# lighttransport/nanort

Hardware: AMD Instinct MI355X
Metric: Mrays/s (primary + 1-bounce) at 1920x1080, 1M-tri mesh; BVH build ms (higher is better)
Workload: dtype f32; 1 GPU; C3: Plane(1000,500) = 1,000,000 triangles fp32; 1920x1080 objrender-camera primaries + 1 cosine bounce per hit (2073600 + 2055142 rays per GPU per step); parallelism=replicated BVH, interleaved image rows per GPU

## Files before the change

### nanort_amd/csrc/api_ctx.hip

```cpp
#include "ctx.h"

struct TunableDesc {
  const char *name;
  long long lo, hi;
  long long (*get)(const nrt_ctx *);
  void (*set)(nrt_ctx *, long long);
};
#define NRT_TUNABLE(name_, lo_, hi_, field_, type_)                                                          \
  {name_, lo_, hi_, [](const nrt_ctx *c) -> long long { return (long long)c->field_; },                      \
   [](nrt_ctx *c, long long v) { c->field_ = (type_)v; }}
static const TunableDesc kTunables[] = {
    NRT_TUNABLE("refill_min", 1, 64, refill_min, unsigned),
    NRT_TUNABLE("trav_min", 1, 64, trav_min, unsigned),
    NRT_TUNABLE("trav_min4", 1, 64, trav_min4, unsigned),
    NRT_TUNABLE("f64_row_fetch", 0, 1, f64_row_fetch, int),
    NRT_TUNABLE("leaf_min", 1, 64, leaf_min, unsigned),
    NRT_TUNABLE("chunk_tail_pct", 0, 100, chunk_tail_pct, unsigned),
    NRT_TUNABLE("parts", 1, kMaxParts, num_parts, unsigned),
    NRT_TUNABLE("static_pct", 0, 100, static_pct, unsigned),
    NRT_TUNABLE("static_bands", 1, 64, static_bands, unsigned),
    NRT_TUNABLE("static_slice_groups", 1, 64, static_slice_groups, unsigned),
    NRT_TUNABLE("blocks_per_cu", 0, 8, max_blocks_per_cu, unsigned),
    NRT_TUNABLE("debug", 0, 0x7FFFFFFF, debug_flags, unsigned),
    NRT_TUNABLE("morton", 0, 1, morton, int),
    NRT_TUNABLE("cyl_split", 1, 64, cyl_split, int),
    NRT_TUNABLE("cyl_seg_radii", 1, 1024, cyl_seg_radii, int),
#ifdef NRT_PROF
    NRT_TUNABLE("subtree_rows", 0, 1, subtree_rows, int),
#endif
    NRT_TUNABLE("wide", 0, 1, wide, int),
    NRT_TUNABLE("wide4_big", 0, 2, wide4_big_ok, int),
    NRT_TUNABLE("wide4", 0, 1, wide4, int),
    NRT_TUNABLE("leaf_compact", 0, 1, leaf_compact, int),
    NRT_TUNABLE("tail_quad", 0, 16, tail_quad, unsigned),
    NRT_TUNABLE("dyn_head", 0, 1, dyn_head, int),
    NRT_TUNABLE("order4", 0, 1, order4, int),
    NRT_TUNABLE("launch_timing", 0, 1, launch_timing, int),
    NRT_TUNABLE("host_pipeline", 0, 1, host_pipeline, int),
    NRT_TUNABLE("wide_scramble", 0, 1, wide_scramble, int),
    {"chunk", 32, 1 << 20, [](const nrt_ctx *c) -> long long { return c->chunk; },
     [](nrt_ctx *c, long long v) { c->chunk = (unsigned)(v / 32) * 32u; }},
    {"lds_stack", 16, 32, [](const nrt_ctx *c) -> long long { return c->lds_stack; },
     [](nrt_ctx *c, long long v) { if (v == 16 || v == 24 || v == 32) c->lds_stack = (int)v; }},
    {"wide_stack", 8, 16, [](const nrt_ctx *c) -> long long { return c->wide_stack; },
     [](nrt_ctx *c, long long v) { if (v == 8 || v == 10 || v == 12 || v == 16) c->wide_stack = (int)v; }},
};
#undef NRT_TUNABLE

static const TunableDesc *tunable_find(const char *name) {
  if (!name) return nullptr;
  for (const TunableDesc &d : kTunables)
    if (!strcmp(d.name, name)) return &d;
  return nullptr;
}
static bool tunable_set(nrt_ctx *c, const char *name, long long v) {
  const TunableDesc *d = tunable_find(name);
  if (!d) return false;
  d->set(c, std::min(d->hi, std::max(d->lo, v)));
  memset(c->occupancy, 0, sizeof(c->occupancy));
  return true;
}

extern "C" {

nrt_status nrtCreate(int device, nrt_ctx **out) {
  if (!out) return fail(nullptr, NRT_ERR_INVALID, "nrtCreate: out == NULL");
  *out = nullptr;
  int ndev = 0;
  hipError_t e = hipGetDeviceCount(&ndev);
  if (e != hipSuccess || ndev <= 0)
    return fail(nullptr, NRT_ERR_DEVICE, "nrtCreate: no HIP device visible (%s)",
                e == hipSuccess ? "count == 0" : hipGetErrorString(e));
  if (device < 0 || device >= ndev)
    return fail(nullptr, NRT_ERR_INVALID, "nrtCreate: device %d out of range [0,%d)", device, ndev);
  nrt_ctx *c = new nrt_ctx();
  c->device = device;
  if ((e = hipSetDevice(device)) != hipSuccess ||
      (e = hipStreamCreateWithFlags(&c->stream, hipStreamNonBlocking)) != hipSuccess ||
      (e = hipEventCreate(&c->ev_b0)) != hipSuccess || (e = hipEventCreate(&c->ev_b1)) != hipSuccess ||
      (e = hipEventCreateWithFlags(&c->ev_build_state, hipEventDisableTiming)) != hipSuccess ||
      (e = hipEventCreateWithFlags(&c->ev_refit, hipEventDisableTiming)) != hipSuccess ||
      (e = hipHostMalloc(&c->build_state, kBuildPinnedBytes, hipHostMallocDefault)) != hipSuccess ||
      (e = hipMalloc((void **)&c->d_counters, 16 * sizeof(unsigned long long))) != hipSuccess) {
    fail(nullptr, NRT_ERR_DEVICE, "nrtCreate: %s", hipGetErrorString(e));
    nrtDestroy(c);
    return NRT_ERR_DEVICE;
  }
  for (nrt_ctx::LaunchSlot &sl : c->slots) {
    if ((e = hipMalloc((void **)&sl.d_cursor, 2 * kCursorStrideWords * 4 * kMaxParts)) != hipSuccess ||
        (e = hipMemset(sl.d_cursor, 0, 2 * kCursorStrideWords * 4 * kMaxParts)) != hipSuccess ||
        (e = hipEventCreateWithFlags(&sl.done, hipEventDisableTiming)) != hipSuccess ||
        (e = hipEventCreate(&sl.t0)) != hipSuccess || (e = hipEventCreate(&sl.t1)) != hipSuccess ||
        (e = hipHostMalloc((void **)&sl.h_done, sizeof(DoneRec), hipHostMallocPortable | hipHostMallocMapped | hipHostMallocCoherent)) != hipSuccess ||
        (e = hipHostGetDevicePointer((void **)&sl.d_done, sl.h_done, 0)) != hipSuccess ||
        (e = hipMalloc((void **)&sl.d_count, sizeof(DoneCount))) != hipSuccess ||
        (e = hipMemset(sl.d_count, 0, sizeof(DoneCount))) != hipSuccess ||
        (e = hipMemset((char *)sl.d_count + offsetof(DoneCount, t_begin), 0xFF, sizeof(unsigned long long))) != hipSuccess) {
      fail(nullptr, NRT_ERR_DEVICE, "nrtCreate: %s", hipGetErrorString(e));
      nrtDestroy(c);
      return NRT_ERR_DEVICE;
    }
  }
  for (nrt_ctx::LaunchSlot &sl : c->slots) memset(sl.h_done, 0, sizeof(DoneRec));
  hipDeviceProp_t prop;
  if (hipGetDeviceProperties(&prop, device) == hipSuccess && prop.multiProcessorCount > 0)
    c->num_cus = prop.multiProcessorCount;
  const bool allow_env = env_overrides_allowed();
  for (const TunableDesc &d : kTunables) {
    if (!allow_env) break;
    char env[64] = "NRT_";
    size_t k = 4;
    for (const char *p = d.name; *p && k + 1 < sizeof(env); p++) env[k++] = (char)toupper((unsigned char)*p);
    env[k] = 0;
    if (const char *e = getenv(env)) (void)tunable_set(c, d.name, atoll(e));
  }
  *out = c;
  return NRT_OK;
}

void nrtDestroy(nrt_ctx *c) {
  if (!c) return;
  (void)hipSetDevice(c->device);
  if (c->stream) (void)hipStreamSynchronize(c->stream);
  if (c->ev_refit) (void)refit_host_wait_locked(c);
  for (nrt_ctx::LaunchSlot &sl : c->slots) {
    if (sl.h_done || sl.done) (void)slot_done(c, sl);
    if (sl.d_cursor) (void)hipFree(sl.d_cursor);
    if (sl.d_count) (void)hipFree(sl.d_count);
    if (sl.h_done) (void)hipHostFree(sl.h_done);
    if (sl.spill.p) (void)hipFree(sl.spill.p);
    if (sl.spill_tmin.p) (void)hipFree(sl.spill_tmin.p);
    if (sl.cyl_hits.p) (void)hipFree(sl.cyl_hits.p);
    if (sl.cyl_bits.p) (void)hipFree(sl.cyl_bits.p);
    if (sl.done) (void)hipEventDestroy(sl.done);
    if (sl.t0) (void)hipEventDestroy(sl.t0);
    if (sl.t1) (void)hipEventDestroy(sl.t1);
  }
  free_tree(c);
  free_mesh(c);
  DevBuf *bufs[] = {&c->b_verts, &c->b_radii, &c->b_faces, &c->st_rays, &c->st_hits, &c->st_mask, &c->st_skip, &c->b_nodes, &c->b_indices, &c->b_tris, &c->b_wide, &c->b_wide4, &c->b_wide_scratch, &c->b_build_ws, &c->b_wave_clock, &c->b_seg_verts, &c->b_seg_radii, &c->b_seg_prim, &c->b_seg_off, &c->b_refit_plan, &c->b_refit_stage, &c->b_max_index, &c->b_verts1, &c->b_tris1, &c->st_times, &c->b_prim_masks, &c->b_leaf_masks, &c->st_ray_masks};
  for (DevBuf *b : bufs)
    if (b->p) (void)hipFree(b->p);
  if (c->d_counters) (void)hipFree(c->d_counters);
  if (c->build_state) (void)hipHostFree(c->build_state);
  if (c->h_max_index) (void)hipHostFree(c->h_max_index);
  hipEvent_t evs[] = {c->ev_b0, c->ev_b1, c->ev_build_state, c->ev_refit};
  for (hipEvent_t ev : evs)
    if (ev) (void)hipEventDestroy(ev);
  for (int k = 0; k < 2; k++)
    for (hipEvent_t e : {c->ev_in[k], c->ev_tr[k], c->ev_out[k]})
      if (e) (void)hipEventDestroy(e);
  if (c->copy_in) (void)hipStreamDestroy(c->copy_in);
  if (c->copy_out) (void)hipStreamDestroy(c->copy_out);
  if (c->stream) (void)hipStreamDestroy(c->stream);
  delete c;
}

const char *nrtLastError(const nrt_ctx *c) { return c ? c->err.c_str() : g_create_error.c_str(); }

const char *nrtVersion(void) { return "libnanort_hip 0.1 (gfx950, HIP)"; }

nrt_status nrtHostAlloc(size_t bytes, void **out) {
  if (!out) return fail(nullptr, NRT_ERR_INVALID, "nrtHostAlloc: out == NULL");
  *out = nullptr;
  if (bytes == 0) return NRT_OK;
  const hipError_t e = hipHostMalloc(out, bytes, hipHostMallocPortable);
  if (e != hipSuccess) {
    *out = nullptr;
    return fail(nullptr, NRT_ERR_DEVICE, "nrtHostAlloc: hipHostMalloc(%zu) failed: %s", bytes, hipGetErrorString(e));
  }
  return NRT_OK;
}
void nrtHostFree(void *p) {
  if (p) (void)hipHostFree(p);
}

int nrtDeviceCount(void) {
  int n = 0;
  if (hipGetDeviceCount(&n) != hipSuccess) {
    (void)hipGetLastError();
    return 0;
  }
  return n;
}

float nrtLastTraverseMs(nrt_ctx *c) {
  if (!c) return -1.f;
  hipEvent_t t0, t1;
  {
    std::unique_lock<std::mutex> lock(c->launch_mutex);
    if (c->last_timed_slot < 0) return -1.f;
    nrt_ctx::LaunchSlot &sl = c->slots[c->last_timed_slot];
    if (sl.last_has_rec) {
      if (wait_record(sl) != hipSuccess) return -1.f;
      const unsigned long long b = sl.h_done->t_begin, e = sl.h_done->t_end;
      const hipStream_t s = sl.stream;
      lock.unlock();
      if (hipStreamSynchronize(s) != hipSuccess) return -1.f;
      return e >= b ? (float)((double)(e - b) * 1e-5) : -1.f;
    }
    if (!sl.last_timed) return -1.f;
    t0 = sl.t0;
    t1 = sl.t1;
  }
  if (hipEventSynchronize(t1) != hipSuccess) return -1.f;
  float ms = -1.f;
  if (hipEventElapsedTime(&ms, t0, t1) != hipSuccess) return -1.f;
  return ms;
}

float nrtLastBuildMs(nrt_ctx *c) {
  if (!c || !c->have_build_time) return -1.f;
  return c->stats.build_secs * 1e3f;
}

nrt_status nrtSetLaunchTiming(nrt_ctx *c, int on) {
  if (!c) return NRT_ERR_INVALID;
  std::lock_guard<std::mutex> lock(c->launch_mutex);
  c->launch_timing = on ? 1 : 0;
  return NRT_OK;
}

nrt_status nrtSetTunable(nrt_ctx *c, const char *name, long long value) {
  if (!c) return NRT_ERR_INVALID;
  std::lock_guard<std::mutex> lock(c->launch_mutex);
  if (!tunable_set(c, name, value)) return fail(c, NRT_ERR_INVALID, "nrtSetTunable: unknown tunable '%s'", name ? name : "(null)");
  return NRT_OK;
}
nrt_status nrtGetTunable(nrt_ctx *c, const char *name, long long *value_out) {
  if (!c || !value_out) return NRT_ERR_INVALID;
  const TunableDesc *d = tunable_find(name);
  if (!d) return fail(c, NRT_ERR_INVALID, "nrtGetTunable: unknown tunable '%s'", name ? name : "(null)");
  std::lock_guard<std::mutex> lock(c->launch_mutex);
  *value_out = d->get(c);
  return NRT_OK;
}

const char *nrtLastKernelName(const nrt_ctx *c) { return c ? c->last_kernel : ""; }

#ifdef NRT_PROF
int nrtDebugCounters(nrt_ctx *c, unsigned long long *out, int cap) {
  if (!c || !out || cap < 16) return 1;
  if (hipStreamSynchronize(c->stream) != hipSuccess) return 1;
  if (hipDeviceSynchronize() != hipSuccess) return 1;
  return hipMemcpy(out, c->d_counters, 16 * sizeof(unsigned long long), hipMemcpyDeviceToHost) == hipSuccess ? 0 : 1;
}

long nrtDebugWaveClocks(nrt_ctx *c, unsigned long long *out, long cap) {
  if (!c || !out || !c->b_wave_clock.p) return -1;
  if (hipDeviceSynchronize() != hipSuccess) return -1;
  const long n = std::min<long>(cap, (long)c->wave_clock_waves);
  if (hipMemcpy(out, c->b_wave_clock.p, (size_t)n * kWaveClockWords * sizeof(unsigned long long), hipMemcpyDeviceToHost) != hipSuccess) return -1;
  return (long)c->wave_clock_waves;
}

#endif

}

nrt_status nrt_internal_tree_view(nrt_ctx *c, nrt::TreeViewF32 *out) {
  if (!c || !out) return NRT_ERR_INVALID;
  if (c->prec != 4 || !c->d_nodes || !c->d_wide) return fail(c, NRT_ERR_INVALID, "no fp32 tree on the device");
  HIPCHK(c, hipSetDevice(c->device));
  HIPCHK(c, refit_host_wait(c));
  HIPCHK(c, hipStreamSynchronize(c->stream));
  out->nodes = (const nrt_node_f32 *)c->d_nodes;
  out->indices = c->d_indices;
  out->wide = c->d_wide;
  out->wide4 = c->d_wide4;
  out->prims = c->d_tris;
  out->num_nodes = (uint32_t)c->num_nodes;
  out->num_indices = (uint32_t)c->num_indices;
  out->packed_leaves = c->packed_leaves;
  out->root_is_branch = c->root_is_branch;
  out->tree_nested = c->tree_nested;
  out->prim_kind = (uint32_t)c->prim_kind;
  out->tree_depth = c->tree_depth;
  out->max_leaf_count = c->max_leaf_count;
  out->generation = c->generation;
  return NRT_OK;
}
uint64_t nrt_internal_generation(const nrt_ctx *c) { return c ? c->generation : 0; }
int nrt_internal_device(const nrt_ctx *c) { return c ? c->device : 0; }
int nrt_internal_prim_kind(const nrt_ctx *c) { return c ? c->prim_kind : (int)kPrimTriangles; }
```

### nanort_amd/csrc/api_tree.hip

```cpp
#include "ctx.h"

template <typename T>
static nrt_status finish_leaf_records(nrt_ctx *c, hipStream_t s) {
  if (nrt_status st = ensure(c, c->b_tris, std::max<size_t>(1, c->num_indices) * leaf_record_bytes<T>(c->prim_kind))) return st;
  c->d_tris = c->b_tris.p;
  HIPCHK(c, launch_gather_leaf<T>(c->prim_kind, c->d_indices, c->d_faces, (const T *)c->d_verts, (const T *)c->d_radii, c->d_tris, (uint32_t)c->num_indices, s));
  if (c->d_verts1 && c->prim_kind == kPrimTriangles) {
    if (nrt_status st = ensure(c, c->b_tris1, std::max<size_t>(1, c->num_indices) * leaf_record_bytes<T>(c->prim_kind))) return st;
    c->d_tris1 = c->b_tris1.p;
    HIPCHK(c, launch_gather_leaf<T>(c->prim_kind, c->d_indices, c->d_faces, (const T *)c->d_verts1, (const T *)nullptr, c->d_tris1, (uint32_t)c->num_indices, s));
  }
  return NRT_OK;
}

template <typename T>
static nrt_status finish_wide(nrt_ctx *c, hipStream_t s) {
  nrt_status st;
  if ((st = ensure(c, c->b_wide, std::max<size_t>(1, c->num_branch_records) * sizeof(WideNode<T>)))) return st;
  c->d_wide = c->b_wide.p;
  c->packed_leaves = (c->min_leaf_count >= 1 && c->max_leaf_count <= kPackedMaxCount &&
                      c->num_indices <= (uint64_t)kPackedFirstMask) ? 1u : 0u;
  const size_t tiles = (c->num_nodes + 1023) / 1024;
  if ((st = ensure(c, c->b_wide_scratch, (tiles + c->num_nodes + 1) * sizeof(uint32_t)))) return st;
  c->d_wide4 = nullptr;
  if (c->wide4 && sizeof(T) == 4 && (c->num_branch_records < (1ull << 25) || (c->prim_kind == kPrimTriangles && c->wide4_big_ok))) {
    if ((st = ensure(c, c->b_wide4, std::max<size_t>(1, c->num_branch_records) * sizeof(Wide4Node<T>)))) return st;
    c->d_wide4 = c->b_wide4.p;
  }
  HIPCHK(c, launch_make_wide<T>((const typename Wire<T>::Node *)c->d_nodes, (uint32_t)c->num_nodes, c->packed_leaves,
                                (uint32_t *)c->b_wide_scratch.p, (WideNode<T> *)c->d_wide, (Wide4Node<T> *)c->d_wide4,
                                c->wide_scramble ? c->num_branch_records : 0u, s));
  return NRT_OK;
}

template <typename T>
static nrt_status finish_tree(nrt_ctx *c, hipStream_t s) {
  nrt_status st = finish_leaf_records<T>(c, s);
  return st ? st : finish_wide<T>(c, s);
}

template <typename T>
static nrt_status set_tree(nrt_ctx *c, const typename Wire<T>::Node *nodes, uint64_t num_nodes,
                           const uint32_t *indices, uint64_t num_indices) {
  if (!c) return NRT_ERR_INVALID;
  if (c->prec != (int)sizeof(T)) return fail(c, NRT_ERR_PRECISION, "nrtSetTree: set a mesh of this precision first");
  if (!nodes || !indices || num_nodes == 0) return fail(c, NRT_ERR_INVALID, "nrtSetTree: empty tree");
  if (num_nodes >= 0xFFFFFFFFull || num_indices >= 0xFFFFFFFFull)
    return fail(c, NRT_ERR_INVALID, "nrtSetTree: tree too large");
  for (uint64_t i = 0; i < num_indices; i++)
    if (indices[i] >= c->num_faces)
      return fail(c, NRT_ERR_INVALID, "nrtSetTree: indices[%llu]=%u >= num_faces %u",
                  (unsigned long long)i, indices[i], c->num_faces);
  uint32_t depth = 0, max_leaf = 0, min_leaf = 0xFFFFFFFFu, nested = 1;
  {
    std::vector<std::pair<uint32_t, uint32_t> > st;
    std::vector<uint8_t> seen(num_nodes, 0);
    st.push_back(std::make_pair(0u, 0u));
    while (!st.empty()) {
      std::pair<uint32_t, uint32_t> e = st.back();
      st.pop_back();
      const typename Wire<T>::Node &n = nodes[e.first];
      if (seen[e.first]) return fail(c, NRT_ERR_INVALID, "nrtSetTree: node %u reachable twice", e.first);
      seen[e.first] = 1;
      depth = std::max(depth, e.second);
      if (n.flag == 0) {
        if (n.data[0] >= num_nodes || n.data[1] >= num_nodes)
          return fail(c, NRT_ERR_INVALID, "nrtSetTree: node %u child out of range", e.first);
        if (n.axis < 0 || n.axis > 2) return fail(c, NRT_ERR_INVALID, "nrtSetTree: node %u axis %d", e.first, n.axis);
        for (int ch = 0; ch < 2; ch++) {
          const typename Wire<T>::Node &k = nodes[n.data[ch]];
          for (int ax = 0; ax < 3; ax++)
            if (!(k.bmin[ax] >= n.bmin[ax] && k.bmax[ax] <= n.bmax[ax])) nested = 0;
        }
        st.push_back(std::make_pair(n.data[1], e.second + 1));
        st.push_back(std::make_pair(n.data[0], e.second + 1));
      } else {
        if ((uint64_t)n.data[1] + n.data[0] > num_indices)
          return fail(c, NRT_ERR_INVALID, "nrtSetTree: leaf %u slots out of range", e.first);
        max_leaf = std::max(max_leaf, n.data[0]);
        min_leaf = std::min(min_leaf, n.data[0]);
      }
    }
  }
  HIPCHK(c, hipSetDevice(c->device));
  HIPCHK(c, wait_for_launches(c));
  free_tree(c);
  c->num_nodes = num_nodes;
  c->num_indices = num_indices;
  c->tree_depth = depth;
  c->max_leaf_count = max_leaf;
  c->min_leaf_count = min_leaf;
  c->root_is_branch = nodes[0].flag == 0 ? 1u : 0u;
  c->tree_nested = nested;
  c->num_branch_records = 0;
  for (uint64_t i = 0; i < num_nodes; i++)
    if (nodes[i].flag == 0) c->num_branch_records++;
  nrt_status st;
  if ((st = ensure(c, c->b_nodes, num_nodes * sizeof(typename Wire<T>::Node)))) return st;
  if ((st = ensure(c, c->b_indices, std::max<uint64_t>(1, num_indices) * sizeof(uint32_t)))) return st;
  c->d_nodes = c->b_nodes.p;
  c->d_indices = (uint32_t *)c->b_indices.p;
  HIPCHK(c, hipMemcpy(c->d_nodes, nodes, num_nodes * sizeof(typename Wire<T>::Node), hipMemcpyHostToDevice));
  HIPCHK(c, hipMemcpy(c->d_indices, indices, num_indices * sizeof(uint32_t), hipMemcpyHostToDevice));
  if ((st = finish_tree<T>(c, c->stream))) return st;
  HIPCHK(c, hipStreamSynchronize(c->stream));
  return NRT_OK;
}

template <typename T>
static nrt_status get_tree(nrt_ctx *c, typename Wire<T>::Node *nodes_out, uint32_t *indices_out) {
  if (!c) return NRT_ERR_INVALID;
  if (c->prec != (int)sizeof(T)) return fail(c, NRT_ERR_PRECISION, "nrtGetTree: precision mismatch");
  if (!c->d_nodes) return fail(c, NRT_ERR_INVALID, "nrtGetTree: no tree");
  NRT_RANGE("nrtGetTree (read-back)");
  HIPCHK(c, hipSetDevice(c->device));
  HIPCHK(c, refit_host_wait(c));
  HIPCHK(c, hipStreamSynchronize(c->stream));
  if (nodes_out)
    HIPCHK(c, hipMemcpy(nodes_out, c->d_nodes, c->num_nodes * sizeof(typename Wire<T>::Node), hipMemcpyDeviceToHost));
  if (indices_out)
    HIPCHK(c, hipMemcpy(indices_out, c->d_indices, c->num_indices * sizeof(uint32_t), hipMemcpyDeviceToHost));
  return NRT_OK;
}

template <typename T>
static nrt_status get_tree_bounds(nrt_ctx *c, T *bmin, T *bmax) {
  if (!c || !bmin || !bmax) return NRT_ERR_INVALID;
  if (c->prec != (int)sizeof(T)) return fail(c, NRT_ERR_PRECISION, "nrtGetTreeBounds: precision mismatch");
  if (!c->d_nodes) return fail(c, NRT_ERR_INVALID, "nrtGetTreeBounds: no tree");
  HIPCHK(c, hipSetDevice(c->device));
  HIPCHK(c, refit_host_wait(c));
  HIPCHK(c, hipStreamSynchronize(c->stream));
  T box[6];
  HIPCHK(c, hipMemcpy(box, c->d_nodes, sizeof(box), hipMemcpyDeviceToHost));
  for (int k = 0; k < 3; k++) {
    bmin[k] = box[k];
    bmax[k] = box[3 + k];
  }
  return NRT_OK;
}

template <typename T>
static nrt_status build(nrt_ctx *c, const typename Wire<T>::BuildOptions *opt, nrt_build_stats *stats_out,
                        uint64_t *num_nodes_out) {
  if (!c) return NRT_ERR_INVALID;
  if (c->prec != (int)sizeof(T)) return fail(c, NRT_ERR_PRECISION, "nrtBuild: set a mesh of this precision first");
  if (c->num_faces == 0) return fail(c, NRT_ERR_EMPTY, "nrtBuild: no primitives (reference Build() returns false)");
  uint32_t min_leaf = 4, max_depth = 256, bin_size = 64;
  if (opt) {
    min_leaf = opt->min_leaf_primitives;
    max_depth = opt->max_tree_depth;
    bin_size = opt->bin_size;
  }
  if (bin_size < 2) return fail(c, NRT_ERR_INVALID, "nrtBuild: bin_size must be > 1 (nanort.h:1905)");
  NRT_RANGE("nrtBuild");
  HIPCHK(c, hipSetDevice(c->device));
  HIPCHK(c, wait_for_launches(c));
  free_tree(c);
  BuildResult res;
  std::string err;
  HIPCHK(c, hipEventRecord(c->ev_b0, c->stream));
  const bool segs = c->prim_kind == kPrimCylinders && c->num_segs != 0 && sizeof(T) == 4;
  const uint32_t build_n = segs ? c->num_segs : c->num_faces;
  hipError_t e = gpu_build<T>(c->stream, segs ? (const T *)c->b_seg_verts.p : (const T *)c->d_verts, c->prim_kind == kPrimTriangles ? (const T *)c->d_verts1 : nullptr, c->d_faces, segs ? (const T *)c->b_seg_radii.p : (const T *)c->d_radii,
                              c->prim_kind, segs ? (const uint32_t *)c->b_seg_prim.p : nullptr, build_n, min_leaf, max_depth,
                              bin_size, (c->morton ? kBuildMorton : 0u) | (c->subtree_rows ? 0u : kBuildSubtreeDfs), &c->b_build_ws, &c->b_nodes, &c->b_indices, c->build_state, c->ev_build_state, &err);
  if (e != hipSuccess) return fail(c, NRT_ERR_DEVICE, "nrtBuild: %s (%s)", err.c_str(), hipGetErrorString(e));
  c->d_nodes = c->b_nodes.p;
  c->d_indices = (uint32_t *)c->b_indices.p;
  c->num_indices = build_n;
  NRT_RANGE_PUSH("build: leaf-ordered primitive records");
  nrt_status fst = finish_leaf_records<T>(c, c->stream);
  NRT_RANGE_POP();
  if (fst) {
    free_tree(c);
    return fst;
  }
  if ((e = gpu_build_result(c->build_state, c->ev_build_state, &res)) != hipSuccess) {
    free_tree(c);
    return fail(c, NRT_ERR_DEVICE, "nrtBuild: %s", hipGetErrorString(e));
  }
  c->num_nodes = res.num_nodes;
  c->tree_depth = res.max_depth;
  c->max_leaf_count = res.max_leaf_count;
  c->num_branch_records = res.num_branches;
  c->root_is_branch = res.num_nodes > 1 ? 1u : 0u;
  c->min_leaf_count = 1;
  c->tree_nested = 1;
  NRT_RANGE_PUSH("build: WideNode / Wide4Node records");
  fst = finish_wide<T>(c, c->stream);
  NRT_RANGE_POP();
  if (fst) {
    free_tree(c);
    return fst;
  }
  HIPCHK(c, hipEventRecord(c->ev_b1, c->stream));
  HIPCHK(c, hipEventSynchronize(c->ev_b1));
  c->have_build_time = true;
  float ms = 0.f;
  HIPCHK(c, hipEventElapsedTime(&ms, c->ev_b0, c->ev_b1));
  c->stats.max_tree_depth = res.max_depth;
  c->stats.num_leaf_nodes = res.num_leaves;
  c->stats.num_branch_nodes = res.num_branches;
  c->stats.build_secs = (ms + (segs ? c->segment_ms : 0.f)) * 1e-3f;
  if (stats_out) *stats_out = c->stats;
  if (num_nodes_out) *num_nodes_out = c->num_nodes;
  return NRT_OK;
}

template <typename T>
static nrt_status refit_plan(nrt_ctx *c, hipStream_t s) {
  if (c->refit_planned) return NRT_OK;
  if (nrt_status st = ensure(c, c->b_refit_plan, refit_plan_bytes(c->tree_depth, c->num_nodes))) return st;
  HIPCHK(c, launch_refit_plan<T>((const typename Wire<T>::Node *)c->d_nodes, c->num_nodes, c->num_branch_records, c->tree_depth,
                                 c->root_is_branch, (uint32_t *)c->b_refit_plan.p, s));
  c->refit_planned = true;
  return NRT_OK;
}

template <typename T>
static nrt_status refit_finish(nrt_ctx *c, const char *fn, hipError_t e, bool device, hipStream_t s, const char *remedy) {
  nrt_status st = NRT_OK;
  c->tree_nested = 1;
  if (e == hipSuccess && (st = finish_tree<T>(c, s))) e = hipErrorUnknown;
  if (e == hipSuccess && !device) e = hipStreamSynchronize(s);
  if (e == hipSuccess && device) {
    std::lock_guard<std::mutex> lock(c->launch_mutex);
    if ((e = hipEventRecord(c->ev_refit, s)) == hipSuccess) c->refit_pending = true;
  }
  if (e != hipSuccess) {
    const std::string why = st ? c->err : std::string(hipGetErrorString(e));
    (void)hipStreamSynchronize(s);
    free_tree(c);
    free_mesh(c);
    return fail(c, NRT_ERR_DEVICE, "%s: %s (the context's tree and primitives were dropped: %s)", fn, why.c_str(), remedy);
  }
  c->generation++;
  return NRT_OK;
}

template <typename T>
static nrt_status refit(nrt_ctx *c, const T *vertices, size_t stride, bool device, hipStream_t s) {
  const char *fn = device ? "nrtRefitDevice" : "nrtRefit";
  if (!c) return NRT_ERR_INVALID;
  if (!vertices) return fail(c, NRT_ERR_INVALID, "%s: NULL vertices", fn);
  if (c->prec != 0 && c->prec != (int)sizeof(T))
    return fail(c, NRT_ERR_PRECISION, "%s: the context holds %s primitives", fn, c->prec == 8 ? "f64" : "f32");
  if (c->prim_kind != kPrimTriangles) return fail(c, NRT_ERR_INVALID, "%s: only triangle meshes refit (this context holds %s)", fn,
                                                  kPrimKinds[c->prim_kind].name);
  if (c->d_verts1)
    return fail(c, NRT_ERR_INVALID, "%s: the context holds a motion keyframe (nrtSetMeshMotion): its boxes cover both keyframes and a refit of "
                "one would shrink them; remove the keyframe or set the mesh and build again", fn);
  if (!c->d_nodes) return fail(c, NRT_ERR_INVALID, "%s: no tree (call nrtBuild or nrtSetTree)", fn);
  if (stride < 3 * sizeof(T)) return fail(c, NRT_ERR_INVALID, "%s: vertex stride %zu < %zu", fn, stride, 3 * sizeof(T));
  if (device && (stride % sizeof(T) != 0 || (uintptr_t)vertices % sizeof(T) != 0))
    return fail(c, NRT_ERR_INVALID, "%s: vertex stride %zu or pointer not aligned to %zu bytes", fn, stride, sizeof(T));
  NRT_RANGE("nrtRefit");
  HIPCHK(c, hipSetDevice(c->device));
  HIPCHK(c, wait_for_launches(c));
  if (!device) s = c->stream;
  nrt_status st = NRT_OK;
  const uint32_t nv = c->num_verts;
  const size_t block = nv ? (size_t)(nv - 1) * stride + 3 * sizeof(T) : 0;
  const void *src = vertices;
  if (!device && nv) {
    if ((st = ensure(c, c->b_refit_stage, block))) return st;
    HIPCHK(c, hipMemcpyAsync(c->b_refit_stage.p, vertices, block, hipMemcpyHostToDevice, s));
    src = c->b_refit_stage.p;
  }
  if ((st = refit_plan<T>(c, s))) return st;
  const hipError_t e = launch_refit<T>(src, stride, nv, (T *)c->d_verts, c->d_faces, c->d_indices,
                                       (typename Wire<T>::Node *)c->d_nodes, c->num_nodes, c->num_branch_records, c->tree_depth,
                                       (const uint32_t *)c->b_refit_plan.p, s);
  return refit_finish<T>(c, fn, e, device, s, "set the mesh again");
}

static nrt_status refit_prims(nrt_ctx *c, const float *positions, const float *radii, uint32_t n, bool device, hipStream_t s) {
  const char *fn = device ? "nrtRefitPrimsDevice" : "nrtRefitPrims";
  if (!c) return NRT_ERR_INVALID;
  if (!positions) return fail(c, NRT_ERR_INVALID, "%s: NULL positions", fn);
  if (c->prec == 8) return fail(c, NRT_ERR_PRECISION, "%s: the context holds f64 primitives", fn);
  if (c->prec != 0 && c->prim_kind == kPrimTriangles)
    return fail(c, NRT_ERR_INVALID, "%s: this context holds triangles: refit a mesh with nrtRefit / nrtRefitDevice", fn);
  if (c->prec != 0 && c->prim_kind == kPrimCylinders)
    return fail(c, NRT_ERR_INVALID, "%s: cylinders do not refit: the tree is built over segments the builder cut them into, and which "
                "cylinder end a slot of the index array stands for is not recoverable from it (nrtSetCylinders + nrtBuild again)", fn);
  if (!c->d_nodes) return fail(c, NRT_ERR_INVALID, "%s: no tree (call nrtBuild or nrtSetTree)", fn);
  const PrimKind &k = kPrimKinds[c->prim_kind];
  if (n != c->num_faces) return fail(c, NRT_ERR_INVALID, "%s: num_prims %u differs from the context's %u %s", fn, n, c->num_faces, k.name);
  if (device && ((uintptr_t)positions % sizeof(float) != 0 || (uintptr_t)radii % sizeof(float) != 0))
    return fail(c, NRT_ERR_INVALID, "%s: pointer not aligned to 4 bytes", fn);
  NRT_RANGE("nrtRefitPrims");
  HIPCHK(c, hipSetDevice(c->device));
  HIPCHK(c, wait_for_launches(c));
  if (!device) s = c->stream;
  if (nrt_status st = refit_plan<float>(c, s)) return st;
  const hipMemcpyKind dir = device ? hipMemcpyDeviceToDevice : hipMemcpyHostToDevice;
  hipError_t e = hipMemcpyAsync(c->d_verts, positions, (size_t)k.pos_floats * n * sizeof(float), dir, s);
  if (e == hipSuccess && radii) e = hipMemcpyAsync(c->d_radii, radii, (size_t)k.radius_floats * n * sizeof(float), dir, s);
  if (e == hipSuccess)
    e = launch_refit_prims(c->prim_kind, (const float *)c->d_verts, (const float *)c->d_radii, c->d_indices, (nrt_node_f32 *)c->d_nodes, c->num_nodes,
                           c->num_branch_records, c->tree_depth, (const uint32_t *)c->b_refit_plan.p, s);
  return refit_finish<float>(c, fn, e, device, s, "set the primitives again");
}

extern "C" {

nrt_status nrtBuild_f32(nrt_ctx *c, const nrt_build_options_f32 *o, nrt_build_stats *st, uint64_t *nn) {
  return build<float>(c, o, st, nn);
}
nrt_status nrtBuild_f64(nrt_ctx *c, const nrt_build_options_f64 *o, nrt_build_stats *st, uint64_t *nn) {
  return build<double>(c, o, st, nn);
}

nrt_status nrtGetTree_f32(nrt_ctx *c, nrt_node_f32 *n, uint32_t *i) { return get_tree<float>(c, n, i); }
nrt_status nrtGetTree_f64(nrt_ctx *c, nrt_node_f64 *n, uint32_t *i) { return get_tree<double>(c, n, i); }
nrt_status nrtTreeSize(nrt_ctx *c, uint64_t *nn, uint64_t *ni) {
  if (!c) return NRT_ERR_INVALID;
  if (nn) *nn = c->num_nodes;
  if (ni) *ni = c->num_indices;
  return NRT_OK;
}
nrt_status nrtGetTreeBounds_f32(nrt_ctx *c, float *lo, float *hi) { return get_tree_bounds<float>(c, lo, hi); }
nrt_status nrtGetTreeBounds_f64(nrt_ctx *c, double *lo, double *hi) { return get_tree_bounds<double>(c, lo, hi); }

nrt_status nrtSetTree_f32(nrt_ctx *c, const nrt_node_f32 *n, uint64_t nn, const uint32_t *i, uint64_t ni) {
  return set_tree<float>(c, n, nn, i, ni);
}
nrt_status nrtSetTree_f64(nrt_ctx *c, const nrt_node_f64 *n, uint64_t nn, const uint32_t *i, uint64_t ni) {
  return set_tree<double>(c, n, nn, i, ni);
}

nrt_status nrtRefit_f32(nrt_ctx *c, const float *v, size_t stride) { return refit<float>(c, v, stride, false, nullptr); }
nrt_status nrtRefit_f64(nrt_ctx *c, const double *v, size_t stride) { return refit<double>(c, v, stride, false, nullptr); }
nrt_status nrtRefitDevice_f32(nrt_ctx *c, const float *v, size_t stride, void *s) { return refit<float>(c, v, stride, true, (hipStream_t)s); }
nrt_status nrtRefitDevice_f64(nrt_ctx *c, const double *v, size_t stride, void *s) { return refit<double>(c, v, stride, true, (hipStream_t)s); }
nrt_status nrtRefitPrims_f32(nrt_ctx *c, const float *p, const float *r, uint32_t n) { return refit_prims(c, p, r, n, false, nullptr); }
nrt_status nrtRefitPrimsDevice_f32(nrt_ctx *c, const float *p, const float *r, uint32_t n, void *s) { return refit_prims(c, p, r, n, true, (hipStream_t)s); }

}
```

### nanort_amd/csrc/build.hip

```cpp
#include <stddef.h>
#include <stdlib.h>

#include <algorithm>
#include <string>
#include <vector>


#include "build_dev.h"
#include "kernels.h"
#include "minmax_dev.h"
#include "prims_dev.h"

namespace nrt {

#ifndef NRT_BIN_REPL
#define NRT_BIN_REPL 4
#endif
#ifndef NRT_BIN_PRELOAD
#define NRT_BIN_PRELOAD 1
#endif
#ifndef NRT_BUILD_TILE
#define NRT_BUILD_TILE 2048
#endif
constexpr int kTile = NRT_BUILD_TILE;
constexpr int kSceneReplicas = 16;

template <typename E>
struct __attribute__((packed, aligned(4))) Vec3Of {
  E x, y, z;
};

template <typename T, bool MOTION>
__global__ __launch_bounds__(256) void k_prim_records(const T *__restrict__ verts, const T *__restrict__ verts1,
                                                      const uint32_t *__restrict__ faces,
                                                      const T *__restrict__ radii, int kind, uint32_t n,
                                                      const uint32_t *__restrict__ prim_map,
                                                      PrimRec<T> *__restrict__ recs,
                                                      BoundsAcc<T> *__restrict__ scene) {
  typedef typename Ord<T>::U U;
  __shared__ U s_acc[12];
  if (threadIdx.x < 12) s_acc[threadIdx.x] = (threadIdx.x % 6 < 3) ? Ord<T>::highest() : Ord<T>::lowest();
  __syncthreads();
  T lo[3], hi[3], clo[3], chi[3];
#pragma unroll
  for (int k = 0; k < 3; k++) {
    lo[k] = clo[k] = Lim<T>::max();
    hi[k] = chi[k] = -Lim<T>::max();
  }
  for (uint32_t i = blockIdx.x * 256u + threadIdx.x; i < n; i += gridDim.x * 256u) {
    PrimRec<T> r;
    Vec3Of<uint32_t> f = {0, 0, 0};
    Vec3Of<T> v0 = {T(0), T(0), T(0)}, v1 = v0, v2 = v0;
    if (faces) {
      f = *reinterpret_cast<const Vec3Of<uint32_t> *>(faces + 3 * (size_t)i);
      v0 = *reinterpret_cast<const Vec3Of<T> *>(verts + 3 * (size_t)f.x);
      v1 = *reinterpret_cast<const Vec3Of<T> *>(verts + 3 * (size_t)f.y);
      v2 = *reinterpret_cast<const Vec3Of<T> *>(verts + 3 * (size_t)f.z);
    }
    Vec3Of<T> w0 = v0, w1 = v0, w2 = v0;
    if constexpr (MOTION) {
      w0 = *reinterpret_cast<const Vec3Of<T> *>(verts1 + 3 * (size_t)f.x);
      w1 = *reinterpret_cast<const Vec3Of<T> *>(verts1 + 3 * (size_t)f.y);
      w2 = *reinterpret_cast<const Vec3Of<T> *>(verts1 + 3 * (size_t)f.z);
    }
#pragma unroll
    for (int k = 0; k < 3; k++) {
      const T p0 = k == 0 ? v0.x : (k == 1 ? v0.y : v0.z), p1 = k == 0 ? v1.x : (k == 1 ? v1.y : v1.z), p2 = k == 0 ? v2.x : (k == 1 ? v2.y : v2.z);
      prim_box_axis<T>(faces != nullptr, kind, i, k, verts, radii, p0, p1, p2, r.bmin[k], r.bmax[k], r.c[k]);
      if constexpr (MOTION) {
        const T q0 = k == 0 ? w0.x : (k == 1 ? w0.y : w0.z), q1 = k == 0 ? w1.x : (k == 1 ? w1.y : w1.z), q2 = k == 0 ? w2.x : (k == 1 ? w2.y : w2.z);
        T bmin1, bmax1, c1;
        prim_box_axis<T>(true, kind, i, k, verts1, radii, q0, q1, q2, bmin1, bmax1, c1);
        r.bmin[k] = tmin(r.bmin[k], bmin1);
        r.bmax[k] = tmax(r.bmax[k], bmax1);
        r.c[k] = (r.c[k] + c1) * T(0.5);
      }
      lo[k] = tmin(lo[k], r.bmin[k]);
      hi[k] = tmax(hi[k], r.bmax[k]);
      clo[k] = tmin(clo[k], r.c[k]);
      chi[k] = tmax(chi[k], r.c[k]);
    }
    r.prim = prim_map ? prim_map[i] : i;
    recs[i] = r;
  }
#pragma unroll
  for (int k = 0; k < 3; k++) {
    for (int off = 32; off > 0; off >>= 1) {
      lo[k] = tmin(lo[k], __shfl_xor(lo[k], off));
      hi[k] = tmax(hi[k], __shfl_xor(hi[k], off));
      clo[k] = tmin(clo[k], __shfl_xor(clo[k], off));
      chi[k] = tmax(chi[k], __shfl_xor(chi[k], off));
    }
  }
  if ((threadIdx.x & 63) == 0) {
#pragma unroll
    for (int k = 0; k < 3; k++) {
      atomicMin(&s_acc[k], Ord<T>::enc(lo[k]));
      atomicMax(&s_acc[3 + k], Ord<T>::enc(hi[k]));
      atomicMin(&s_acc[6 + k], Ord<T>::enc(clo[k]));
      atomicMax(&s_acc[9 + k], Ord<T>::enc(chi[k]));
    }
  }
  __syncthreads();
  BoundsAcc<T> *rep = scene + 1 + (blockIdx.x % kSceneReplicas);
  if (threadIdx.x < 12) {
    if (threadIdx.x % 6 < 3)
      atomicMin(&rep->v[threadIdx.x], s_acc[threadIdx.x]);
    else
      atomicMax(&rep->v[threadIdx.x], s_acc[threadIdx.x]);
  }
}

template <typename T>
struct GBins {
  uint32_t count[3][kMaxBins];
  typename Ord<T>::U bmin[3][kMaxBins][3];
  typename Ord<T>::U bmax[3][kMaxBins][3];
};

template <typename T>
__device__ __forceinline__ void clean_bins(GBins<T> *g, int k, unsigned bin) {
  g->count[k][bin] = 0;
  empty_box_e<T>(g->bmin[k][bin], g->bmax[k][bin]);
}
template <typename T>
__device__ __forceinline__ void clean_acc(BoundsAcc<T> *acc) {
  typedef typename Ord<T>::U U;
#pragma unroll
  for (int j = 0; j < 12; j++) acc->v[j] = (j % 6 < 3) ? (U)Ord<T>::highest() : (U)Ord<T>::lowest();
}

#ifndef NRT_TOP_REP
#define NRT_TOP_REP 4
#endif
constexpr uint32_t kRep = NRT_TOP_REP, kRepNodes = 8, kRepMinChunks = 64;
__device__ __forceinline__ bool rep_node(uint32_t num_active, uint32_t nchunks) {
  return kRep > 1u && num_active <= kRepNodes && nchunks >= kRepMinChunks;
}

template <typename T>
__global__ void k_init_scene(BoundsAcc<T> *scene, LevelInfo *info, uint32_t top_cap, GBins<T> *gbins, BoundsAcc<T> *child_acc,
                             uint32_t max_active) {
  if (blockIdx.x > 0) {
    const uint32_t c = blockIdx.x - 1u;
    for (int k = 0; k < 3; k++) clean_bins<T>(&gbins[max_active + c], k, threadIdx.x);
    if (threadIdx.x < 2) clean_acc<T>(&child_acc[2u * max_active + 2u * c + threadIdx.x]);
    return;
  }
  if (threadIdx.x < 12)
    for (int r = 0; r <= kSceneReplicas; r++) scene[r].v[threadIdx.x] = (threadIdx.x % 6 < 3) ? Ord<T>::highest() : Ord<T>::lowest();
  for (int k = 0; k < 3; k++) clean_bins<T>(&gbins[0], k, threadIdx.x);
  if (threadIdx.x < 2) clean_acc<T>(&child_acc[threadIdx.x]);
  if (threadIdx.x == 0) {
    info->num_active = 0;
    info->num_chunks = 0;
    info->num_small = 0;
    info->max_depth = 0;
    info->num_leaves = 0;
    info->num_branches = 0;
    info->max_leaf_count = 0;
    info->error = 0;
    info->cand_begin = 0;
    info->cand_end = 1;
    info->top_count = 1;
    info->child_base = 1;
    info->top_cap = top_cap;
    info->num_levels = 1;
    info->level_begin[0] = 0;
    info->level_begin[1] = 1;
  }
}

template <typename T>
__device__ __forceinline__ uint32_t classify(uint32_t n, uint32_t depth, LeafRule rule) {
  if (n <= (uint32_t)kHandoff) return KIND_SMALL;
  if (is_leaf(n, depth, rule)) return KIND_LEAF;
  return KIND_SPLIT;
}

template <typename T>
__device__ __forceinline__ void combine_scene(BoundsAcc<T> *scene, unsigned j) {
  typename Ord<T>::U x = scene[0].v[j];
  for (int r = 1; r <= kSceneReplicas; r++) {
    const typename Ord<T>::U y = scene[r].v[j];
    x = (j % 6 < 3) ? (y < x ? y : x) : (y > x ? y : x);
  }
  scene[0].v[j] = x;
}
template <typename T>
__global__ void k_combine_scene(BoundsAcc<T> *scene) {
  if (threadIdx.x < 12) combine_scene<T>(scene, threadIdx.x);
}

template <typename T>
__global__ void k_make_root(BoundsAcc<T> *scene, uint32_t n, LeafRule rule, uint32_t buf, TopNode<T> *top,
                            uint32_t *small_list, LevelInfo *info) {
  if (threadIdx.x < 12) combine_scene<T>(scene, threadIdx.x);
  __syncthreads();
  if (threadIdx.x != 0) return;
  TopNode<T> t;
#pragma unroll
  for (int k = 0; k < 3; k++) {
    t.bmin[k] = Ord<T>::dec(scene->v[k]);
    t.bmax[k] = Ord<T>::dec(scene->v[3 + k]);
    t.cmin[k] = Ord<T>::dec(scene->v[6 + k]);
    t.cmax[k] = Ord<T>::dec(scene->v[9 + k]);
  }
  t.l = 0;
  t.r = n;
  t.depth = 0;
  t.kind = classify<T>(n, 0, rule);
  t.axis = 0;
  t.split_bin = kMedian;
  t.nleft = 0;
  t.child0 = 0;
  t.size = 1;
  t.dfs = 0;
  t.buf = buf;
  t.chunk_base = 0;
  t.nchunks = 0;
  t.parent = kNoParent;
  top[0] = t;
  if (t.kind == KIND_SMALL) small_list[atomicAdd(&info->num_small, 1u)] = 0;
}

constexpr int kSortTile = 4096;

__device__ __forceinline__ uint32_t expand_bits10(uint32_t v) {
  v = (v * 0x00010001u) & 0xFF0000FFu;
  v = (v * 0x00000101u) & 0x0F00F00Fu;
  v = (v * 0x00000011u) & 0xC30C30C3u;
  v = (v * 0x00000005u) & 0x49249249u;
  return v;
}

template <typename T>
__global__ __launch_bounds__(256) void k_morton_keys(const PrimRec<T> *__restrict__ recs, uint32_t n,
                                                     const BoundsAcc<T> *__restrict__ scene,
                                                     uint32_t *__restrict__ keys, uint32_t *__restrict__ vals) {
  const uint32_t i = blockIdx.x * 256u + threadIdx.x;
  if (i >= n) return;
  uint32_t q[3];
#pragma unroll
  for (int k = 0; k < 3; k++) {
    const T lo = Ord<T>::dec(scene->v[6 + k]), hi = Ord<T>::dec(scene->v[9 + k]);
    q[k] = (uint32_t)bin_of<T>(recs[i].c[k], lo, bin_scale<T>(lo, hi, 1024), 1024);
  }
  keys[i] = (expand_bits10(q[0]) << 2) | (expand_bits10(q[1]) << 1) | expand_bits10(q[2]);
  vals[i] = i;
}

__global__ __launch_bounds__(256) void k_radix_hist(const uint32_t *__restrict__ keys, uint32_t n, int shift,
                                                    uint32_t *__restrict__ block_hist, uint32_t num_blocks) {
  __shared__ uint32_t s_h[256];
  s_h[threadIdx.x] = 0;
  __syncthreads();
  const uint32_t base = blockIdx.x * kSortTile;
  for (uint32_t k = threadIdx.x; k < (uint32_t)kSortTile; k += 256u) {
    const uint32_t i = base + k;
    if (i < n) atomicAdd(&s_h[(keys[i] >> shift) & 255u], 1u);
  }
  __syncthreads();
  block_hist[(size_t)threadIdx.x * num_blocks + blockIdx.x] = s_h[threadIdx.x];
}

__global__ __launch_bounds__(1024) void k_radix_scan(uint32_t *hist, uint32_t count) {
  __shared__ uint32_t s_wave[16];
  __shared__ uint32_t s_carry;
  const unsigned tid = threadIdx.x, lane = tid & 63, w = tid >> 6;
  if (tid == 0) s_carry = 0;
  __syncthreads();
  for (uint32_t base = 0; base < count; base += 1024u) {
    const uint32_t i = base + tid;
    const uint32_t v = i < count ? hist[i] : 0u;
    uint32_t inc = v;
    for (int off = 1; off < 64; off <<= 1) {
      const uint32_t t = __shfl_up(inc, off);
      if (lane >= (unsigned)off) inc += t;
    }
    if (lane == 63) s_wave[w] = inc;
    __syncthreads();
    uint32_t pre = s_carry;
    for (unsigned j = 0; j < w; j++) pre += s_wave[j];
    if (i < count) hist[i] = pre + inc - v;
    __syncthreads();
    if (tid == 1023) s_carry = pre + inc;
    __syncthreads();
  }
}

__global__ __launch_bounds__(256) void k_radix_scatter(const uint32_t *__restrict__ keys_in,
                                                       const uint32_t *__restrict__ vals_in,
                                                       uint32_t *__restrict__ keys_out, uint32_t *__restrict__ vals_out,
                                                       uint32_t n, int shift, const uint32_t *__restrict__ block_hist,
                                                       uint32_t num_blocks) {
  __shared__ uint32_t s_off[4][256];
  const unsigned tid = threadIdx.x, lane = tid & 63, w = tid >> 6;
  const uint32_t base = blockIdx.x * kSortTile + w * (kSortTile / 4);
  for (int d = lane; d < 256; d += 64) s_off[w][d] = 0;
  __syncthreads();
  for (uint32_t r = 0; r < (uint32_t)kSortTile / 4; r += 64u) {
    const uint32_t i = base + r + lane;
    if (i < n) atomicAdd(&s_off[w][(keys_in[i] >> shift) & 255u], 1u);
  }
  __syncthreads();
  {
    const uint32_t g = block_hist[(size_t)tid * num_blocks + blockIdx.x];
    uint32_t run = g;
    for (int ww = 0; ww < 4; ww++) {
      const uint32_t c = s_off[ww][tid];
      s_off[ww][tid] = run;
      run += c;
    }
  }
  __syncthreads();
  const unsigned long long lt = (1ull << lane) - 1ull;
  for (uint32_t r = 0; r < (uint32_t)kSortTile / 4; r += 64u) {
    const uint32_t i = base + r + lane;
    const bool valid = i < n;
    uint32_t key = 0, val = 0, d = 0;
    if (valid) {
      key = keys_in[i];
      val = vals_in[i];
      d = (key >> shift) & 255u;
    }
    unsigned long long same = valid ? __ballot(valid) : ~__ballot(valid);
#pragma unroll
    for (int b = 0; b < 8; b++) {
      const unsigned long long bal = __ballot((d >> b) & 1u);
      same &= ((d >> b) & 1u) ? bal : ~bal;
    }
    if (valid) {
      const uint32_t rank = (uint32_t)__builtin_popcountll(same & lt);
      const uint32_t off = s_off[w][d];
      keys_out[off + rank] = key;
      vals_out[off + rank] = val;
    }
    __builtin_amdgcn_wave_barrier();
    if (valid && (same & lt) == 0ull) s_off[w][d] += (uint32_t)__builtin_popcountll(same);
    __builtin_amdgcn_wave_barrier();
  }
}

template <typename T>
__global__ __launch_bounds__(256) void k_gather_records(const PrimRec<T> *__restrict__ in,
                                                        const uint32_t *__restrict__ order, uint32_t n,
                                                        PrimRec<T> *__restrict__ out) {
  const uint32_t i = blockIdx.x * 256u + threadIdx.x;
  if (i < n) out[i] = in[order[i]];
}


template <typename T>
__device__ __forceinline__ void make_children(TopNode<T> *top, const uint32_t *active, BoundsAcc<T> *child_acc, uint32_t a,
                                              uint32_t num_active, uint32_t max_active, LeafRule rule, uint32_t dst_buf,
                                              uint32_t *small_list, LevelInfo *info) {
  const TopNode<T> p = top[active[a]];
  bool small[2];
  uint32_t ci2[2];
  const bool folded = rep_node(num_active, p.nchunks);
  for (uint32_t c = 0; c < 2; c++) {
    TopNode<T> t;
    BoundsAcc<T> &acc = child_acc[2 * a + c];
    typename Ord<T>::U m[12];
#pragma unroll
    for (int j = 0; j < 12; j++) m[j] = acc.v[j];
    if (folded) {
      static_assert(kRep % 2u == 0u || kRep == 1u, "copies are folded in pairs");
      static_assert((kRep & (kRep - 1u)) == 0u, "a copy is selected with & (kRep - 1): NRT_TOP_REP must be a power of two");
      for (uint32_t r0 = 0; r0 < kRep; r0 += 2u) {
        BoundsAcc<T> *ar = &child_acc[2u * max_active + 2u * (a * kRep + r0) + c];
        typename Ord<T>::U x[2][12];
#pragma unroll
        for (int q = 0; q < 2; q++)
#pragma unroll
          for (int j = 0; j < 12; j++) x[q][j] = ar[2 * q].v[j];
#pragma unroll
        for (int q = 0; q < 2; q++)
#pragma unroll
          for (int j = 0; j < 12; j++) m[j] = (j % 6 < 3) ? (x[q][j] < m[j] ? x[q][j] : m[j]) : (x[q][j] > m[j] ? x[q][j] : m[j]);
        clean_acc<T>(&ar[0]);
        clean_acc<T>(&ar[2]);
      }
    }
#pragma unroll
    for (int k = 0; k < 3; k++) {
      t.bmin[k] = Ord<T>::dec(m[k]);
      t.bmax[k] = Ord<T>::dec(m[3 + k]);
      t.cmin[k] = Ord<T>::dec(m[6 + k]);
      t.cmax[k] = Ord<T>::dec(m[9 + k]);
    }
    clean_acc<T>(&acc);
    if (a + num_active < max_active) clean_acc<T>(&child_acc[2 * (a + num_active) + c]);
    t.l = c == 0 ? p.l : p.l + p.nleft;
    t.r = c == 0 ? p.l + p.nleft : p.r;
    t.depth = p.depth + 1;
    t.kind = classify<T>(t.r - t.l, t.depth, rule);
    t.axis = 0;
    t.split_bin = kMedian;
    t.nleft = 0;
    t.child0 = 0;
    t.size = 1;
    t.dfs = 0;
    t.buf = dst_buf;
    t.chunk_base = 0;
    t.nchunks = 0;
    t.parent = active[a] | (c ? kHighChild : 0u);
    const uint32_t ci = p.child0 + c;
    top[ci] = t;
    small[c] = t.kind == KIND_SMALL;
    ci2[c] = ci;
  }
  const unsigned long long m0 = __ballot(small[0]), m1 = __ballot(small[1]), live = __ballot(true);
  const uint32_t n0 = (uint32_t)__builtin_popcountll(m0), total = n0 + (uint32_t)__builtin_popcountll(m1);
  if (total) {
    const int leader = __builtin_ctzll(live);
    const unsigned lane = threadIdx.x & 63u;
    uint32_t base = 0;
    if ((int)lane == leader) base = atomicAdd(&info->num_small, total);
    base = (uint32_t)__builtin_amdgcn_readlane((int)base, leader);
    const unsigned long long below = (1ull << lane) - 1ull;
    if (small[0]) small_list[base + (uint32_t)__builtin_popcountll(m0 & below)] = ci2[0];
    if (small[1]) small_list[base + n0 + (uint32_t)__builtin_popcountll(m1 & below)] = ci2[1];
  }
}

#ifndef NRT_NARROW_LEVEL
#define NRT_NARROW_LEVEL 256
#endif
constexpr size_t kNarrowLevel = NRT_NARROW_LEVEL;
template <typename T>
__global__ __launch_bounds__(256) void k_children(TopNode<T> *top, const uint32_t *__restrict__ active, BoundsAcc<T> *child_acc,
                                                  uint32_t max_active, LeafRule rule, uint32_t dst_buf,
                                                  uint32_t *small_list, LevelInfo *info) {
  const uint32_t a = blockIdx.x * 256u + threadIdx.x;
  const uint32_t num_active = info->num_active;
  if (a >= num_active) return;
  make_children<T>(top, active, child_acc, a, num_active, max_active, rule, dst_buf, small_list, info);
}

template <typename T>
__global__ __launch_bounds__(1024) void k_level_setup(TopNode<T> *top, uint32_t *active, uint32_t *chunk_base,
                                                       LevelInfo *info, BoundsAcc<T> *child_acc, uint32_t max_active,
                                                       LeafRule rule, uint32_t dst_buf, uint32_t *small_list,
                                                       int with_children) {
  if (with_children) {
    const uint32_t prev_active = info->num_active;
    for (uint32_t a = threadIdx.x; a < prev_active; a += 1024u)
      make_children<T>(top, active, child_acc, a, prev_active, max_active, rule, dst_buf, small_list, info);
    __syncthreads();
  }
  const uint32_t cand_begin = info->cand_begin, cand_end = info->cand_end;
  __shared__ uint32_t s_wave[2][16];
  __shared__ uint32_t s_carry[2];
  const unsigned tid = threadIdx.x, lane = tid & 63, w = tid >> 6;
  if (tid < 2) s_carry[tid] = 0;
  __syncthreads();
  for (uint32_t base = cand_begin; base < cand_end; base += 1024u) {
    const uint32_t i = base + tid;
    uint32_t is_active = 0, nch = 0;
    if (i < cand_end && top[i].kind == KIND_SPLIT) {
      is_active = 1;
      nch = (top[i].r - top[i].l + kTile - 1) / kTile;
    }
    uint32_t a = is_active, c = nch;
    for (int off = 1; off < 64; off <<= 1) {
      uint32_t ta = __shfl_up(a, off), tc = __shfl_up(c, off);
      if (lane >= (unsigned)off) {
        a += ta;
        c += tc;
      }
    }
    if (lane == 63) {
      s_wave[0][w] = a;
      s_wave[1][w] = c;
    }
    __syncthreads();
    uint32_t pa = s_carry[0], pc = s_carry[1];
    for (unsigned j = 0; j < w; j++) {
      pa += s_wave[0][j];
      pc += s_wave[1][j];
    }
    if (is_active) {
      const uint32_t slot = pa + a - 1;
      active[slot] = i;
      chunk_base[slot] = pc + c - nch;
      top[i].chunk_base = pc + c - nch;
      top[i].nchunks = nch;
    }
    __syncthreads();
    if (tid == 1023) {
      s_carry[0] = pa + a;
      s_carry[1] = pc + c;
    }
    __syncthreads();
  }
  if (tid == 0) {
    uint32_t A = s_carry[0];
    const uint32_t tc = info->top_count;
    if (A && ((unsigned long long)tc + 2ull * A > info->top_cap || info->num_levels >= (uint32_t)kMaxTopLevels)) {
      info->error = 1;
      A = 0;
    }
    info->num_active = A;
    info->num_chunks = A ? s_carry[1] : 0;
    info->child_base = tc;
    info->cand_begin = tc;
    info->cand_end = tc + 2 * A;
    info->top_count = tc + 2 * A;
    if (A) {
      info->num_levels += 1;
      info->level_begin[info->num_levels] = tc + 2 * A;
    }
  }
}

__device__ __forceinline__ uint32_t find_task_wave(const uint32_t *chunk_base, uint32_t num_active, uint32_t chunk, unsigned lane) {
  uint32_t lo = 0, hi = num_active;
  while (hi - lo > 1) {
    const uint32_t step = (hi - lo + 63u) >> 6;
    const uint32_t idx = lo + lane * step;
    const bool ok = idx < hi && chunk_base[idx] <= chunk;
    const uint32_t j = (uint32_t)__builtin_popcountll(__ballot(ok)) - 1u;
    lo += j * step;
    hi = hi < lo + step ? hi : lo + step;
  }
  return lo;
}

template <typename T>
__device__ __forceinline__ void eval_split(int K, unsigned lane, const uint32_t cnt3[3], const typename Ord<T>::U mn3[3][3],
                                           const typename Ord<T>::U mx3[3][3], int &best_axis, uint32_t &best_bin,
                                           uint32_t &best_nl) {
  typedef typename Ord<T>::U U;
  T best_cost = Lim<T>::inf();
  best_axis = 0;
  best_bin = kMedian;
  best_nl = 0;
#pragma unroll
  for (int k = 0; k < 3; k++) {
    const uint32_t cnt = cnt3[k];
    U pmn[3], pmx[3];
#pragma unroll
    for (int d = 0; d < 3; d++) {
      pmn[d] = cnt ? mn3[k][d] : Ord<T>::highest();
      pmx[d] = cnt ? mx3[k][d] : Ord<T>::lowest();
    }
    uint32_t pc = cnt, sc = cnt;
    U smn[3] = {pmn[0], pmn[1], pmn[2]}, smx[3] = {pmx[0], pmx[1], pmx[2]};
    wave_prefix_e<T>(pc, pmn, pmx, lane);
    wave_suffix_e<T>(sc, smn, smx, lane);
    const uint32_t nl = wave_shr1<uint32_t>(0u, pc);
    U lmn[3], lmx[3];
#pragma unroll
    for (int d = 0; d < 3; d++) {
      lmn[d] = wave_shr1<U>(Ord<T>::highest(), pmn[d]);
      lmx[d] = wave_shr1<U>(Ord<T>::lowest(), pmx[d]);
    }
    const T cost = sah_cost<T>(lane >= 1 && (int)lane < K, nl, sc, lmn, lmx, smn, smx);
    const U ecost = Ord<T>::enc(cost);
    const U ebest = wave_umin<U>(ecost);
    const T c = Ord<T>::dec(ebest);
    const int who = (int)__builtin_ctzll(__ballot(ecost == ebest));
    if (c < best_cost) {
      best_cost = c;
      best_axis = k;
      best_bin = (uint32_t)who;
      best_nl = lane_bcast(nl, who);
    }
  }
}

template <typename T>
__global__ __launch_bounds__(256) void k_bin(TopNode<T> *top, const uint32_t *__restrict__ active,
                                             const uint32_t *__restrict__ chunk_base, const LevelInfo *info,
                                             const PrimRec<T> *__restrict__ recs, int kpack, GBins<T> *gbins,
                                             uint32_t *__restrict__ chunk_hist, uint32_t *chunk_left_base, uint32_t max_active) {
  if (blockIdx.x >= info->num_chunks) return;
  const uint32_t num_active = info->num_active;
  typedef typename Ord<T>::U U;
  constexpr int R = sizeof(T) == 4 ? NRT_BIN_REPL : (NRT_BIN_REPL > 2 ? 2 : NRT_BIN_REPL);
  static_assert(R >= 1 && (R & (R - 1)) == 0, "a lane's copy is threadIdx.x & (R - 1): NRT_BIN_REPL must be a power of two");
  __shared__ uint32_t s_cnt[3][kMaxBins][R];
  __shared__ U s_min[3][kMaxBins][3][R];
  __shared__ U s_max[3][kMaxBins][3][R];
  __shared__ uint32_t s_task;
  const unsigned rep = threadIdx.x & (unsigned)(R - 1);
  const uint32_t chunk = blockIdx.x;
  if (threadIdx.x < 64u) {
    const uint32_t t = find_task_wave(chunk_base, num_active, chunk, threadIdx.x);
    if (threadIdx.x == 0) s_task = t;
  }
  for (int i = threadIdx.x; i < 3 * kMaxBins * R; i += 256) {
    const int k = i / (kMaxBins * R), b = (i / R) % kMaxBins, r = i % R;
    s_cnt[k][b][r] = 0;
    for (int d = 0; d < 3; d++) {
      s_min[k][b][d][r] = Ord<T>::highest();
      s_max[k][b][d][r] = Ord<T>::lowest();
    }
  }
  __syncthreads();
  const uint32_t a = s_task;
  TopNode<T> &nd = top[active[a]];
  const uint32_t begin = nd.l + (chunk - chunk_base[a]) * kTile;
  const uint32_t end = (nd.r - begin < (uint32_t)kTile) ? nd.r : begin + kTile;
  const int K = node_bins(kpack, nd.r - nd.l);
  const bool whole_node = nd.nchunks == 1u;
  T lo[3], sc[3];
#pragma unroll
  for (int k = 0; k < 3; k++) {
    lo[k] = nd.cmin[k];
    sc[k] = bin_scale<T>(nd.cmin[k], nd.cmax[k], K);
  }
  static_assert(kTile % 256 == 0, "k_bin: a whole number of primitives per lane");
  constexpr uint32_t kPerLane = kTile / 256;
  {
    int pb[3] = {-1, -1, -1};
    uint32_t pc[3] = {0, 0, 0};
    U pmin[3][3], pmax[3][3];
    const uint32_t per = (end - begin + 255u) >> 8;
    const uint32_t p0 = begin + threadIdx.x * per;
    auto flush = [&](int k) {
      atomicAdd(&s_cnt[k][pb[k]][rep], pc[k]);
#pragma unroll
      for (int d = 0; d < 3; d++) {
        atomicMin(&s_min[k][pb[k]][d][rep], pmin[k][d]);
        atomicMax(&s_max[k][pb[k]][d][rep], pmax[k][d]);
      }
    };
    auto bin_rec = [&](const PrimRec<T> &r) {
      U emin[3], emax[3];
      int bk[3];
      encode_box<T>(r, emin, emax);
      record_bins<T>(r, lo, sc, K, bk);
#pragma unroll
      for (int k = 0; k < 3; k++) {
        const int b = bk[k];
        if (b == pb[k]) {
          pc[k]++;
#pragma unroll
          for (int d = 0; d < 3; d++) {
            pmin[k][d] = emin[d] < pmin[k][d] ? emin[d] : pmin[k][d];
            pmax[k][d] = emax[d] > pmax[k][d] ? emax[d] : pmax[k][d];
          }
        } else {
          if (pb[k] >= 0) flush(k);
          pb[k] = b;
          pc[k] = 1;
#pragma unroll
          for (int d = 0; d < 3; d++) {
            pmin[k][d] = emin[d];
            pmax[k][d] = emax[d];
          }
        }
      }
    };
#if NRT_BIN_PRELOAD
    constexpr uint32_t kHold = sizeof(T) == 4 ? (kPerLane < 8u ? kPerLane : 8u) : (kPerLane < 4u ? kPerLane : 4u);
    static_assert(kPerLane % kHold == 0, "k_bin: whole batches");
    for (uint32_t h0 = 0; h0 < per; h0 += kHold) {
      PrimRec<T> rr[kHold];
#pragma unroll
      for (uint32_t q = 0; q < kHold; q++)
        if (h0 + q < per && p0 + h0 + q < end) rr[q] = recs[p0 + h0 + q];
#pragma unroll
      for (uint32_t q = 0; q < kHold; q++)
        if (h0 + q < per && p0 + h0 + q < end) bin_rec(rr[q]);
    }
#else
    for (uint32_t it = 0; it < per; it++) {
      const uint32_t p = p0 + it;
      if (p >= end) break;
      bin_rec(recs[p]);
    }
#endif
#pragma unroll
    for (int k = 0; k < 3; k++)
      if (pb[k] >= 0) flush(k);
  }
  __syncthreads();
  if (R > 1) {
    for (int i = threadIdx.x; i < 3 * kMaxBins; i += 256) {
      const int k = i / kMaxBins, b = i % kMaxBins;
      uint32_t c = s_cnt[k][b][0];
#pragma unroll
      for (int r = 1; r < R; r++) c += s_cnt[k][b][r];
      s_cnt[k][b][0] = c;
#pragma unroll
      for (int d = 0; d < 3; d++) {
        U mn = s_min[k][b][d][0], mx = s_max[k][b][d][0];
#pragma unroll
        for (int r = 1; r < R; r++) {
          const U a_ = s_min[k][b][d][r], b_ = s_max[k][b][d][r];
          mn = a_ < mn ? a_ : mn;
          mx = b_ > mx ? b_ : mx;
        }
        s_min[k][b][d][0] = mn;
        s_max[k][b][d][0] = mx;
      }
    }
    __syncthreads();
  }
  if (whole_node) {
    if (threadIdx.x < 64u) {
      const unsigned lane = threadIdx.x;
      uint32_t cnt3[3] = {0, 0, 0};
      U mn3[3][3], mx3[3][3];
#pragma unroll
      for (int k = 0; k < 3; k++) {
        if ((int)lane < K) cnt3[k] = s_cnt[k][lane][0];
#pragma unroll
        for (int d = 0; d < 3; d++) {
          mn3[k][d] = s_min[k][lane][d][0];
          mx3[k][d] = s_max[k][lane][d][0];
        }
      }
      int best_axis;
      uint32_t best_bin, best_nl;
      eval_split<T>(K, lane, cnt3, mn3, mx3, best_axis, best_bin, best_nl);
      if (best_bin == kMedian) best_nl = (nd.r - nd.l) >> 1;
      if (lane == 0) {
        nd.axis = best_axis;
        nd.split_bin = best_bin;
        nd.nleft = best_nl;
        nd.child0 = info->child_base + 2 * a;
        chunk_left_base[chunk] = 0;
      }
      if (a + num_active < max_active)
        for (int k = 0; k < 3; k++) clean_bins<T>(&gbins[a + num_active], k, lane);
    }
    return;
  }
  GBins<T> *g = rep_node(num_active, nd.nchunks) ? &gbins[max_active + a * kRep + ((chunk - chunk_base[a]) & (kRep - 1u))] : &gbins[a];
  for (int i = threadIdx.x; i < 3 * kMaxBins; i += 256) {
    const int k = i / kMaxBins, b = i % kMaxBins;
    const uint32_t c = s_cnt[k][b][0];
    chunk_hist[(size_t)chunk * (3 * kMaxBins) + i] = c;
    if (c) {
      atomicAdd(&g->count[k][b], c);
      for (int d = 0; d < 3; d++) {
        atomicMin(&g->bmin[k][b][d], s_min[k][b][d][0]);
        atomicMax(&g->bmax[k][b][d], s_max[k][b][d][0]);
      }
    }
  }
}

template <typename T>
__global__ __launch_bounds__(64) void k_split(TopNode<T> *top, const uint32_t *__restrict__ active,
                                              GBins<T> *gbins, int kpack,
                                              const uint32_t *__restrict__ chunk_hist, uint32_t *chunk_left_base,
                                              const LevelInfo *info, uint32_t max_active) {
  const uint32_t a = blockIdx.x;
  const uint32_t num_active = info->num_active;
  if (a >= num_active) return;
  const uint32_t next_top_base = info->child_base;
  const unsigned lane = threadIdx.x;
  TopNode<T> &nd = top[active[a]];
  GBins<T> &g = gbins[a];
  typedef typename Ord<T>::U U;
  const uint32_t n = nd.r - nd.l, cb = nd.chunk_base, nch = nd.nchunks;
  if (nch == 1u) return;
  const int K = node_bins(kpack, n);
  uint32_t cnt3[3] = {0, 0, 0};
  U mn3[3][3], mx3[3][3];
#pragma unroll
  for (int k = 0; k < 3; k++) {
    if ((int)lane < K) cnt3[k] = g.count[k][lane];
    empty_box_e<T>(mn3[k], mx3[k]);
#pragma unroll
    for (int d = 0; d < 3; d++)
      if ((int)lane < K) {
        mn3[k][d] = g.bmin[k][lane][d];
        mx3[k][d] = g.bmax[k][lane][d];
      }
  }
  if (rep_node(num_active, nch)) {
#pragma unroll
    for (int k = 0; k < 3; k++) {
      uint32_t rc[kRep];
      U rmn[kRep][3], rmx[kRep][3];
#pragma unroll
      for (uint32_t r = 0; r < kRep; r++) {
        const GBins<T> &gr = gbins[max_active + a * kRep + r];
        rc[r] = 0;
        empty_box_e<T>(rmn[r], rmx[r]);
        if ((int)lane < K) {
          rc[r] = gr.count[k][lane];
#pragma unroll
          for (int d = 0; d < 3; d++) {
            rmn[r][d] = gr.bmin[k][lane][d];
            rmx[r][d] = gr.bmax[k][lane][d];
          }
        }
      }
#pragma unroll
      for (uint32_t r = 0; r < kRep; r++) {
        cnt3[k] += rc[r];
#pragma unroll
        for (int d = 0; d < 3; d++) {
          mn3[k][d] = rmn[r][d] < mn3[k][d] ? rmn[r][d] : mn3[k][d];
          mx3[k][d] = rmx[r][d] > mx3[k][d] ? rmx[r][d] : mx3[k][d];
        }
      }
    }
#pragma unroll
    for (uint32_t r = 0; r < kRep; r++)
#pragma unroll
      for (int k = 0; k < 3; k++) clean_bins<T>(&gbins[max_active + a * kRep + r], k, lane);
  }
#pragma unroll
  for (int k = 0; k < 3; k++) {
    clean_bins<T>(&g, k, lane);
    if (a + num_active < max_active) clean_bins<T>(&gbins[a + num_active], k, lane);
  }
  int best_axis;
  uint32_t best_bin, best_nl;
  eval_split<T>(K, lane, cnt3, mn3, mx3, best_axis, best_bin, best_nl);
  if (best_bin == kMedian) best_nl = n >> 1;

  uint32_t carry = 0;
  for (uint32_t j0 = 0; j0 < nch; j0 += 64u) {
    const uint32_t j = j0 + lane;
    uint32_t left = 0;
    if (j < nch) {
      if (best_bin == kMedian) {
        const uint32_t start = j * kTile, len = (n - start < (uint32_t)kTile) ? n - start : kTile;
        left = best_nl > start ? (best_nl - start < len ? best_nl - start : len) : 0;
      } else {
        const uint4 *h4 = reinterpret_cast<const uint4 *>(chunk_hist + (size_t)(cb + j) * (3 * kMaxBins) + best_axis * kMaxBins);
        uint4 hv[kMaxBins / 4];
#pragma unroll
        for (int q = 0; q < kMaxBins / 4; q++) hv[q] = h4[q];
#pragma unroll
        for (int q = 0; q < kMaxBins / 4; q++) {
          const uint32_t b0 = 4u * (uint32_t)q;
          left += (b0 < best_bin ? hv[q].x : 0u) + (b0 + 1u < best_bin ? hv[q].y : 0u) + (b0 + 2u < best_bin ? hv[q].z : 0u) +
                  (b0 + 3u < best_bin ? hv[q].w : 0u);
        }
      }
    }
    uint32_t inc = left;
    for (int off = 1; off < 64; off <<= 1) {
      const uint32_t t = __shfl_up(inc, off);
      if (lane >= (unsigned)off) inc += t;
    }
    if (j < nch) chunk_left_base[cb + j] = carry + inc - left;
    carry += __shfl(inc, 63);
  }
  if (lane == 0) {
    nd.axis = best_axis;
    nd.split_bin = best_bin;
    nd.nleft = best_nl;
    nd.child0 = next_top_base + 2 * a;
  }
}

template <typename T>
__global__ __launch_bounds__(256) void k_partition(const TopNode<T> *__restrict__ top,
                                                   const uint32_t *__restrict__ active,
                                                   const uint32_t *__restrict__ chunk_base, const LevelInfo *info,
                                                   const uint32_t *__restrict__ chunk_left_base,
                                                   const PrimRec<T> *__restrict__ src, PrimRec<T> *__restrict__ dst,
                                                   int kpack, BoundsAcc<T> *child_acc, uint32_t max_active) {
  typedef typename Ord<T>::U U;
  __shared__ uint32_t s_task;
  __shared__ uint32_t s_w[2][4];
  __shared__ U s_acc[2][12];
  const unsigned tid = threadIdx.x, lane = tid & 63, w = tid >> 6;
  const uint32_t chunk = blockIdx.x;
  if (chunk >= info->num_chunks) return;
  const uint32_t num_active = info->num_active;
  if (tid < 64u) {
    const uint32_t t = find_task_wave(chunk_base, num_active, chunk, tid);
    if (tid == 0) s_task = t;
  }
  if (tid < 24) s_acc[tid / 12][tid % 12] = ((tid % 12) % 6 < 3) ? (U)Ord<T>::highest() : (U)Ord<T>::lowest();
  __syncthreads();
  const uint32_t a = s_task;
  const TopNode<T> &nd = top[active[a]];
  const uint32_t off_in_node = (chunk - chunk_base[a]) * kTile;
  const uint32_t begin = nd.l + off_in_node;
  const uint32_t end = (nd.r - begin < (uint32_t)kTile) ? nd.r : begin + kTile;
  const uint32_t left_base = chunk_left_base[chunk];
  const uint32_t right_base = off_in_node - left_base;
  const int axis = nd.axis;
  const uint32_t split_bin = nd.split_bin, nleft = nd.nleft;
  const T lo = axis == 0 ? nd.cmin[0] : (axis == 1 ? nd.cmin[1] : nd.cmin[2]);
  const T hi = axis == 0 ? nd.cmax[0] : (axis == 1 ? nd.cmax[1] : nd.cmax[2]);
  const T sc = bin_scale<T>(lo, hi, node_bins(kpack, nd.r - nd.l));
  const int K = node_bins(kpack, nd.r - nd.l);

  T acc_lo[2][3], acc_hi[2][3], acc_clo[2][3], acc_chi[2][3];
#pragma unroll
  for (int s = 0; s < 2; s++)
#pragma unroll
    for (int d = 0; d < 3; d++) {
      acc_lo[s][d] = acc_clo[s][d] = Lim<T>::max();
      acc_hi[s][d] = acc_chi[s][d] = -Lim<T>::max();
    }

  uint32_t run_l = 0, run_r = 0;
  PrimRec<T> r_next;
  if (begin + tid < end) r_next = src[begin + tid];
  for (uint32_t p0 = begin; p0 < end; p0 += 256u) {
    const uint32_t p = p0 + tid;
    const bool valid = p < end;
    PrimRec<T> r;
    if (valid) r = r_next;
    if (p + 256u < end) r_next = src[p + 256u];
    bool left = false;
    if (valid) left = goes_left<T>(split_bin == kMedian, p - nd.l, nleft, pick_axis<T>(r.c, axis), lo, sc, K, split_bin);
    const unsigned long long bl = __ballot(valid && left), br = __ballot(valid && !left);
    if (lane == 0) {
      s_w[0][w] = (uint32_t)__builtin_popcountll(bl);
      s_w[1][w] = (uint32_t)__builtin_popcountll(br);
    }
    __syncthreads();
    uint32_t pl = 0, pr = 0, tl = 0, tr = 0;
#pragma unroll
    for (unsigned j = 0; j < 4; j++) {
      if (j < w) {
        pl += s_w[0][j];
        pr += s_w[1][j];
      }
      tl += s_w[0][j];
      tr += s_w[1][j];
    }
    if (valid) {
      const unsigned long long lt = (1ull << lane) - 1ull;
      uint32_t d;
      const int s = left ? 0 : 1;
      if (left)
        d = nd.l + left_base + run_l + pl + (uint32_t)__builtin_popcountll(bl & lt);
      else
        d = nd.l + nleft + right_base + run_r + pr + (uint32_t)__builtin_popcountll(br & lt);
      dst[d] = r;
#pragma unroll
      for (int k = 0; k < 3; k++) {
        if (s == 0) {
          acc_lo[0][k] = tmin(acc_lo[0][k], r.bmin[k]);
          acc_hi[0][k] = tmax(acc_hi[0][k], r.bmax[k]);
          acc_clo[0][k] = tmin(acc_clo[0][k], r.c[k]);
          acc_chi[0][k] = tmax(acc_chi[0][k], r.c[k]);
        } else {
          acc_lo[1][k] = tmin(acc_lo[1][k], r.bmin[k]);
          acc_hi[1][k] = tmax(acc_hi[1][k], r.bmax[k]);
          acc_clo[1][k] = tmin(acc_clo[1][k], r.c[k]);
          acc_chi[1][k] = tmax(acc_chi[1][k], r.c[k]);
        }
      }
    }
    run_l += tl;
    run_r += tr;
    __syncthreads();
  }
#pragma unroll
  for (int s = 0; s < 2; s++)
#pragma unroll
    for (int k = 0; k < 3; k++) {
      for (int off = 32; off > 0; off >>= 1) {
        acc_lo[s][k] = tmin(acc_lo[s][k], __shfl_xor(acc_lo[s][k], off));
        acc_hi[s][k] = tmax(acc_hi[s][k], __shfl_xor(acc_hi[s][k], off));
        acc_clo[s][k] = tmin(acc_clo[s][k], __shfl_xor(acc_clo[s][k], off));
        acc_chi[s][k] = tmax(acc_chi[s][k], __shfl_xor(acc_chi[s][k], off));
      }
      if (lane == 0) {
        atomicMin(&s_acc[s][k], Ord<T>::enc(acc_lo[s][k]));
        atomicMax(&s_acc[s][3 + k], Ord<T>::enc(acc_hi[s][k]));
        atomicMin(&s_acc[s][6 + k], Ord<T>::enc(acc_clo[s][k]));
        atomicMax(&s_acc[s][9 + k], Ord<T>::enc(acc_chi[s][k]));
      }
    }
  __syncthreads();
  if (tid < 24) {
    const int s = tid / 12, j = tid % 12;
    BoundsAcc<T> *acc = rep_node(num_active, nd.nchunks)
                            ? &child_acc[2u * max_active + 2u * (a * kRep + ((chunk - chunk_base[a]) & (kRep - 1u))) + s]
                            : &child_acc[2 * a + s];
    if (j % 6 < 3)
      atomicMin(&acc->v[j], s_acc[s][j]);
    else
      atomicMax(&acc->v[j], s_acc[s][j]);
  }
}


#ifndef NRT_LAYOUT_LDS
#define NRT_LAYOUT_LDS 16384
#endif
constexpr uint32_t kLayoutLds = NRT_LAYOUT_LDS;
constexpr uint32_t kLayoutOwn = kLayoutLds / 1024;

constexpr uint32_t kLayoutCut = 8;
template <typename T>
__global__ __launch_bounds__(1024) void k_layout(TopNode<T> *top, LevelInfo *info) {
  extern __shared__ uint32_t s_dyn[];
  __shared__ uint32_t s_upper[1u << kLayoutCut];
  __shared__ uint32_t s_nupper;
  const uint32_t total = info->top_count;
  uint32_t *s_size = s_dyn, *s_par = s_dyn + kLayoutLds;
  uint32_t leaves = 0, branches = 0, deepest = 0, biggest = 0;
  auto count_node = [&](uint32_t kind, uint32_t depth, uint32_t prims, uint32_t size, uint32_t nleft, uint32_t split_bin, uint32_t nchunks) {
    if (kind == KIND_SPLIT) branches++;
    if (kind == KIND_LEAF) {
      leaves++;
      deepest = depth > deepest ? depth : deepest;
      biggest = prims > biggest ? prims : biggest;
    }
    if (kind == KIND_SMALL) {
      leaves += nleft;
      branches += size - nleft;
      deepest = split_bin > deepest ? split_bin : deepest;
      biggest = nchunks > biggest ? nchunks : biggest;
    }
  };
  if (total <= kLayoutLds) {
    uint32_t own[kLayoutOwn], dep[kLayoutOwn];
    uint32_t kid[kLayoutOwn];
    uint32_t small_mask = 0;
#pragma unroll
    for (uint32_t j = 0; j < kLayoutOwn; j++) {
      const uint32_t i = threadIdx.x + 1024u * j;
      own[j] = 0;
      dep[j] = 0xFFFFFFFFu;
      kid[j] = kNoParent;
      if (i < total) {
        static_assert(offsetof(TopNode<T>, l) % 8 == 0 && sizeof(TopNode<T>) % 8 == 0 && offsetof(TopNode<T>, parent) == offsetof(TopNode<T>, l) + 52, "TopNode: 14 words from l");
        const uint2 *w = reinterpret_cast<const uint2 *>(&top[i].l);
        const uint2 lr = w[0], dk = w[1], as = w[2], nc = w[3], sd = w[4], np = w[6];
        const uint32_t kind = dk.y;
        own[j] = kind == KIND_SMALL ? sd.x : 1u;
        dep[j] = dk.x;
        s_size[i] = own[j];
        s_par[i] = np.y;
        if (kind == KIND_SPLIT) kid[j] = nc.y;
        if (kind == KIND_SMALL) small_mask |= 1u << j;
        count_node(kind, dk.x, lr.y - lr.x, sd.x, nc.x, as.y, np.x);
      }
    }
    __syncthreads();
#pragma unroll
    for (uint32_t j = 0; j < kLayoutOwn; j++) {
      const uint32_t i = threadIdx.x + 1024u * j;
      if (i < total && dep[j] > kLayoutCut) {
        uint32_t p = s_par[i] & ~kHighChild;
        for (uint32_t d = dep[j] - 1u; d >= kLayoutCut; d--) {
          atomicAdd(&s_size[p], own[j]);
          p = s_par[p] & ~kHighChild;
        }
      }
    }
    __syncthreads();
    for (int d = (int)kLayoutCut - 1; d >= 0; d--) {
#pragma unroll
      for (uint32_t j = 0; j < kLayoutOwn; j++) {
        const uint32_t i = threadIdx.x + 1024u * j;
        if (dep[j] == (uint32_t)d && kid[j] != kNoParent) s_size[i] = 1u + s_size[kid[j]] + s_size[kid[j] + 1u];
      }
      __syncthreads();
    }
#pragma unroll
    for (uint32_t j = 0; j < kLayoutOwn; j++) {
      const uint32_t i = threadIdx.x + 1024u * j;
      if (i < total) {
        uint32_t dfs = 0;
        for (uint32_t x = i, pw = s_par[i]; (pw & ~kHighChild) != kNoParent; x = pw & ~kHighChild, pw = s_par[x])
          dfs += 1u + ((pw & kHighChild) ? s_size[x - 1u] : 0u);
        reinterpret_cast<uint2 *>(&top[i].l)[4] = make_uint2(((small_mask >> j) & 1u) ? own[j] : s_size[i], dfs);
      }
    }
    if (threadIdx.x == 0) info->num_nodes = s_size[0];
  } else {
    if (threadIdx.x == 0) s_nupper = 0;
    __syncthreads();
    for (uint32_t i = threadIdx.x; i < total; i += 1024u)
      if (top[i].depth < kLayoutCut && top[i].kind == KIND_SPLIT) s_upper[atomicAdd(&s_nupper, 1u)] = i;
    __syncthreads();
    for (int d = (int)kLayoutCut - 1; d >= 0; d--) {
      for (uint32_t k = threadIdx.x; k < s_nupper; k += 1024u) {
        TopNode<T> &t = top[s_upper[k]];
        if (t.depth == (uint32_t)d) t.size = 1u + top[t.child0].size + top[t.child0 + 1u].size;
      }
      __syncthreads();
    }
    if (threadIdx.x == 0) info->num_nodes = top[0].size;
    for (uint32_t i = threadIdx.x; i < total; i += 1024u) {
      const TopNode<T> &t = top[i];
      count_node(t.kind, t.depth, t.r - t.l, t.size, t.nleft, t.split_bin, t.nchunks);
    }
  }
  for (int off = 32; off > 0; off >>= 1) {
    leaves += __shfl_down(leaves, off);
    branches += __shfl_down(branches, off);
    const uint32_t od = __shfl_down(deepest, off), ob = __shfl_down(biggest, off);
    deepest = od > deepest ? od : deepest;
    biggest = ob > biggest ? ob : biggest;
  }
  if ((threadIdx.x & 63u) == 0u) {
    if (leaves) atomicAdd(&info->num_leaves, leaves);
    if (branches) atomicAdd(&info->num_branches, branches);
    if (deepest) atomicMax(&info->max_depth, deepest);
    if (biggest) atomicMax(&info->max_leaf_count, biggest);
  }
}

template <typename T>
__global__ __launch_bounds__(256) void k_layout_init(TopNode<T> *top, const LevelInfo *info) {
  const uint32_t i = blockIdx.x * 256u + threadIdx.x;
  if (i >= info->top_count || info->top_count <= kLayoutLds) return;
  if (top[i].kind != KIND_SMALL) top[i].size = 1u;
}
template <typename T>
__global__ __launch_bounds__(256) void k_layout_sizes(TopNode<T> *top, const LevelInfo *info) {
  const uint32_t i = blockIdx.x * 256u + threadIdx.x;
  if (i >= info->top_count || info->top_count <= kLayoutLds) return;
  const uint32_t own = top[i].kind == KIND_SMALL ? top[i].size : 1u;
  const uint32_t dep = top[i].depth;
  if (dep <= kLayoutCut) return;
  uint32_t p = top[i].parent & ~kHighChild;
  for (uint32_t d = dep - 1u; d >= kLayoutCut; d--) {
    atomicAdd(&top[p].size, own);
    p = top[p].parent & ~kHighChild;
  }
}
template <typename T>
__global__ __launch_bounds__(256) void k_layout_dfs(TopNode<T> *top, const LevelInfo *info) {
  const uint32_t i = blockIdx.x * 256u + threadIdx.x;
  if (i >= info->top_count || info->top_count <= kLayoutLds) return;
  uint32_t dfs = 0;
  for (uint32_t x = i, pw = top[i].parent; (pw & ~kHighChild) != kNoParent; x = pw & ~kHighChild, pw = top[x].parent)
    dfs += 1u + ((pw & kHighChild) ? top[x - 1u].size : 0u);
  top[i].dfs = dfs;
}

template <typename T>
__global__ __launch_bounds__(256) void k_emit_top(const TopNode<T> *__restrict__ top, const LevelInfo *info,
                                                  const PrimRec<T> *__restrict__ recs0,
                                                  const PrimRec<T> *__restrict__ recs1,
                                                  typename Wire<T>::Node *nodes, uint32_t *indices) {
  const uint32_t i = blockIdx.x * 256u + threadIdx.x;
  if (i >= info->top_count) return;
  const TopNode<T> &t = top[i];
  if (t.kind == KIND_SMALL) return;
  typename Wire<T>::Node nd;
#pragma unroll
  for (int d = 0; d < 3; d++) {
    nd.bmin[d] = t.bmin[d];
    nd.bmax[d] = t.bmax[d];
  }
  if (t.kind == KIND_SPLIT) {
    nd.flag = 0;
    nd.axis = t.axis;
    nd.data[0] = top[t.child0].dfs;
    nd.data[1] = top[t.child0 + 1].dfs;
  } else {
    nd.flag = 1;
    nd.axis = 0;
    nd.data[0] = t.r - t.l;
    nd.data[1] = t.l;
    const PrimRec<T> *src = t.buf ? recs1 : recs0;
    for (uint32_t p = t.l; p < t.r; p++) indices[p] = src[p].prim;
  }
  nodes[t.dfs] = nd;
}

template <typename T>
__global__ __launch_bounds__(64) void k_emit_small(const TopNode<T> *__restrict__ top,
                                                   const uint32_t *__restrict__ small_list,
                                                   const typename Wire<T>::Node *__restrict__ scratch_nodes,
                                                   const uint16_t *__restrict__ premap, typename Wire<T>::Node *nodes,
                                                   const LevelInfo *info) {
  if (blockIdx.x >= info->num_small) return;
  const TopNode<T> &t = top[small_list[blockIdx.x]];
  const typename Wire<T>::Node *src = scratch_nodes + 2 * (size_t)t.l;
  if (premap) {
    const uint16_t *map = premap + 2 * (size_t)t.l;
    for (uint32_t i = threadIdx.x; i < t.size; i += 64u) {
      typename Wire<T>::Node nd = src[i];
      if (nd.flag == 0) {
        nd.data[0] = t.dfs + map[nd.data[0]];
        nd.data[1] = t.dfs + map[nd.data[1]];
      }
      nodes[t.dfs + map[i]] = nd;
    }
    return;
  }
  for (uint32_t i = threadIdx.x; i < t.size; i += 64u) {
    typename Wire<T>::Node nd = src[i];
    if (nd.flag == 0) {
      nd.data[0] += t.dfs;
      nd.data[1] += t.dfs;
    }
    nodes[t.dfs + i] = nd;
  }
}

static inline size_t align_up(size_t x, size_t a) { return (x + a - 1) / a * a; }

template <typename T>
struct BuildPlan {
  size_t max_top, max_active, max_chunks;
  size_t off_recs0, off_recs1, off_scratch, off_top, off_child_acc, off_active, off_chunk_base, off_gbins,
      off_chunk_hist, off_chunk_left, off_small, off_scene, off_info, off_sort, off_premap, sort_blocks, total;
  BuildPlan(uint32_t n, size_t top_scale, bool tiny_top = false) {
    typedef typename Wire<T>::Node Node;
    max_active = (size_t)n / kHandoff + 2;
    max_chunks = (size_t)n / kTile + max_active + 1;
    max_top = top_scale * (4 * ((size_t)n / kHandoff + 1) + 64);
    if (tiny_top) max_top = 16;
    size_t o = 0;
    auto take = [&](size_t bytes) {
      const size_t at = o;
      o = align_up(o + bytes, 256);
      return at;
    };
    off_recs0 = take((size_t)n * sizeof(PrimRec<T>));
    off_recs1 = take((size_t)n * sizeof(PrimRec<T>));
    off_scratch = take(2 * (size_t)n * sizeof(Node));
    off_premap = take(2 * (size_t)n * sizeof(uint16_t));
    off_top = take(max_top * sizeof(TopNode<T>));
    off_child_acc = take(2 * (max_active + kRepNodes * kRep) * sizeof(BoundsAcc<T>));
    off_active = take(max_active * sizeof(uint32_t));
    off_chunk_base = take(max_active * sizeof(uint32_t));
    off_gbins = take((max_active + kRepNodes * kRep) * sizeof(GBins<T>));
    off_chunk_hist = take(max_chunks * 3 * kMaxBins * sizeof(uint32_t));
    off_chunk_left = take(max_chunks * sizeof(uint32_t));
    off_small = take((max_top + 1) * sizeof(uint32_t));
    off_scene = take((1 + kSceneReplicas) * sizeof(BoundsAcc<T>));
    off_info = take(sizeof(LevelInfo));
    sort_blocks = ((size_t)n + kSortTile - 1) / kSortTile;
    off_sort = take((4 * (size_t)n + 256 * sort_blocks) * sizeof(uint32_t));
    total = o;
  }
};

#define BCHK(call)                                                      \
  do {                                                                  \
    hipError_t e_ = (call);                                             \
    if (e_ != hipSuccess) {                                             \
      *err = std::string(#call) + ": " + hipGetErrorString(e_);         \
      return e_;                                                        \
    }                                                                   \
  } while (0)

template <typename T>
hipError_t gpu_build(hipStream_t s, const T *d_verts, const T *d_verts1, const uint32_t *d_faces, const T *d_radii, int prim_kind, const uint32_t *d_prim_map, uint32_t n,
                     uint32_t min_leaf, uint32_t max_depth, uint32_t bin_size, unsigned build_flags, DevBuf *workspace, DevBuf *nodes_buf,
                     DevBuf *indices_buf, void *pinned, hipEvent_t ev, std::string *err) {
  typedef typename Wire<T>::Node Node;
  const bool morton_order = (build_flags & kBuildMorton) != 0;
  static_assert(offsetof(LevelInfo, level_begin) <= kBuildPinnedBytes, "state block");
  const int K = (int)(bin_size < 2 ? 2 : (bin_size > (uint32_t)kMaxBins ? (uint32_t)kMaxBins : bin_size));
  const int Ks = K < kSmallBins ? K : kSmallBins;
  const size_t state_bytes = offsetof(LevelInfo, level_begin);
  volatile const LevelInfo *hp = (volatile const LevelInfo *)pinned;

  const char *tiny_env = env_overrides_allowed() ? getenv("NRT_BUILD_TINY_TOP") : nullptr;
  const bool tiny_top = tiny_env && atoi(tiny_env) != 0;
  for (size_t top_scale = 1;; top_scale *= 8) {
    const BuildPlan<T> plan(n, top_scale, tiny_top && top_scale == 1);
    BCHK(devbuf_ensure(workspace, plan.total));
    BCHK(devbuf_ensure(indices_buf, (size_t)n * sizeof(uint32_t)));
    BCHK(devbuf_ensure(nodes_buf, (2 * (size_t)n) * sizeof(Node)));
    char *base = (char *)workspace->p;
    PrimRec<T> *recs[2] = {(PrimRec<T> *)(base + plan.off_recs0), (PrimRec<T> *)(base + plan.off_recs1)};
    Node *scratch = (Node *)(base + plan.off_scratch);
    uint16_t *premap = (uint16_t *)(base + plan.off_premap);
    TopNode<T> *top = (TopNode<T> *)(base + plan.off_top);
    BoundsAcc<T> *child_acc = (BoundsAcc<T> *)(base + plan.off_child_acc);
    uint32_t *active = (uint32_t *)(base + plan.off_active);
    uint32_t *chunk_base = (uint32_t *)(base + plan.off_chunk_base);
    GBins<T> *gbins = (GBins<T> *)(base + plan.off_gbins);
    uint32_t *chunk_hist = (uint32_t *)(base + plan.off_chunk_hist);
    uint32_t *chunk_left = (uint32_t *)(base + plan.off_chunk_left);
    uint32_t *small_list = (uint32_t *)(base + plan.off_small);
    BoundsAcc<T> *scene = (BoundsAcc<T> *)(base + plan.off_scene);
    LevelInfo *info = (LevelInfo *)(base + plan.off_info);
    uint32_t *indices = (uint32_t *)indices_buf->p;

    NRT_RANGE_PUSH("build: primitive records (per-prim AABB + centroid, scene bounds)");
    hipLaunchKernelGGL((k_init_scene<T>), dim3(1 + kRepNodes * kRep), dim3(64), 0, s, scene, info, (uint32_t)plan.max_top, gbins, child_acc,
                       (uint32_t)plan.max_active);
    {
      unsigned grid = (unsigned)std::min<size_t>(((size_t)n + 255) / 256, 2048);
      if (d_verts1 != nullptr && d_faces != nullptr)
        hipLaunchKernelGGL((k_prim_records<T, true>), dim3(grid), dim3(256), 0, s, d_verts, d_verts1, d_faces, d_radii, prim_kind, n, d_prim_map, recs[0], scene);
      else
        hipLaunchKernelGGL((k_prim_records<T, false>), dim3(grid), dim3(256), 0, s, d_verts, nullptr, d_faces, d_radii, prim_kind, n, d_prim_map, recs[0], scene);
    }
    NRT_RANGE_POP();
    int cur = 0;
    if (morton_order && n > 1) {
      NRT_RANGE("build: Morton keys + radix sort");
      uint32_t *keys[2] = {(uint32_t *)(base + plan.off_sort), (uint32_t *)(base + plan.off_sort) + (size_t)n};
      uint32_t *vals[2] = {keys[1] + (size_t)n, keys[1] + 2 * (size_t)n};
      uint32_t *block_hist = keys[1] + 3 * (size_t)n;
      const unsigned nb = (unsigned)plan.sort_blocks;
      hipLaunchKernelGGL((k_combine_scene<T>), dim3(1), dim3(64), 0, s, scene);
      hipLaunchKernelGGL((k_morton_keys<T>), dim3((n + 255) / 256), dim3(256), 0, s, recs[0], n, scene, keys[0], vals[0]);
      int pp = 0;
      for (int shift = 0; shift < 32; shift += 8) {
        hipLaunchKernelGGL(k_radix_hist, dim3(nb), dim3(256), 0, s, keys[pp], n, shift, block_hist, nb);
        hipLaunchKernelGGL(k_radix_scan, dim3(1), dim3(1024), 0, s, block_hist, 256u * nb);
        hipLaunchKernelGGL(k_radix_scatter, dim3(nb), dim3(256), 0, s, keys[pp], vals[pp], keys[1 - pp], vals[1 - pp], n,
                           shift, block_hist, nb);
        pp = 1 - pp;
      }
      hipLaunchKernelGGL((k_gather_records<T>), dim3((n + 255) / 256), dim3(256), 0, s, recs[0], vals[pp], n, recs[1]);
      cur = 1;
    }
    const LeafRule rule = make_leaf_rule(min_leaf, max_depth);
    hipLaunchKernelGGL((k_make_root<T>), dim3(1), dim3(64), 0, s, scene, n, rule, (uint32_t)cur, top, small_list,
                       info);
    BCHK(hipGetLastError());

    int expect = 0;
    for (size_t m = (size_t)n / kHandoff; m > 0; m >>= 1) expect++;
    const int first_check = (n <= (uint32_t)kHandoff) ? 0 : expect + 2;
    bool overflow = false;
    uint32_t num_small = 0;
    NRT_RANGE_PUSH("build: top phase (level setup / bin / split / partition per level)");
    for (int level = 0;; level++) {
      const size_t prev_max = level == 0 ? 0 : (level - 1 < 31 ? std::min<size_t>((size_t)1 << (level - 1), plan.max_active) : plan.max_active);
      const bool wide = prev_max > kNarrowLevel;
      if (wide)
        hipLaunchKernelGGL((k_children<T>), dim3((unsigned)((prev_max + 255) / 256)), dim3(256), 0, s, top, active, child_acc,
                           (uint32_t)plan.max_active, rule, (uint32_t)cur, small_list, info);
      hipLaunchKernelGGL((k_level_setup<T>), dim3(1), dim3(1024), 0, s, top, active, chunk_base, info, child_acc,
                         (uint32_t)plan.max_active, rule, (uint32_t)cur, small_list, wide ? 0 : 1);
      const bool check = level >= first_check;
      if (check) {
        BCHK(hipMemcpyAsync(pinned, info, state_bytes, hipMemcpyDeviceToHost, s));
        BCHK(hipEventRecord(ev, s));
      }
      const size_t a_max = level < 31 ? std::min<size_t>((size_t)1 << level, plan.max_active) : plan.max_active;
      const size_t c_max = std::min<size_t>((size_t)n / kTile + a_max + 1, plan.max_chunks);
      hipLaunchKernelGGL((k_bin<T>), dim3((unsigned)c_max), dim3(256), 0, s, top, active, chunk_base, info, recs[cur],
                         K | (Ks << 8), gbins, chunk_hist, chunk_left, (uint32_t)plan.max_active);
      hipLaunchKernelGGL((k_split<T>), dim3((unsigned)a_max), dim3(64), 0, s, top, active, gbins, K | (Ks << 8), chunk_hist,
                         chunk_left, info, (uint32_t)plan.max_active);
      hipLaunchKernelGGL((k_partition<T>), dim3((unsigned)c_max), dim3(256), 0, s, top, active, chunk_base, info,
                         chunk_left, recs[cur], recs[1 - cur], K | (Ks << 8), child_acc, (uint32_t)plan.max_active);
      BCHK(hipGetLastError());
      cur = 1 - cur;
      if (check) {
        BCHK(hipEventSynchronize(ev));
        if (hp->error) {
          overflow = true;
          break;
        }
        if (hp->num_active == 0) {
          num_small = hp->num_small;
          break;
        }
      }
    }
    NRT_RANGE_POP();
    if (overflow) continue;
    NRT_RANGE("build: subtree phase + layout + emission");

    const uint16_t *emit_map = nullptr;
    if (num_small)
      emit_map = launch_subtree<T>(top, small_list, recs[0], recs[1], Ks, rule, scratch, premap, indices, info, num_small,
                                   (build_flags & kBuildSubtreeDfs) != 0, s);
    BCHK(hipFuncSetAttribute(reinterpret_cast<const void *>(&k_layout<T>), hipFuncAttributeMaxDynamicSharedMemorySize,
                             (int)(2 * kLayoutLds * sizeof(uint32_t))));
    if (plan.max_top > kLayoutLds) {
      const unsigned lg = (unsigned)((plan.max_top + 255) / 256);
      hipLaunchKernelGGL((k_layout_init<T>), dim3(lg), dim3(256), 0, s, top, info);
      hipLaunchKernelGGL((k_layout_sizes<T>), dim3(lg), dim3(256), 0, s, top, info);
    }
    hipLaunchKernelGGL((k_layout<T>), dim3(1), dim3(1024), 2 * kLayoutLds * sizeof(uint32_t), s, top, info);
    if (plan.max_top > kLayoutLds)
      hipLaunchKernelGGL((k_layout_dfs<T>), dim3((unsigned)((plan.max_top + 255) / 256)), dim3(256), 0, s, top, info);
    BCHK(hipMemcpyAsync(pinned, info, state_bytes, hipMemcpyDeviceToHost, s));
    BCHK(hipEventRecord(ev, s));
    Node *nodes = (Node *)nodes_buf->p;
    hipLaunchKernelGGL((k_emit_top<T>), dim3((unsigned)((plan.max_top + 255) / 256)), dim3(256), 0, s, top, info, recs[0], recs[1],
                       nodes, indices);
    if (num_small)
      hipLaunchKernelGGL((k_emit_small<T>), dim3(num_small), dim3(64), 0, s, top, small_list, scratch, emit_map, nodes, info);
    BCHK(hipGetLastError());
    return hipSuccess;
  }
}

hipError_t gpu_build_result(const void *pinned, hipEvent_t ev, BuildResult *res) {
  hipError_t e = hipEventSynchronize(ev);
  if (e != hipSuccess) return e;
  volatile const LevelInfo *hp = (volatile const LevelInfo *)pinned;
  res->num_nodes = hp->num_nodes;
  res->max_depth = hp->max_depth;
  res->num_leaves = hp->num_leaves;
  res->num_branches = hp->num_branches;
  res->max_leaf_count = hp->max_leaf_count;
  return hipSuccess;
}

NRT_INSTANTIATE_F32_F64(gpu_build)

}
```

### nanort_amd/csrc/ctx.h

```cpp
#pragma once
#include <hip/hip_runtime.h>
#include <stdarg.h>
#include <stdio.h>
#include <stdlib.h>
#include <string.h>
#include <ctype.h>
#include <math.h>
#include <cmath>

#include <algorithm>
#include <atomic>
#include <chrono>
#include <mutex>
#include <thread>
#include <string>
#include <vector>

#include "kernels.h"
#include "launch_plan.h"
#ifdef NRT_PROF
#include "../../include/nanort_hip_prof.h"
#endif

using namespace nrt;

inline thread_local std::string g_create_error;

enum class Walk { Literal, OneLevel, TwoLevel, Own };

struct nrt_ctx {
  int device = 0;
  hipStream_t stream = nullptr;
  std::string err;
  int prec = 0;
  int num_cus = 256;

  int prim_kind = kPrimTriangles;
  uint32_t cyl_test_cap = 1;
  uint32_t curve_subdiv = 4;
  DevBuf b_seg_verts, b_seg_radii, b_seg_prim, b_seg_off;
  uint32_t num_segs = 0;
  int cyl_split = 32;
  int cyl_seg_radii = 8;
  DevBuf b_verts, b_radii, b_faces;
  void *d_verts = nullptr;
  void *d_radii = nullptr;
  uint32_t *d_faces = nullptr;
  uint32_t num_faces = 0, num_verts = 0;
  DevBuf b_max_index;
  uint32_t *h_max_index = nullptr;

  DevBuf b_nodes, b_indices, b_tris, b_wide, b_wide4, b_wide_scratch, b_build_ws;
  void *d_nodes = nullptr;
  uint32_t *d_indices = nullptr;
  void *d_tris = nullptr;
  void *d_wide = nullptr;
  void *d_wide4 = nullptr;
  uint32_t num_branch_records = 0;
  uint64_t num_nodes = 0, num_indices = 0;
  uint32_t tree_depth = 0;
  uint32_t max_leaf_count = 0, min_leaf_count = 0;
  uint32_t packed_leaves = 0;
  uint32_t root_is_branch = 0;
  uint32_t tree_nested = 1;
  nrt_build_stats stats = {0, 0, 0, 0.f};
  uint64_t generation = 0;
  DevBuf b_refit_plan, b_refit_stage;
  bool refit_planned = false;
  hipEvent_t ev_refit = nullptr;
  bool refit_pending = false;

  struct LaunchSlot {
    uint32_t *d_cursor = nullptr;
    unsigned parity = 0;
    DevBuf spill, spill_tmin;
    DevBuf cyl_hits, cyl_bits;
    hipEvent_t done = nullptr;
    hipEvent_t t0 = nullptr, t1 = nullptr;
    hipStream_t stream = nullptr;
    bool used = false;
    DoneRec *h_done = nullptr, *d_done = nullptr;
    DoneCount *d_count = nullptr;
    uint32_t seq = 0;
    bool rec_pending = false;
    bool last_has_rec = false;
    bool last_timed = false;
  };
  static constexpr int kSlots = 4;
  LaunchSlot slots[kSlots];
  unsigned next_victim = 0;
  std::mutex launch_mutex;
  std::mutex host_mutex;
  unsigned long long *d_counters = nullptr;
  DevBuf st_rays, st_hits, st_mask;
  DevBuf st_skip;
  hipStream_t copy_in = nullptr, copy_out = nullptr;
  hipEvent_t ev_in[2] = {nullptr, nullptr}, ev_tr[2] = {nullptr, nullptr}, ev_out[2] = {nullptr, nullptr};
  int host_pipeline = 1;
  DevBuf b_wave_clock;
  uint32_t wave_clock_waves = 0;

  int lds_stack = kLdsStackDefault;
  unsigned chunk = 128, chunk_tail_pct = 0, refill_min = 44, trav_min = 16, leaf_min = 32;
  int f64_row_fetch = 1;
  unsigned tail_quad = 4;
  unsigned trav_min4 = 24;
  unsigned num_parts = 8;
  unsigned debug_flags = 0;
  int subtree_rows = 1;
  int morton = 0;
  unsigned static_pct = 16;
  unsigned static_bands = 8;
  unsigned static_slice_groups = 2;
  unsigned max_blocks_per_cu = 0;
  int wide = 1, wide_stack = 10;
  int wide4 = 1;
  int wide4_big_ok = 1;
  int order4 = 0;
  int leaf_compact = 1;
  int dyn_head = 1;
  int wide_scramble = 0;
  struct { int lds_entries; unsigned blocks_per_cu; } occupancy[(int)Walk::Own + kNumOwnWalks][kNumPrimKinds] = {};

  hipEvent_t ev_b0 = nullptr, ev_b1 = nullptr;
  hipEvent_t ev_build_state = nullptr;
  void *build_state = nullptr;
  int last_timed_slot = -1;
  int launch_timing = 0;
  bool have_build_time = false;
  float segment_ms = 0.f;
  const char *last_kernel = "";

  DevBuf b_verts1, b_tris1, st_times;
  void *d_verts1 = nullptr;
  void *d_tris1 = nullptr;

  DevBuf b_prim_masks, b_leaf_masks, st_ray_masks;
  uint32_t *d_prim_masks = nullptr;
  bool leaf_masks_stale = true;
};

inline nrt_status fail(nrt_ctx *c, nrt_status st, const char *fmt, ...) {
  char buf[512];
  va_list ap;
  va_start(ap, fmt);
  vsnprintf(buf, sizeof(buf), fmt, ap);
  va_end(ap);
  if (c)
    c->err = buf;
  else
    g_create_error = buf;
  return st;
}

#define HIPCHK(c, call)                                                                   \
  do {                                                                                    \
    hipError_t e_ = (call);                                                               \
    if (e_ != hipSuccess)                                                                 \
      return fail((c), NRT_ERR_DEVICE, "%s failed: %s (%s:%d)", #call, hipGetErrorString(e_), \
                  __FILE__, __LINE__);                                                    \
  } while (0)

inline nrt_status ensure(nrt_ctx *c, DevBuf &b, size_t bytes) {
  HIPCHK(c, devbuf_ensure(&b, bytes));
  return NRT_OK;
}

inline hipError_t wait_record(nrt_ctx::LaunchSlot &sl) {
  if (!sl.rec_pending) return hipSuccess;
  volatile uint32_t *seq = &sl.h_done->seq;
  const auto t_start = std::chrono::steady_clock::now();
  for (unsigned long spins = 0; *seq != sl.seq; spins++) {
    if (spins < 4000) continue;
    std::this_thread::sleep_for(std::chrono::microseconds(20));
    if ((spins & 1023) == 0 && std::chrono::steady_clock::now() - t_start > std::chrono::seconds(30)) {
      hipError_t e = hipDeviceSynchronize();
      if (e != hipSuccess) return e;
      if (*seq != sl.seq) return hipErrorUnknown;
    }
  }
  std::atomic_thread_fence(std::memory_order_acquire);
  sl.rec_pending = false;
  return hipSuccess;
}

inline hipError_t slot_done(nrt_ctx *c, nrt_ctx::LaunchSlot &sl) {
  (void)c;
  if (!sl.used) return hipSuccess;
  if (sl.last_has_rec) return wait_record(sl);
  return sl.done ? hipEventSynchronize(sl.done) : hipSuccess;
}

inline hipError_t refit_host_wait_locked(nrt_ctx *c) {
  if (!c->refit_pending) return hipSuccess;
  hipError_t e = hipEventSynchronize(c->ev_refit);
  if (e != hipSuccess) return e;
  c->refit_pending = false;
  return hipSuccess;
}
inline hipError_t refit_host_wait(nrt_ctx *c) {
  std::lock_guard<std::mutex> lock(c->launch_mutex);
  return refit_host_wait_locked(c);
}

inline hipError_t refit_stream_wait(nrt_ctx *c, hipStream_t s) {
  if (!c->refit_pending) return hipSuccess;
  const hipError_t q = hipEventQuery(c->ev_refit);
  if (q == hipSuccess) {
    c->refit_pending = false;
    return hipSuccess;
  }
  if (q != hipErrorNotReady) return q;
  return hipStreamWaitEvent(s, c->ev_refit, 0);
}

inline hipError_t wait_for_launches(nrt_ctx *c) {
  std::lock_guard<std::mutex> lock(c->launch_mutex);
  hipError_t re = refit_host_wait_locked(c);
  if (re != hipSuccess) return re;
  for (nrt_ctx::LaunchSlot &sl : c->slots) {
    hipError_t e = slot_done(c, sl);
    if (e != hipSuccess) return e;
  }
  return hipStreamSynchronize(c->stream);
}

inline void free_tree(nrt_ctx *c) {
  c->generation++;
  c->d_wide = nullptr;
  c->d_wide4 = nullptr;
  c->d_nodes = nullptr;
  c->d_indices = nullptr;
  c->d_tris = nullptr;
  c->d_tris1 = nullptr;
  c->leaf_masks_stale = true;
  c->num_nodes = c->num_indices = 0;
  c->tree_depth = 0;
  c->refit_planned = false;
}

inline void free_mesh(nrt_ctx *c) {
  c->d_verts = nullptr;
  c->d_faces = nullptr;
  c->d_radii = nullptr;
  c->d_verts1 = nullptr;
  c->d_prim_masks = nullptr;
  c->num_faces = c->num_verts = 0;
  c->num_segs = 0;
}
```

### nanort_amd/csrc/kernels.h

```cpp
#pragma once
#include <string>

#include "common.h"

nrt_status nrt_internal_tree_view(nrt_ctx *c, nrt::TreeViewF32 *out);
uint64_t nrt_internal_generation(const nrt_ctx *c);
int nrt_internal_device(const nrt_ctx *c);
int nrt_internal_prim_kind(const nrt_ctx *c);

namespace nrt {

#define NRT_INSTANTIATE_F32_F64(fn)       \
  template decltype(fn<float>) fn<float>; \
  template decltype(fn<double>) fn<double>;

template <typename T>
hipError_t launch_traverse(const TraverseArgs<T> &, unsigned grid, bool count, int lds_entries, hipStream_t);
template <typename T>
int traverse_blocks_per_cu(int lds_entries);
template <typename T>
hipError_t launch_traverse_wide(const TraverseArgs<T> &args, unsigned grid, int lds_entries, int prim_kind, hipStream_t, const char **name_out);
template <typename T>
int traverse_wide_blocks_per_cu(int lds_entries, int prim_kind, bool wide4);
template <typename T>
hipError_t launch_make_wide(const typename Wire<T>::Node *nodes, uint32_t n, uint32_t packed, uint32_t *scratch, WideNode<T> *wide,
                            Wide4Node<T> *wide4, uint32_t scramble_mod, hipStream_t s);

hipError_t launch_scene_trace(const SceneTraceArgs &args, unsigned grid, hipStream_t s);
int scene_trace_blocks_per_cu();
hipError_t launch_scene_walk(const SceneWalkArgs &args, unsigned grid, hipStream_t s);
int scene_walk_blocks_per_cu();
enum SceneListForm : int { kSceneListScan, kSceneListBvh, kSceneListW4, kSceneListW4Prune };
hipError_t launch_scene_list(SceneListForm form, const TreeViewF32 &top, const nrt_ray_f32 *rays, uint32_t n, const NodeDev *nodes, uint32_t num_nodes,
                             uint32_t cap, float *list_t, uint32_t *list_node, uint32_t *count, const uint32_t *subset, const uint32_t *inst_masks,
                             const uint32_t *ray_masks, hipStream_t s);

enum OwnWalk : int {
  kOwnMultiHit,
  kOwnMotion,
  kOwnMasked,
  kOwnQueryMotion, kOwnQueryMasked, kOwnQueryMotionMasked,
  kOwnMultiHitIds, kOwnMultiHitMotion, kOwnMultiHitMasked, kOwnMultiHitMotionMasked,
  kNumOwnWalks
};
template <typename T>
struct OwnWalkInputs {
  uint32_t max_hits;
  uint32_t *counts;
  const void *tris1;
  const T *times;
  const uint32_t *leaf_masks;
  const uint32_t *ray_masks;
};
template <typename T>
hipError_t launch_own_walk(OwnWalk w, const TraverseArgs<T> &args, const OwnWalkInputs<T> &in, unsigned grid, hipStream_t s, const char **name_out);
template <typename T>
int own_walk_blocks_per_cu(OwnWalk w);

enum : unsigned { kBuildMorton = 1u, kBuildSubtreeDfs = 2u };
struct BuildResult {
  uint64_t num_nodes;
  uint32_t max_depth, num_leaves, num_branches, max_leaf_count;
};
template <typename T>
hipError_t gpu_build(hipStream_t s, const T *d_verts, const T *d_verts1, const uint32_t *d_faces, const T *d_radii, int prim_kind, const uint32_t *d_prim_map,
                     uint32_t num_faces, uint32_t min_leaf, uint32_t max_depth, uint32_t bin_size, unsigned build_flags, DevBuf *workspace,
                     DevBuf *nodes_buf, DevBuf *indices_buf, void *pinned, hipEvent_t ev, std::string *err);
hipError_t gpu_build_result(const void *pinned, hipEvent_t ev, BuildResult *res);

template <typename T>
struct TopNode;
template <typename T>
struct PrimRec;
struct LeafRule;
struct LevelInfo;
template <typename T>
const uint16_t *launch_subtree(TopNode<T> *top, const uint32_t *small_list, const PrimRec<T> *recs0, const PrimRec<T> *recs1, int Ks,
                               LeafRule rule, typename Wire<T>::Node *scratch, uint16_t *premap, uint32_t *indices, LevelInfo *info,
                               uint32_t num_small, bool dfs_form, hipStream_t stream);

size_t refit_plan_bytes(uint32_t tree_depth, uint64_t num_nodes);
template <typename T>
hipError_t launch_refit_plan(const typename Wire<T>::Node *nodes, uint64_t num_nodes, uint32_t num_branch_records, uint32_t tree_depth,
                             uint32_t root_is_branch, uint32_t *plan, hipStream_t s);
template <typename T>
hipError_t launch_refit(const void *src, size_t stride, uint32_t nv, T *verts, const uint32_t *faces, const uint32_t *indices,
                        typename Wire<T>::Node *nodes, uint64_t num_nodes, uint32_t num_branch_records, uint32_t tree_depth,
                        const uint32_t *plan, hipStream_t s);
hipError_t launch_refit_prims(int kind, const float *verts, const float *radii, const uint32_t *indices, nrt_node_f32 *nodes, uint64_t num_nodes,
                              uint32_t num_branch_records, uint32_t tree_depth, const uint32_t *plan, hipStream_t s);

hipError_t launch_max_index(const uint32_t *faces, uint64_t n_indices, uint32_t *out, hipStream_t s);
template <typename T>
hipError_t launch_gather_vertices(const void *src, size_t stride, uint32_t nv, T *tight, hipStream_t s);
template <typename T>
hipError_t launch_permute_masks(const void *tris, const uint32_t *masks, uint32_t num_faces, uint32_t *leaf_masks, uint32_t n, hipStream_t s);
hipError_t launch_cylinder_segments(const float *verts, const float *radii, const uint32_t *seg_off, uint32_t n, float *seg_verts,
                                    float *seg_radii, uint32_t *seg_prim, hipStream_t s);
template <typename T>
size_t leaf_record_bytes(int kind);
template <typename T>
hipError_t launch_gather_leaf(int kind, const uint32_t *indices, const uint32_t *faces, const T *verts, const T *radii, void *out, uint32_t n,
                              hipStream_t s);
template <typename T>
hipError_t launch_post_pass(int kind, const typename Wire<T>::Ray *rays, typename Wire<T>::Hit *hits, const uint8_t *bits, const T *verts, uint32_t n,
                            void *out, uint8_t *mask, DoneRec *done_rec, DoneCount *done_count, uint32_t done_seq, hipStream_t s);

}
```

### nanort_amd/csrc/traverse.hip

```cpp
#include "binary_walk_dev.h"
#include "kernels.h"
#include "walk_dev.h"

#include <algorithm>

namespace nrt {

template <typename T, bool COUNT>
struct ClosestQuery : BinaryQuery {
  unsigned long long c_nodes = 0, c_leaves = 0, c_tris = 0;
  unsigned c_stack = 0;
  uint32_t skip = 0;

  __device__ __forceinline__ typename Wire<T>::Ray load(const TraverseArgs<T> &a, uint32_t rid) const {
    return load_ray<T>(as_global(a.rays) + rid, a.debug_flags);
  }
  __device__ __forceinline__ void begin(const TraverseArgs<T> &, uint32_t) {
    if (COUNT) c_stack = c_stack > 1u ? c_stack : 1u;
  }
  __device__ __forceinline__ void node() {
    if (COUNT) c_nodes++;
  }
  __device__ __forceinline__ void pushed(int sp) {
    if (COUNT) {
      const unsigned need = (unsigned)sp + 1u;
      c_stack = need > c_stack ? need : c_stack;
    }
  }
  __device__ __forceinline__ void leaf() {
    if (COUNT) c_leaves++;
  }
  __device__ __forceinline__ void enter_leaves(const TraverseArgs<T> &a, uint32_t rid, bool at_leaf) {
    skip = a.skip_prim;
    if constexpr (!COUNT)
      if (a.skip_ids != nullptr && at_leaf) skip = a.skip_ids[rid];
  }
  __device__ __forceinline__ void record(const TraverseArgs<T> &a, Lane<T> &L, uint32_t, uint32_t k) {
    const LeafTri<T> tri = a.tris[k];
    if (COUNT) c_tris++;
    tri_test<T>(L, tri, true, a.range0, a.range1, skip, a.cull_back_face != 0);
  }
  __device__ __forceinline__ void finish(const TraverseArgs<T> &a, const Lane<T> &L, uint32_t rid) const { store_closest_hit<T>(a, L, rid); }
  __device__ __forceinline__ void after(const TraverseArgs<T> &a, unsigned lane) {
    if (!COUNT) return;
    for (int off = 32; off > 0; off >>= 1) {
      c_nodes += __shfl_xor(c_nodes, off);
      c_leaves += __shfl_xor(c_leaves, off);
      c_tris += __shfl_xor(c_tris, off);
      const unsigned o = __shfl_xor(c_stack, off);
      c_stack = o > c_stack ? o : c_stack;
    }
    if (lane == 0) {
      atomicAdd(&a.counters[0], c_nodes);
      atomicAdd(&a.counters[1], c_leaves);
      atomicAdd(&a.counters[2], c_tris);
      atomicMax(&a.counters[3], (unsigned long long)c_stack);
    }
  }
};

template <typename T, bool COUNT, int STACK>
__global__ __launch_bounds__(kTraverseBlock) void k_traverse(const TraverseArgs<T> a) {
  __shared__ uint32_t s_stack[STACK][kTraverseBlock];
  binary_walk<T, STACK>(a, s_stack, ClosestQuery<T, COUNT>());
}

#ifndef NRT_W4_P1_UNROLL
#define NRT_W4_P1_UNROLL 2
#endif
#ifndef NRT_W2_F64_P1_UNROLL
#define NRT_W2_F64_P1_UNROLL 2
#endif
#ifndef NRT_W4_PRESEL
#define NRT_W4_PRESEL 1
#endif
#ifndef NRT_W2_F64_PRESEL
#define NRT_W2_F64_PRESEL 1
#endif
#ifndef NRT_W4_TRI_UNROLL
#define NRT_W4_TRI_UNROLL 2
#endif
#ifndef NRT_SPHERE_UNROLL
#define NRT_SPHERE_UNROLL 2
#endif
#ifndef NRT_W2_TRI_UNROLL
#define NRT_W2_TRI_UNROLL 2
#endif
#ifndef NRT_W4_WAVES
#define NRT_W4_WAVES 1
#endif

__device__ __forceinline__ uint32_t quad_or(uint32_t x) {
  x |= (uint32_t)__builtin_amdgcn_update_dpp(0, (int)x, 0xB1, 0xF, 0xF, true);
  x |= (uint32_t)__builtin_amdgcn_update_dpp(0, (int)x, 0x4E, 0xF, 0xF, true);
  return x;
}
template <int K>
__device__ __forceinline__ float quad_bcast(float v) {
  return __int_as_float(__builtin_amdgcn_update_dpp(0, __float_as_int(v), K * 0x55, 0xF, 0xF, true));
}

template <typename T, int STACK, bool STATS, int KIND, bool PLAIN = false, bool CLOCK = false, int WIDTH = 2, int ORDER = 0>
__global__ __launch_bounds__(kTraverseBlock, (WIDTH == 4 && sizeof(T) == 4) ? NRT_W4_WAVES : 1) void k_traverse_wide(const TraverseArgs<T> a) {
  static_assert(WIDTH == 2 || WIDTH == 4, "one or two tree levels per step");
  static_assert(KIND != kPrimCurves || sizeof(T) == 4, "curves are fp32 only, as their example");
  static_assert(ORDER == 0 || (WIDTH == 4 && sizeof(T) == 4), "distance order / leaf items are variants of the fp32 two-level step");
  static_assert((ORDER & 2) == 0 || (KIND == kPrimTriangles && !STATS), "leaf items: triangle records, production instantiations");
  static_assert((ORDER & 4) == 0 || ((ORDER & 1) == 0 && KIND == kPrimTriangles && !STATS && !CLOCK), "records addressed by 64-bit offsets: the default walk of triangle trees");
  constexpr bool LEAFC = (ORDER & 2) != 0;
  constexpr bool BIG = (ORDER & 4) != 0;
  typedef typename std::conditional<BIG, uint64_t, uint32_t>::type RecOff;
  constexpr bool QUAD = WIDTH == 4 && sizeof(T) == 4 && KIND == kPrimTriangles && !STATS && (ORDER & 1) == 0 && !BIG;
  __shared__ uint32_t s_item_owner[LEAFC ? kTraverseBlock / kWave : 1][LEAFC ? kWave : 1];
  __shared__ uint32_t s_item_rec[LEAFC ? kTraverseBlock / kWave : 1][LEAFC ? kWave : 1];
  typedef StackEntry<T> SE;
  __shared__ typename SE::type s_stack[STACK][kTraverseBlock];

  typedef typename Wire<T>::Node Node;
  typedef typename Wire<T>::Ray Ray;
  typedef typename Wire<T>::Hit Hit;

  const unsigned tid = threadIdx.x;
  const unsigned lane = lane_id();
  const unsigned gslot = blockIdx.x * kTraverseBlock + tid;
  const bool cull = a.cull_back_face != 0;
  const LaneStack<SE, STACK, TraverseArgs<T>> stk = {a, tid, gslot};

  NRT_BATCH_TABLE_SETUP();
  Lane<T> L;
  uint32_t rid = kInvalid;
  uint32_t cur = 0;
  int state = W_IDLE;
  int sp = 0;
  const bool clocked = CLOCK && a.wave_clock != nullptr;
  unsigned long long clk_begin = 0ull, clk_dry = 0ull;
  unsigned long long clk_l16 = 0ull, clk_l8 = 0ull, clk_l4 = 0ull;
  if (clocked) clk_begin = __builtin_amdgcn_s_memrealtime();
#define NRT_TAIL_N (a.tail_lanes < 16u ? a.tail_lanes : 16u)
#define NRT_CLOCK_LIVE(live_)                                                  \
  do {                                                                         \
    if constexpr (CLOCK) {                                                     \
      if (clocked && ck.exhausted && clk_l4 == 0ull && (live_) <= 16u) {       \
        const unsigned long long now_ = __builtin_amdgcn_s_memrealtime();      \
        if (clk_l16 == 0ull) clk_l16 = now_;                                   \
        if (clk_l8 == 0ull && (live_) <= 8u) clk_l8 = now_;                    \
        if ((live_) <= 4u) clk_l4 = now_;                                      \
      }                                                                        \
    }                                                                          \
  } while (0)
  Claim ck;
  claim_init<T>(a, ck);
  if (blockIdx.x == 0 && threadIdx.x < kMaxParts)
    __hip_atomic_store(a.next_cursor + kCursorStrideWords * threadIdx.x, 0u, __ATOMIC_RELAXED, __HIP_MEMORY_SCOPE_AGENT);
  done_begin<T>(a);
  unsigned long long st_it1 = 0, st_act1 = 0, st_idle2 = 0, st_it2 = 0, st_act2 = 0, st_refills = 0, st_refilled = 0, st_entries2 = 0;
  uint32_t st_steps = 0, st_tris = 0;
  unsigned long long st_t_refill = 0, st_t_p1 = 0, st_t_p2 = 0, st_act2b = 0, st_stamp = 0;
  unsigned long long st_it1_s = 0, st_act1_s = 0, st_it2_s = 0, st_act2_s = 0;

#define NRT_WRITE_RESULT()                              \
  do {                                                  \
    const bool hit_ = L.hit_t < L.max_t;                \
    Hit h_;                                             \
    h_.u = hit_ ? L.u : T(0);                           \
    h_.v = hit_ ? L.v : T(0);                           \
    if (STATS && (a.debug_flags & 64u)) {               \
      h_.u = T(st_steps);                               \
      h_.v = T(st_tris);                                \
    }                                                   \
    h_.t = hit_ ? L.hit_t : L.max_t;                    \
    h_.prim_id = hit_ ? L.prim : kInvalid;              \
    Hit NRT_GLOBAL *hp_ = as_global(a.hits);            \
    uint8_t NRT_GLOBAL *mp_ = as_global(a.mask);        \
    if (multi) {                                        \
      const BatchPtrs bp_ = s_tbl[batch_of<T>(a, rid)]; \
      hp_ = as_global((Hit *)bp_.hits_v);               \
      mp_ = as_global(bp_.mask_v);                      \
    }                                                   \
    if (hp_) store_hit_nt<T>(hp_ + rid, h_);            \
    if (mp_) mp_[rid] = hit_ ? ((KIND == kPrimCylinders && !a.any_hit) ? (uint8_t)(1u | (L.cap << 1)) : (uint8_t)1) : (uint8_t)0;  \
  } while (0)

#define NRT_RAY_SKIP(skip_, live_)                                                                     \
  uint32_t skip_ = a.skip_prim;                                                                        \
  if constexpr (!PLAIN && KIND == kPrimTriangles) {                                                    \
    const uint32_t NRT_GLOBAL *ids_ = as_global(a.skip_ids);                                           \
    if (multi) ids_ = as_global(s_tbl[batch_of<T>(a, rid)].skip_v);                                    \
    if ((live_) && ids_ != nullptr) skip_ = ids_[rid];                                                 \
  }                                                                                                    \
  (void)skip_

  const bool anyhit_ = KIND != kPrimTriangles && a.any_hit != 0u;
#define NRT_RAY_OPEN(AH_) (!((AH_) && L.hit_t < L.max_t))

#define NRT_TEST_PRIM(slot_, act_, AH_)                                                                \
  do {                                                                                                 \
    if (KIND == kPrimSpheres) {                                                                        \
      const LeafSphere<T> sp_ = a.spheres[(slot_)];                                                    \
      sphere_test<T>(L, sp_, (act_), a.range0, a.range1);                                              \
    } else if (KIND == kPrimCylinders) {                                                               \
      const LeafCylinder<T> cy_ = a.cylinders[(slot_)];                                                \
      cylinder_test<T>(L, cy_, (act_), a.range0, a.range1, a.cyl_test_cap != 0u);                      \
    } else if constexpr (KIND == kPrimCurves) {    \
      const LeafCurve cv_ = a.curves[(slot_)];                                                         \
      curve_test<T>(L, cv_, (act_), a.range0, a.range1, a.curve_subdiv, (AH_));                        \
    } else {                                                                                           \
      const LeafTri<T> tri_ = a.tris[(slot_)];                                                         \
      if (PLAIN)                                                                                       \
        tri_test<T, true>(L, tri_, (act_), 0u, 0u, 0u, false);                                         \
      else                                                                                             \
        tri_test<T>(L, tri_, (act_), a.range0, a.range1, skip, cull);                                  \
    }                                                                                                  \
  } while (0)

#define NRT_SPHERE_LOOP(AH_)                                                                                              \
  for (uint32_t i = 0; __ballot(i < cnt && NRT_RAY_OPEN(AH_)) != 0ull; i += NRT_SPHERE_UNROLL) {                          \
    LeafSphere<T> s_[NRT_SPHERE_UNROLL];                                                                                  \
    _Pragma("unroll") for (uint32_t j = 0; j < NRT_SPHERE_UNROLL; j++) s_[j] = a.spheres[first + (i + j < cnt ? i + j : 0u)]; \
    _Pragma("unroll") for (uint32_t j = 0; j < NRT_SPHERE_UNROLL; j++)                                                    \
      sphere_test<T>(L, s_[j], i + j < cnt && NRT_RAY_OPEN(AH_), a.range0, a.range1);                                     \
  }
#define NRT_RECORD_LOOP(AH_)                                                                                              \
  for (uint32_t i = 0; __ballot(i < cnt && NRT_RAY_OPEN(AH_)) != 0ull; i++) {                                             \
    if (STATS) {                                                                                                          \
      st_it2++;                                                                                                           \
      st_act2 += (unsigned)__builtin_popcountll(__ballot(i < cnt));                                                       \
      if (i < cnt) st_tris++;                                                                                             \
    }                                                                                                                     \
                        \
    NRT_TEST_PRIM(first + (i < cnt ? i : 0u), i < cnt && NRT_RAY_OPEN(AH_), AH_);                                         \
  }

  bool to_tail = false;
  unsigned long long tail_idle = 0ull;
  for (;;) {
    if (STATS) st_stamp = __builtin_amdgcn_s_memtime();
    unsigned long long idle = __ballot(state == W_IDLE);
    if (!ck.exhausted && (unsigned)__builtin_popcountll(idle) >= a.refill_min) {
      unsigned long long fresh = idle;
      while (fresh != 0ull && !ck.exhausted) {
        if (ck.next == ck.end && !claim_chunk<T>(a, ck, lane, __builtin_ctzll(fresh))) break;
        const unsigned want = (unsigned)__builtin_popcountll(fresh);
        const unsigned avail = ck.end - ck.next;
        const unsigned take = want < avail ? want : avail;
        const unsigned rank = (unsigned)__builtin_popcountll(fresh & ((1ull << lane) - 1ull));
        if (state == W_IDLE && rank < take) {
          if (rid != kInvalid) NRT_WRITE_RESULT();
          rid = ck.next + rank;
          const Ray NRT_GLOBAL *rp_ = as_global(a.rays);
          uint32_t bq_ = 0u;
          if (multi) {
            const uint32_t b_ = batch_of<T>(a, rid);
            rp_ = as_global((const Ray *)s_tbl[b_].rays_v);
            bq_ = (a.batch_anyhit >> b_) & 1u;
          }
          const Ray r = load_ray<T>(rp_ + rid, a.debug_flags);
          lane_init<T>(L, r);
          L.pk |= bq_ << 9;
          sp = 0;
          if (STATS) st_steps = st_tris = 0;
          if (a.root_is_branch && !a.root_test) {
            cur = 0u;
            state = W_TRAV;
          } else if (a.root_is_branch) {
            const Node root = a.nodes[0];
            cur = 0u;
            state = slab_test<T>(L, root.bmin, root.bmax) ? W_TRAV : W_POP;
          } else {
            const Node root = a.nodes[0];
            const bool root_hit = slab_test<T>(L, root.bmin, root.bmax);
            cur = a.packed_leaves ? packed_leaf_ref(root.data[0], root.data[1]) : 0u;
            state = root_hit ? W_LEAF : W_POP;
          }
          if (a.debug_flags & 2u) state = W_POP;
        }
        if (STATS) {
          st_refills++;
          st_refilled += take;
        }
        ck.next += take;
        fresh = __ballot(state == W_IDLE);
      }
      idle = __ballot(state == W_IDLE);
    }
    if (clocked && ck.exhausted && clk_dry == 0ull) clk_dry = __builtin_amdgcn_s_memrealtime();
    NRT_CLOCK_LIVE(64u - (unsigned)__builtin_popcountll(idle));
    if constexpr (QUAD) {
      const unsigned live_n_ = 64u - (unsigned)__builtin_popcountll(idle);
      if (ck.exhausted && live_n_ != 0u && live_n_ <= NRT_TAIL_N) {
        tail_idle = idle;
        to_tail = true;
        break;
      }
    }
    if (idle == ~0ull) {
      if (ck.exhausted) break;
      continue;
    }

    if (STATS) {
      const unsigned long long now_ = __builtin_amdgcn_s_memtime();
      st_t_refill += now_ - st_stamp;
      st_stamp = now_;
    }
    unsigned n_wait_leaf = (unsigned)__builtin_popcountll(__ballot(state == W_LEAF));
    while (state == W_TRAV || state == W_POP) {
      if (STATS) {
        st_it1++;
        st_act1 += (unsigned)__builtin_popcountll(__ballot(true));
        if (!ck.exhausted) {
          st_it1_s++;
          st_act1_s += (unsigned)__builtin_popcountll(__ballot(true));
        }
      }
#pragma unroll
      for (int u_ = 0; u_ < ((WIDTH == 4 && sizeof(T) == 4 && !STATS) ? NRT_W4_P1_UNROLL : ((WIDTH == 2 && sizeof(T) == 8 && !STATS) ? NRT_W2_F64_P1_UNROLL : 1)); u_++) {
      if (state == W_POP) NRT_POP_ENTRY(stk);
      if (state == W_TRAV) {
        if (STATS) st_steps++;
        if constexpr (WIDTH == 4) {
#if NRT_W4_PRESEL
          if constexpr (sizeof(T) == 4) {
            const char *wb_ = reinterpret_cast<const char *>(a.wide4);
            const RecOff rec_ = (RecOff)cur << 7;
            const Slab4<float> sl = slab4_presel<RecOff>(L, wb_, rec_);
            const Wide4Tail w = *reinterpret_cast<const Wide4Tail *>(wb_ + (size_t)rec_ + 96);
            if constexpr ((ORDER & 1) == 1)
              NRT_STEP_NODE4_DIST(sl, w);
            else
              NRT_STEP_NODE4_SL(sl, w);
          } else
#endif
          {
            const Wide4Node<T> w = a.wide4[cur];
            NRT_STEP_NODE4(w);
          }
        } else {
#ifdef NRT_PROBE_EXTRA_LOADS
          typedef uint32_t u4v_ __attribute__((ext_vector_type(4)));
          u4v_ d0_;
          asm volatile("global_load_dwordx4 %0, %1, off" : "=v"(d0_) : "v"(a.wide + cur) : "memory");
          for (int x_ = 1; x_ < NRT_PROBE_EXTRA_LOADS; x_++)
            asm volatile("global_load_dwordx4 %0, %1, off offset:16" : "+v"(d0_) : "v"(a.wide + cur) : "memory");
#endif
#if NRT_W2_F64_PRESEL
          bool stepped_ = false;
          if constexpr (sizeof(T) == 8) {
            if (a.wide_below_4g) {
              const char *wb_ = reinterpret_cast<const char *>(a.wide);
              const uint32_t rec_ = cur * (uint32_t)sizeof(WideNode<double>);
              const SlabPair<double> sl = slab_pair_presel(L, wb_, rec_);
              const WideTail w = *reinterpret_cast<const WideTail *>(wb_ + (size_t)rec_ + 96);
              NRT_STEP_NODE_SL(sl, w);
              stepped_ = true;
            }
          }
          if (!stepped_)
#endif
          {
          const WideNode<T> w = a.wide[cur];
#ifdef NRT_PROBE_EXTRA_VALU
          {
            float f_ = __uint_as_float(cur);
            for (int x_ = 0; x_ < NRT_PROBE_EXTRA_VALU; x_++) asm volatile("v_fma_f32 %0, %0, %0, %0" : "+v"(f_));
            asm volatile("" :: "v"(f_));
          }
#endif
          NRT_STEP_NODE(w);
          }
#ifdef NRT_PROBE_EXTRA_LOADS
          asm volatile("" :: "v"(d0_));
#endif
        }
      }
      }
      n_wait_leaf += (unsigned)__builtin_popcountll(__ballot(state == W_LEAF));
      const unsigned n_walk_ = (unsigned)__builtin_popcountll(__ballot(state == W_TRAV || state == W_POP));
      NRT_CLOCK_LIVE(n_walk_ + n_wait_leaf);
      if (n_walk_ < a.trav_min && (n_wait_leaf != 0u || !ck.exhausted)) break;
      if constexpr (QUAD) {
        if (ck.exhausted && n_walk_ + n_wait_leaf <= NRT_TAIL_N) break;
      }
    }
    if constexpr (QUAD) {
      if (ck.exhausted && (unsigned)__builtin_popcountll(__ballot(state != W_IDLE)) <= NRT_TAIL_N) continue;
    }

    if (STATS) {
      const unsigned long long now_ = __builtin_amdgcn_s_memtime();
      st_t_p1 += now_ - st_stamp;
      st_stamp = now_;
    }
    const unsigned n_leaf = (unsigned)__builtin_popcountll(__ballot(state == W_LEAF));
    const bool refill_due = !ck.exhausted && (unsigned)__builtin_popcountll(__ballot(state == W_IDLE)) >= a.refill_min;
    if (n_leaf != 0u && !(n_leaf < a.leaf_min && refill_due)) {
      uint32_t cnt = 0, first = 0;
      if (state == W_LEAF) leaf_span(a.packed_leaves, a.nodes, cur, cnt, first);
      if (a.debug_flags & 1u) cnt = 0;
      NRT_RAY_SKIP(skip, state == W_LEAF);
      if (STATS) {
        st_entries2++;
        st_idle2 += (unsigned)__builtin_popcountll(__ballot(state == W_IDLE));
      }
      bool items_done_ = false;
      if constexpr (LEAFC) {
        items_done_ = leaf_items_one_trip<PLAIN, uint32_t>(L, cnt, a.tris, first, lane, s_item_owner[tid / kWave], s_item_rec[tid / kWave], a.range0, a.range1,
                                                 skip, cull);
      }
      if (items_done_) {
      } else if constexpr (KIND == kPrimTriangles && (WIDTH == 4 ? NRT_W4_TRI_UNROLL : NRT_W2_TRI_UNROLL) > 1) {
        constexpr uint32_t U_ = WIDTH == 4 ? NRT_W4_TRI_UNROLL : NRT_W2_TRI_UNROLL;
        for (uint32_t i = 0; __ballot(i < cnt) != 0ull; i += U_) {
          LeafTri<T> t_[U_];
          if (STATS) {
            st_it2++;
            st_act2 += (unsigned)__builtin_popcountll(__ballot(i < cnt));
            st_act2b += (unsigned)__builtin_popcountll(__ballot(i + 1u < cnt));
            if (!ck.exhausted) {
              st_it2_s++;
              st_act2_s += (unsigned)__builtin_popcountll(__ballot(i < cnt)) + (unsigned)__builtin_popcountll(__ballot(i + 1u < cnt));
            }
            if (i < cnt) st_tris += (i + 1u < cnt) ? 2u : 1u;
          }
#pragma unroll
          for (uint32_t j = 0; j < U_; j++) t_[j] = a.tris[first + (i + j < cnt ? i + j : 0u)];
#pragma unroll
          for (uint32_t j = 0; j < U_; j++) {
            if (PLAIN)
              tri_test<T, true>(L, t_[j], i + j < cnt, 0u, 0u, 0u, false);
            else
              tri_test<T>(L, t_[j], i + j < cnt, a.range0, a.range1, skip, cull);
          }
        }
      } else if constexpr (!STATS && KIND == kPrimSpheres && NRT_SPHERE_UNROLL > 1) {
        if (anyhit_) {
          NRT_SPHERE_LOOP(true)
        } else {
          NRT_SPHERE_LOOP(false)
        }
      } else if constexpr (KIND != kPrimTriangles) {
        if (anyhit_) {
          NRT_RECORD_LOOP(true)
        } else {
          NRT_RECORD_LOOP(false)
        }
      } else {
        NRT_RECORD_LOOP(false)
      }
      if (a.any_hit | a.batch_anyhit) sp = (state == W_LEAF && L.hit_t < L.max_t && (a.any_hit != 0u || (L.pk & 512u) != 0u)) ? 0 : sp;
      state = (state == W_LEAF) ? W_POP : state;
    }
    if (STATS) st_t_p2 += __builtin_amdgcn_s_memtime() - st_stamp;
  }
  if constexpr (QUAD) {
    if (to_tail) {
      const unsigned long long idle = tail_idle;
      const unsigned live_n_ = 64u - (unsigned)__builtin_popcountll(idle);
      if (state == W_IDLE && rid != kInvalid) NRT_WRITE_RESULT();
      const unsigned q_ = lane >> 2, j_ = lane & 3u;
      uint32_t src_ = 0u;
      {
        unsigned k_ = 0u;
        for (unsigned long long m_ = ~idle; m_ != 0ull; m_ &= m_ - 1ull, k_++) src_ = (q_ == k_) ? (uint32_t)__builtin_ctzll(m_) : src_;
      }
      const bool has_ = q_ < live_n_;
      const int sa_ = (int)(src_ << 2);
#define NRT_QMOVE_F(x_) x_ = __int_as_float(__builtin_amdgcn_ds_bpermute(sa_, __float_as_int(x_)))
#define NRT_QMOVE_U(x_) x_ = (uint32_t)__builtin_amdgcn_ds_bpermute(sa_, (int)(x_))
      NRT_QMOVE_F(L.org0);
      NRT_QMOVE_F(L.org1);
      NRT_QMOVE_F(L.org2);
      NRT_QMOVE_F(L.inv0);
      NRT_QMOVE_F(L.inv1);
      NRT_QMOVE_F(L.inv2);
      NRT_QMOVE_F(L.min_t);
      NRT_QMOVE_F(L.max_t);
      NRT_QMOVE_F(L.hit_t);
      NRT_QMOVE_F(L.Sx);
      NRT_QMOVE_F(L.Sy);
      NRT_QMOVE_F(L.Sz);
      NRT_QMOVE_F(L.u);
      NRT_QMOVE_F(L.v);
      NRT_QMOVE_U(L.pk);
      NRT_QMOVE_U(L.prim);
      NRT_QMOVE_U(rid);
      NRT_QMOVE_U(cur);
      state = __builtin_amdgcn_ds_bpermute(sa_, state);
      sp = __builtin_amdgcn_ds_bpermute(sa_, sp);
#undef NRT_QMOVE_F
#undef NRT_QMOVE_U
      L.so0 = (L.pk & 1u) ? 48u : 0u;
      L.so1 = (L.pk & 2u) ? 48u : 0u;
      L.so2 = (L.pk & 4u) ? 48u : 0u;
      state = has_ ? state : W_IDLE;
      rid = has_ ? rid : kInvalid;
      sp = has_ ? sp : 0;
      const unsigned otid_ = (tid & ~63u) | src_;
      const LaneStack<SE, STACK, TraverseArgs<T>> ostk_ = {a, otid_, blockIdx.x * kTraverseBlock + otid_};
      bool owner_ = j_ == 0u;
      const char *wb_ = reinterpret_cast<const char *>(a.wide4);
      for (;;) {
        const unsigned long long liveq_ = __ballot(state != W_IDLE);
        NRT_CLOCK_LIVE((unsigned)__builtin_popcountll(liveq_) >> 2);
        if (liveq_ == 0ull) break;
        if (state == W_POP) NRT_POP_ENTRY(ostk_);
        if (state == W_TRAV) {
          const uint32_t rec0_ = cur << 7, rec_ = rec0_ + 4u * j_, rec48_ = rec_ + 48u;
          const float lo0 = *reinterpret_cast<const float *>(wb_ + (size_t)(rec_ + L.so0));
          const float hi0 = *reinterpret_cast<const float *>(wb_ + (size_t)(rec48_ - L.so0));
          const float lo1 = *reinterpret_cast<const float *>(wb_ + (size_t)(rec_ + L.so1) + 16);
          const float hi1 = *reinterpret_cast<const float *>(wb_ + (size_t)(rec48_ - L.so1) + 16);
          const float lo2 = *reinterpret_cast<const float *>(wb_ + (size_t)(rec_ + L.so2) + 32);
          const float hi2 = *reinterpret_cast<const float *>(wb_ + (size_t)(rec48_ - L.so2) + 32);
          const uint32_t c_ = *reinterpret_cast<const uint32_t *>(wb_ + (size_t)rec_ + 96);
          const int ax0_ = *reinterpret_cast<const int32_t *>(wb_ + (size_t)rec0_ + 112);
          const int axh_ = *reinterpret_cast<const int32_t *>(wb_ + (size_t)(rec0_ + 4u * (j_ >> 1)) + 116);
          float tmin = L.min_t, tmax = L.hit_t;
          slab_axis<float>(lo0, hi0, L.org0, L.inv0, tmin, tmax);
          slab_axis<float>(lo1, hi1, L.org1, L.inv1, tmin, tmax);
          slab_axis<float>(lo2, hi2, L.org2, L.inv2, tmin, tmax);
          const bool h_ = (tmin <= tmax) & (((j_ & 1u) == 0u) | (c_ != kWide4Empty));
          const uint32_t s0_ = (uint32_t)L.sign(ax0_), sh_ = (uint32_t)L.sign(axh_);
          const uint32_t rank_ = ((((j_ >> 1) ^ s0_) & 1u) << 1) | ((j_ ^ sh_) & 1u);
          const uint32_t m_ = quad_or(h_ ? (1u << rank_) : 0u);
          const uint32_t n_ = (uint32_t)__builtin_popcount(m_);
          const uint32_t pos_ = (uint32_t)__builtin_popcount(m_ & ((1u << rank_) - 1u));
          if (h_ && pos_ != 0u) NRT_STACK_STORE(ostk_, sp + (int)(n_ - 1u - pos_), c_, tmin);
          __builtin_amdgcn_fence(__ATOMIC_RELEASE, "wavefront");
          sp += n_ != 0u ? (int)(n_ - 1u) : 0;
          const uint32_t next_ = quad_or((h_ && pos_ == 0u) ? c_ : 0u);
          cur = n_ != 0u ? (next_ & ~kLeafBit) : cur;
          state = n_ != 0u ? ((next_ & kLeafBit) ? W_LEAF : W_TRAV) : W_POP;
        }
        if (__ballot(state == W_LEAF) != 0ull) {
          uint32_t cnt = 0, first = 0;
          if (state == W_LEAF) leaf_span(a.packed_leaves, a.nodes, cur, cnt, first);
          if (a.debug_flags & 1u) cnt = 0;
          NRT_RAY_SKIP(skip, state == W_LEAF);
          for (uint32_t i = 0; __ballot(i < cnt) != 0ull; i += 4u) {
            const bool act_ = i + j_ < cnt;
            const LeafTri<T> tri = a.tris[first + (act_ ? i + j_ : 0u)];
            const uint32_t prim_i = tri.prim_id;
            const TriSolve<T> ts_ = tri_solve<T, PLAIN>(tri, act_, L.org0, L.org1, L.org2, L.Sx, L.Sy, L.Sz, L.kx(), L.ky(), L.kz(), a.range0, a.range1, skip, cull);
            const bool ok = ts_.ok;
            const T tt_i = ts_.tt, uu_i = ts_.uu, vv_i = ts_.vv;
            const uint32_t okm_ = quad_or(ok ? (1u << j_) : 0u);
            if (__ballot(okm_ != 0u) != 0ull) {
              bool got_ = false;
              uint32_t win_ = 0u;
#define NRT_QUAD_ACCEPT(K_)                                                                                                    \
              do {                                                                                                           \
                const T ttk_ = quad_bcast<K_>(tt_i);                                                                         \
                const bool acc_ = ((okm_ >> K_) & 1u) != 0u && !(ttk_ > L.hit_t) && !(ttk_ < L.min_t);  \
                L.hit_t = acc_ ? ttk_ : L.hit_t;                                                                             \
                win_ = acc_ ? (uint32_t)K_ : win_;                                                                           \
                got_ = got_ | acc_;                                                                                          \
              } while (0)
              NRT_QUAD_ACCEPT(0);
              NRT_QUAD_ACCEPT(1);
              NRT_QUAD_ACCEPT(2);
              NRT_QUAD_ACCEPT(3);
#undef NRT_QUAD_ACCEPT
              const bool me_ = got_ & (win_ == j_);
              owner_ = got_ ? me_ : owner_;
              L.u = me_ ? uu_i : L.u;
              L.v = me_ ? vv_i : L.v;
              L.prim = me_ ? prim_i : L.prim;
            }
          }
          if (a.any_hit | a.batch_anyhit) sp = (state == W_LEAF && L.hit_t < L.max_t && (a.any_hit != 0u || (L.pk & 512u) != 0u)) ? 0 : sp;
          state = (state == W_LEAF) ? W_POP : state;
        }
      }
      if (owner_ && rid != kInvalid) NRT_WRITE_RESULT();
      rid = kInvalid;
    }
  }
  if (rid != kInvalid) NRT_WRITE_RESULT();
#undef NRT_WRITE_RESULT
#undef NRT_RECORD_LOOP
#undef NRT_SPHERE_LOOP
#undef NRT_TEST_PRIM
#undef NRT_RAY_OPEN
#undef NRT_RAY_SKIP
#undef NRT_CLOCK_LIVE
#undef NRT_TAIL_N
  done_end<T>(a, lane);
  if (clocked && lane == 0u) {
    unsigned long long *rec = a.wave_clock + (size_t)kWaveClockWords * (size_t)(gslot / kWave);
    const unsigned long long clk_end = __builtin_amdgcn_s_memrealtime();
    rec[0] = clk_begin;
    rec[1] = clk_dry == 0ull ? clk_end : clk_dry;
    rec[2] = clk_end;
    rec[3] = clk_l16 == 0ull ? clk_end : clk_l16;
    rec[4] = clk_l8 == 0ull ? clk_end : clk_l8;
    rec[5] = clk_l4 == 0ull ? clk_end : clk_l4;
  }
  if (STATS && lane == 0) {
    atomicAdd(&a.counters[0], st_it1);
    atomicAdd(&a.counters[1], st_act1);
    atomicAdd(&a.counters[2], st_idle2);
    atomicAdd(&a.counters[3], st_it2);
    atomicAdd(&a.counters[4], st_act2);
    atomicAdd(&a.counters[5], st_refills);
    atomicAdd(&a.counters[6], st_refilled);
    atomicAdd(&a.counters[7], st_entries2);
    atomicAdd(&a.counters[8], st_t_refill);
    atomicAdd(&a.counters[9], st_t_p1);
    atomicAdd(&a.counters[10], st_t_p2);
    atomicAdd(&a.counters[11], st_act2b);
    atomicAdd(&a.counters[12], st_it1_s);
    atomicAdd(&a.counters[13], st_act1_s);
    atomicAdd(&a.counters[14], st_it2_s);
    atomicAdd(&a.counters[15], st_act2_s);
  }
}

__device__ __forceinline__ uint32_t block_exclusive_scan_256(uint32_t v, uint32_t *s_wave, uint32_t &total) {
  const unsigned lane = threadIdx.x & 63, w = threadIdx.x >> 6;
  uint32_t inc = v;
  for (int off = 1; off < 64; off <<= 1) {
    const uint32_t t = __shfl_up(inc, off);
    if (lane >= (unsigned)off) inc += t;
  }
  if (lane == 63) s_wave[w] = inc;
  __syncthreads();
  uint32_t pre = 0;
  total = 0;
  for (unsigned j = 0; j < 4; j++) {
    if (j < w) pre += s_wave[j];
    total += s_wave[j];
  }
  __syncthreads();
  return pre + inc - v;
}

template <typename T>
__global__ __launch_bounds__(256) void k_wide_count(const typename Wire<T>::Node *__restrict__ nodes, uint32_t n,
                                                    uint32_t *__restrict__ tile_count) {
  __shared__ uint32_t s_wave[4];
  uint32_t c = 0;
  const uint32_t base = blockIdx.x * 1024u + threadIdx.x * 4u;
  for (uint32_t k = 0; k < 4; k++)
    if (base + k < n && nodes[base + k].flag == 0) c++;
  uint32_t total;
  (void)block_exclusive_scan_256(c, s_wave, total);
  if (threadIdx.x == 0) tile_count[blockIdx.x] = total;
}

__global__ __launch_bounds__(256) void k_wide_scan_tiles(uint32_t *tile_count, uint32_t num_tiles) {
  __shared__ uint32_t s_wave[4];
  uint32_t carry = 0;
  for (uint32_t base = 0; base < num_tiles; base += 256u) {
    const uint32_t i = base + threadIdx.x;
    const uint32_t v = i < num_tiles ? tile_count[i] : 0u;
    uint32_t total;
    const uint32_t ex = block_exclusive_scan_256(v, s_wave, total);
    if (i < num_tiles) tile_count[i] = carry + ex;
    carry += total;
  }
}

template <typename T>
__global__ __launch_bounds__(256) void k_wide_index(const typename Wire<T>::Node *__restrict__ nodes, uint32_t n,
                                                    const uint32_t *__restrict__ tile_base,
                                                    uint32_t *__restrict__ dense_of, uint32_t scramble_mod) {
  __shared__ uint32_t s_wave[4];
  const uint32_t base = blockIdx.x * 1024u + threadIdx.x * 4u;
  uint32_t flags[4], c = 0;
  for (uint32_t k = 0; k < 4; k++) {
    flags[k] = (base + k < n && nodes[base + k].flag == 0) ? 1u : 0u;
    c += flags[k];
  }
  uint32_t total;
  uint32_t ex = tile_base[blockIdx.x] + block_exclusive_scan_256(c, s_wave, total);
  for (uint32_t k = 0; k < 4; k++) {
    if (base + k < n) dense_of[base + k] = scramble_mod ? (uint32_t)(((uint64_t)ex * 2654435761ull) % scramble_mod) : ex;
    ex += flags[k];
  }
}

template <typename T>
__global__ __launch_bounds__(256) void k_make_wide(const typename Wire<T>::Node *__restrict__ nodes, uint32_t n,
                                                   const uint32_t *__restrict__ dense_of, uint32_t packed,
                                                   WideNode<T> *__restrict__ wide, Wide4Node<T> *__restrict__ wide4) {
  typedef typename Wire<T>::Node Node;
  const uint32_t i = blockIdx.x * 256u + threadIdx.x;
  if (i >= n) return;
  const Node nd = nodes[i];
  if (nd.flag != 0) return;
  if (nd.data[0] >= n || nd.data[1] >= n) return;
  const Node a = nodes[nd.data[0]], b = nodes[nd.data[1]];
  WideNode<T> w;
#pragma unroll
  for (int k = 0; k < 3; k++) {
    if constexpr (sizeof(T) == 8) {
      w.mn[k][0] = a.bmin[k];
      w.mx[k][0] = a.bmax[k];
      w.mn[k][1] = b.bmin[k];
      w.mx[k][1] = b.bmax[k];
    } else {
      w.box0[k] = a.bmin[k];
      w.box0[3 + k] = a.bmax[k];
      w.box1[k] = b.bmin[k];
      w.box1[3 + k] = b.bmax[k];
    }
  }
  const uint32_t la = packed ? packed_leaf_ref(a.data[0], a.data[1]) : nd.data[0];
  const uint32_t lb = packed ? packed_leaf_ref(b.data[0], b.data[1]) : nd.data[1];
  w.c0 = a.flag != 0 ? (kLeafBit | la) : dense_of[nd.data[0]];
  w.c1 = b.flag != 0 ? (kLeafBit | lb) : dense_of[nd.data[1]];
  w.axis = nd.axis;
  w.pad = 0;
  wide[dense_of[i]] = w;
  if (wide4 == nullptr) return;
  Wide4Node<T> q;
  q.axis0 = nd.axis;
  q.pad = 0;
#pragma unroll
  for (int h = 0; h < 2; h++) {
    const Node &ch = h == 0 ? a : b;
    const uint32_t ch_ref = h == 0 ? w.c0 : w.c1;
    const bool two = ch.flag == 0 && ch.data[0] < n && ch.data[1] < n;
    int32_t axis = 0;
    if (two) {
      axis = ch.axis;
#pragma unroll
      for (int j = 0; j < 2; j++) {
        const uint32_t gi = ch.data[j];
        const Node g = nodes[gi];
#pragma unroll
        for (int k = 0; k < 3; k++) {
          q.bmin[k][2 * h + j] = g.bmin[k];
          q.bmax[k][2 * h + j] = g.bmax[k];
        }
        const uint32_t lg = packed ? packed_leaf_ref(g.data[0], g.data[1]) : gi;
        q.c[2 * h + j] = g.flag != 0 ? (kLeafBit | lg) : dense_of[gi];
      }
    } else {
#pragma unroll
      for (int k = 0; k < 3; k++) {
        q.bmin[k][2 * h] = ch.bmin[k];
        q.bmax[k][2 * h] = ch.bmax[k];
        q.bmin[k][2 * h + 1] = ch.bmin[k];
        q.bmax[k][2 * h + 1] = ch.bmax[k];
      }
      q.c[2 * h] = ch_ref;
      q.c[2 * h + 1] = kWide4Empty;
    }
    if (h == 0) q.axis1 = axis; else q.axis2 = axis;
  }
  wide4[dense_of[i]] = q;
}


template <typename T>
static const void *traverse_kernel(bool count, int lds_entries) {
  switch (lds_entries) {
    case 16: return count ? (const void *)k_traverse<T, true, 16> : (const void *)k_traverse<T, false, 16>;
    case 24: return count ? (const void *)k_traverse<T, true, 24> : (const void *)k_traverse<T, false, 24>;
    default: return count ? (const void *)k_traverse<T, true, 32> : (const void *)k_traverse<T, false, 32>;
  }
}
template <typename T>
hipError_t launch_traverse(const TraverseArgs<T> &args, unsigned grid, bool count, int lds_entries, hipStream_t s) {
  launch_persistent(traverse_kernel<T>(count, lds_entries), grid, args, s);
  return hipGetLastError();
}
template <typename T>
int traverse_blocks_per_cu(int lds_entries) {
  return resident_blocks(traverse_kernel<T>(false, lds_entries), 4);
}

#ifdef NRT_PROF
constexpr bool kProfBuild = true;
#else
constexpr bool kProfBuild = false;
#endif
struct WideKernel {
  WalkVariant v;
  const void *kernel;
  const char *name;
};
#define NRT_STR2(x) #x
#define NRT_STR(x) NRT_STR2(x)
#define NRT_WIDE_KERNEL(T_, STACK_, STATS_, KIND_, PLAIN_, CLOCK_, WIDTH_, ORDER_)                          \
  {{sizeof(T_) == 4, STACK_, STATS_, KIND_, PLAIN_, CLOCK_, WIDTH_, ORDER_},                                \
   (const void *)k_traverse_wide<T_, STACK_, STATS_, KIND_, PLAIN_, CLOCK_, WIDTH_, ORDER_>,                \
   "nrt::k_traverse_wide<" #T_ ", " NRT_STR(STACK_) ", " #STATS_ ", " #KIND_ ", " #PLAIN_ ", " #CLOCK_ ", " #WIDTH_ ", " #ORDER_ ">"},
static const WideKernel kWideKernels[] = {
    NRT_WALK_VARIANTS(NRT_WIDE_KERNEL)
#ifdef NRT_PROF
    NRT_WALK_VARIANTS_PROF(NRT_WIDE_KERNEL)
#endif
};
#undef NRT_WIDE_KERNEL
static const WideKernel *find_wide_kernel(const WalkVariant &v) {
  for (const WideKernel &k : kWideKernels)
    if (k.v == v) return &k;
  return nullptr;
}

template <typename T>
hipError_t launch_traverse_wide(const TraverseArgs<T> &args, unsigned grid, int lds_entries, int prim_kind, hipStream_t s,
                                const char **name_out) {
  const WalkRequest r = {sizeof(T) == 4, prim_kind, lds_entries, args.wide4 != nullptr, args.wide4_big != 0, args.leaf_items != 0, args.order4 != 0,
                         args.plain_options != 0, (args.debug_flags & 32u) != 0, args.wave_clock != nullptr};
  const WideKernel *k = find_wide_kernel(pick_wide_variant(r, kProfBuild));
  if (!k) return hipErrorInvalidValue;
  NRT_RANGE_PUSH(k->name);
  launch_persistent(k->kernel, grid, args, s);
  NRT_RANGE_POP();
  if (name_out) *name_out = k->name;
  return hipGetLastError();
}

template <typename T>
int traverse_wide_blocks_per_cu(int lds_entries, int prim_kind, bool wide4) {
  const WideKernel *k = find_wide_kernel(occupancy_variant(sizeof(T) == 4, prim_kind, lds_entries, wide4));
  return k ? resident_blocks(k->kernel, 4) : 4;
}

template <typename T>
hipError_t launch_make_wide(const typename Wire<T>::Node *nodes, uint32_t n, uint32_t packed, uint32_t *scratch,
                            WideNode<T> *wide, Wide4Node<T> *wide4, uint32_t scramble_mod, hipStream_t s) {
  if (n == 0) return hipSuccess;
  const uint32_t tiles = (n + 1023u) / 1024u;
  uint32_t *tile_count = scratch, *dense_of = scratch + tiles;
  hipLaunchKernelGGL((k_wide_count<T>), dim3(tiles), dim3(256), 0, s, nodes, n, tile_count);
  hipLaunchKernelGGL(k_wide_scan_tiles, dim3(1), dim3(256), 0, s, tile_count, tiles);
  hipLaunchKernelGGL((k_wide_index<T>), dim3(tiles), dim3(256), 0, s, nodes, n, tile_count, dense_of, scramble_mod);
  hipLaunchKernelGGL((k_make_wide<T>), dim3((n + 255u) / 256u), dim3(256), 0, s, nodes, n, dense_of, packed, wide, wide4);
  return hipGetLastError();
}

NRT_INSTANTIATE_F32_F64(launch_traverse)
NRT_INSTANTIATE_F32_F64(launch_traverse_wide)
NRT_INSTANTIATE_F32_F64(traverse_wide_blocks_per_cu)
NRT_INSTANTIATE_F32_F64(launch_make_wide)
NRT_INSTANTIATE_F32_F64(traverse_blocks_per_cu)

}
```

Baseline: 7257 Mrays/s.

## Poll mapped host memory for build state, fuse branch ranking, widen split scan

The build state block moves to mapped, coherent host memory. Kernels now write level and tree counters into it with system-scope atomics and a sequence number, and the host polls that number instead of issuing a D2H memcpy and waiting on an event each checked level. The layout and emit kernels also compute a dense rank for each branch node during the build, so make_wide can skip its count/scan/index kernels when scrambling is off. k_split gets a 4-wave variant that spreads the chunk prefix scan when nodes have many chunks. Together these aim to cut BVH build latency, at the cost of host spin-polling and extra scratch memory.

```diff
diff --git a/nanort_amd/csrc/api_ctx.hip b/nanort_amd/csrc/api_ctx.hip
--- a/nanort_amd/csrc/api_ctx.hip
+++ b/nanort_amd/csrc/api_ctx.hip
@@ -78,9 +78,9 @@
   if ((e = hipSetDevice(device)) != hipSuccess ||
       (e = hipStreamCreateWithFlags(&c->stream, hipStreamNonBlocking)) != hipSuccess ||
       (e = hipEventCreate(&c->ev_b0)) != hipSuccess || (e = hipEventCreate(&c->ev_b1)) != hipSuccess ||
-      (e = hipEventCreateWithFlags(&c->ev_build_state, hipEventDisableTiming)) != hipSuccess ||
       (e = hipEventCreateWithFlags(&c->ev_refit, hipEventDisableTiming)) != hipSuccess ||
-      (e = hipHostMalloc(&c->build_state, kBuildPinnedBytes, hipHostMallocDefault)) != hipSuccess ||
+      (e = hipHostMalloc(&c->build_state, kBuildPinnedBytes, hipHostMallocPortable | hipHostMallocMapped | hipHostMallocCoherent)) != hipSuccess ||
+      (e = hipHostGetDevicePointer(&c->d_build_state, c->build_state, 0)) != hipSuccess ||
       (e = hipMalloc((void **)&c->d_counters, 16 * sizeof(unsigned long long))) != hipSuccess) {
     fail(nullptr, NRT_ERR_DEVICE, "nrtCreate: %s", hipGetErrorString(e));
     nrtDestroy(c);
@@ -102,6 +102,7 @@
     }
   }
   for (nrt_ctx::LaunchSlot &sl : c->slots) memset(sl.h_done, 0, sizeof(DoneRec));
+  memset(c->build_state, 0, kBuildPinnedBytes);
   hipDeviceProp_t prop;
   if (hipGetDeviceProperties(&prop, device) == hipSuccess && prop.multiProcessorCount > 0)
     c->num_cus = prop.multiProcessorCount;
@@ -144,7 +145,7 @@
   if (c->d_counters) (void)hipFree(c->d_counters);
   if (c->build_state) (void)hipHostFree(c->build_state);
   if (c->h_max_index) (void)hipHostFree(c->h_max_index);
-  hipEvent_t evs[] = {c->ev_b0, c->ev_b1, c->ev_build_state, c->ev_refit};
+  hipEvent_t evs[] = {c->ev_b0, c->ev_b1, c->ev_refit};
   for (hipEvent_t ev : evs)
     if (ev) (void)hipEventDestroy(ev);
   for (int k = 0; k < 2; k++)
diff --git a/nanort_amd/csrc/api_tree.hip b/nanort_amd/csrc/api_tree.hip
--- a/nanort_amd/csrc/api_tree.hip
+++ b/nanort_amd/csrc/api_tree.hip
@@ -14,7 +14,7 @@
 }
 
 template <typename T>
-static nrt_status finish_wide(nrt_ctx *c, hipStream_t s) {
+static nrt_status finish_wide(nrt_ctx *c, hipStream_t s, bool ranked = false) {
   nrt_status st;
   if ((st = ensure(c, c->b_wide, std::max<size_t>(1, c->num_branch_records) * sizeof(WideNode<T>)))) return st;
   c->d_wide = c->b_wide.p;
@@ -28,7 +28,7 @@
     c->d_wide4 = c->b_wide4.p;
   }
   HIPCHK(c, launch_make_wide<T>((const typename Wire<T>::Node *)c->d_nodes, (uint32_t)c->num_nodes, c->packed_leaves,
-                                (uint32_t *)c->b_wide_scratch.p, (WideNode<T> *)c->d_wide, (Wide4Node<T> *)c->d_wide4,
+                                (uint32_t *)c->b_wide_scratch.p, ranked, (WideNode<T> *)c->d_wide, (Wide4Node<T> *)c->d_wide4,
                                 c->wide_scramble ? c->num_branch_records : 0u, s));
   return NRT_OK;
 }
@@ -159,12 +159,16 @@
   free_tree(c);
   BuildResult res;
   std::string err;
-  HIPCHK(c, hipEventRecord(c->ev_b0, c->stream));
   const bool segs = c->prim_kind == kPrimCylinders && c->num_segs != 0 && sizeof(T) == 4;
   const uint32_t build_n = segs ? c->num_segs : c->num_faces;
+  const bool ranked = !c->wide_scramble;
+  if (nrt_status st = ensure(c, c->b_wide_scratch, ((2 * (size_t)build_n + 1023) / 1024 + 2 * (size_t)build_n + 1) * sizeof(uint32_t))) return st;
+  const BuildStateRef state = {(volatile const BuildState *)c->build_state, (BuildState *)c->d_build_state, &c->build_seq};
+  HIPCHK(c, hipEventRecord(c->ev_b0, c->stream));
   hipError_t e = gpu_build<T>(c->stream, segs ? (const T *)c->b_seg_verts.p : (const T *)c->d_verts, c->prim_kind == kPrimTriangles ? (const T *)c->d_verts1 : nullptr, c->d_faces, segs ? (const T *)c->b_seg_radii.p : (const T *)c->d_radii,
                               c->prim_kind, segs ? (const uint32_t *)c->b_seg_prim.p : nullptr, build_n, min_leaf, max_depth,
-                              bin_size, (c->morton ? kBuildMorton : 0u) | (c->subtree_rows ? 0u : kBuildSubtreeDfs), &c->b_build_ws, &c->b_nodes, &c->b_indices, c->build_state, c->ev_build_state, &err);
+                              bin_size, (c->morton ? kBuildMorton : 0u) | (c->subtree_rows ? 0u : kBuildSubtreeDfs), &c->b_build_ws, &c->b_nodes, &c->b_indices,
+                              ranked ? (uint32_t *)c->b_wide_scratch.p : nullptr, state, &err);
   if (e != hipSuccess) return fail(c, NRT_ERR_DEVICE, "nrtBuild: %s (%s)", err.c_str(), hipGetErrorString(e));
   c->d_nodes = c->b_nodes.p;
   c->d_indices = (uint32_t *)c->b_indices.p;
@@ -176,7 +180,7 @@
     free_tree(c);
     return fst;
   }
-  if ((e = gpu_build_result(c->build_state, c->ev_build_state, &res)) != hipSuccess) {
+  if ((e = gpu_build_result(state, &res)) != hipSuccess) {
     free_tree(c);
     return fail(c, NRT_ERR_DEVICE, "nrtBuild: %s", hipGetErrorString(e));
   }
@@ -188,7 +192,7 @@
   c->min_leaf_count = 1;
   c->tree_nested = 1;
   NRT_RANGE_PUSH("build: WideNode / Wide4Node records");
-  fst = finish_wide<T>(c, c->stream);
+  fst = finish_wide<T>(c, c->stream, ranked);
   NRT_RANGE_POP();
   if (fst) {
     free_tree(c);
diff --git a/nanort_amd/csrc/build.hip b/nanort_amd/csrc/build.hip
--- a/nanort_amd/csrc/build.hip
+++ b/nanort_amd/csrc/build.hip
@@ -2,7 +2,10 @@
 #include <stdlib.h>
 
 #include <algorithm>
+#include <atomic>
+#include <chrono>
 #include <string>
+#include <thread>
 #include <vector>
 
 
@@ -443,7 +446,7 @@
 __global__ __launch_bounds__(1024) void k_level_setup(TopNode<T> *top, uint32_t *active, uint32_t *chunk_base,
                                                        LevelInfo *info, BoundsAcc<T> *child_acc, uint32_t max_active,
                                                        LeafRule rule, uint32_t dst_buf, uint32_t *small_list,
-                                                       int with_children) {
+                                                       int with_children, BuildState *state, uint32_t seq) {
   if (with_children) {
     const uint32_t prev_active = info->num_active;
     for (uint32_t a = threadIdx.x; a < prev_active; a += 1024u)
@@ -511,6 +514,13 @@
     if (A) {
       info->num_levels += 1;
       info->level_begin[info->num_levels] = tc + 2 * A;
+    }
+    if (seq) {
+      __hip_atomic_store(&state->num_active, A, __ATOMIC_RELAXED, __HIP_MEMORY_SCOPE_SYSTEM);
+      __hip_atomic_store(&state->num_small, __hip_atomic_load(&info->num_small, __ATOMIC_RELAXED, __HIP_MEMORY_SCOPE_AGENT),
+                         __ATOMIC_RELAXED, __HIP_MEMORY_SCOPE_SYSTEM);
+      __hip_atomic_store(&state->error, info->error, __ATOMIC_RELAXED, __HIP_MEMORY_SCOPE_SYSTEM);
+      __hip_atomic_store(&state->seq, seq, __ATOMIC_RELEASE, __HIP_MEMORY_SCOPE_SYSTEM);
     }
   }
 }
@@ -747,20 +757,11 @@
 }
 
 template <typename T>
-__global__ __launch_bounds__(64) void k_split(TopNode<T> *top, const uint32_t *__restrict__ active,
-                                              GBins<T> *gbins, int kpack,
-                                              const uint32_t *__restrict__ chunk_hist, uint32_t *chunk_left_base,
-                                              const LevelInfo *info, uint32_t max_active) {
-  const uint32_t a = blockIdx.x;
-  const uint32_t num_active = info->num_active;
-  if (a >= num_active) return;
-  const uint32_t next_top_base = info->child_base;
-  const unsigned lane = threadIdx.x;
-  TopNode<T> &nd = top[active[a]];
+__device__ __forceinline__ void node_cut(GBins<T> *gbins, uint32_t a, uint32_t num_active, uint32_t max_active, uint32_t n,
+                                         uint32_t nch, int kpack, unsigned lane, int &best_axis, uint32_t &best_bin,
+                                         uint32_t &best_nl) {
+  typedef typename Ord<T>::U U;
   GBins<T> &g = gbins[a];
-  typedef typename Ord<T>::U U;
-  const uint32_t n = nd.r - nd.l, cb = nd.chunk_base, nch = nd.nchunks;
-  if (nch == 1u) return;
   const int K = node_bins(kpack, n);
   uint32_t cnt3[3] = {0, 0, 0};
   U mn3[3][3], mx3[3][3];
@@ -814,14 +815,45 @@
     clean_bins<T>(&g, k, lane);
     if (a + num_active < max_active) clean_bins<T>(&gbins[a + num_active], k, lane);
   }
-  int best_axis;
-  uint32_t best_bin, best_nl;
   eval_split<T>(K, lane, cnt3, mn3, mx3, best_axis, best_bin, best_nl);
   if (best_bin == kMedian) best_nl = n >> 1;
+}
+
+template <typename T, int WAVES>
+__global__ __launch_bounds__(64 * WAVES) void k_split(TopNode<T> *top, const uint32_t *__restrict__ active,
+                                                      GBins<T> *gbins, int kpack,
+                                                      const uint32_t *__restrict__ chunk_hist, uint32_t *chunk_left_base,
+                                                      const LevelInfo *info, uint32_t max_active) {
+  const uint32_t a = blockIdx.x;
+  const uint32_t num_active = info->num_active;
+  if (a >= num_active) return;
+  const uint32_t next_top_base = info->child_base;
+  const unsigned lane = WAVES > 1 ? threadIdx.x & 63u : threadIdx.x, wave = WAVES > 1 ? threadIdx.x >> 6 : 0u;
+  __shared__ uint32_t s_cut[3];
+  __shared__ uint32_t s_total[2][WAVES];
+  TopNode<T> &nd = top[active[a]];
+  const uint32_t n = nd.r - nd.l, cb = nd.chunk_base, nch = nd.nchunks;
+  if (nch == 1u) return;
+  const bool shared = WAVES > 1 && nch > 64u;
+  if (!shared && wave != 0u) return;
+  int best_axis = 0;
+  uint32_t best_bin = 0, best_nl = 0;
+  if (wave == 0u) node_cut<T>(gbins, a, num_active, max_active, n, nch, kpack, lane, best_axis, best_bin, best_nl);
+  if (shared && lane == 0u) {
+    s_cut[0] = (uint32_t)best_axis;
+    s_cut[1] = best_bin;
+    s_cut[2] = best_nl;
+  }
+  if (shared) {
+    __syncthreads();
+    best_axis = (int)s_cut[0];
+    best_bin = s_cut[1];
+    best_nl = s_cut[2];
+  }
 
   uint32_t carry = 0;
-  for (uint32_t j0 = 0; j0 < nch; j0 += 64u) {
-    const uint32_t j = j0 + lane;
+  for (uint32_t j0 = 0, round = 0; j0 < nch; j0 += 64u * WAVES, round++) {
+    const uint32_t j = j0 + 64u * wave + lane;
     uint32_t left = 0;
     if (j < nch) {
       if (best_bin == kMedian) {
@@ -845,10 +877,22 @@
       const uint32_t t = __shfl_up(inc, off);
       if (lane >= (unsigned)off) inc += t;
     }
-    if (j < nch) chunk_left_base[cb + j] = carry + inc - left;
-    carry += __shfl(inc, 63);
-  }
-  if (lane == 0) {
+    uint32_t before = 0, total = __shfl(inc, 63);
+    if (shared) {
+      if (lane == 63u) s_total[round & 1u][wave] = inc;
+      __syncthreads();
+      total = 0;
+#pragma unroll
+      for (unsigned w = 0; w < (unsigned)WAVES; w++) {
+        const uint32_t t = s_total[round & 1u][w];
+        before += w < wave ? t : 0u;
+        total += t;
+      }
+    }
+    if (j < nch) chunk_left_base[cb + j] = carry + before + inc - left;
+    carry += total;
+  }
+  if (lane == 0 && wave == 0u) {
     nd.axis = best_axis;
     nd.split_bin = best_bin;
     nd.nleft = best_nl;
@@ -994,7 +1038,7 @@
 
 constexpr uint32_t kLayoutCut = 8;
 template <typename T>
-__global__ __launch_bounds__(1024) void k_layout(TopNode<T> *top, LevelInfo *info) {
+__global__ __launch_bounds__(1024) void k_layout(TopNode<T> *top, LevelInfo *info, uint32_t *top_rank) {
   extern __shared__ uint32_t s_dyn[];
   __shared__ uint32_t s_upper[1u << kLayoutCut];
   __shared__ uint32_t s_nupper;
@@ -1064,10 +1108,14 @@
     for (uint32_t j = 0; j < kLayoutOwn; j++) {
       const uint32_t i = threadIdx.x + 1024u * j;
       if (i < total) {
-        uint32_t dfs = 0;
-        for (uint32_t x = i, pw = s_par[i]; (pw & ~kHighChild) != kNoParent; x = pw & ~kHighChild, pw = s_par[x])
-          dfs += 1u + ((pw & kHighChild) ? s_size[x - 1u] : 0u);
+        uint32_t dfs = 0, rank = 0;
+        for (uint32_t x = i, pw = s_par[i]; (pw & ~kHighChild) != kNoParent; x = pw & ~kHighChild, pw = s_par[x]) {
+          const uint32_t low = (pw & kHighChild) ? s_size[x - 1u] : 0u;
+          dfs += 1u + low;
+          rank += 1u + (low ? (low - 1u) >> 1 : 0u);
+        }
         reinterpret_cast<uint2 *>(&top[i].l)[4] = make_uint2(((small_mask >> j) & 1u) ? own[j] : s_size[i], dfs);
+        top_rank[i] = rank;
       }
     }
     if (threadIdx.x == 0) info->num_nodes = s_size[0];
@@ -1125,22 +1173,36 @@
   }
 }
 template <typename T>
-__global__ __launch_bounds__(256) void k_layout_dfs(TopNode<T> *top, const LevelInfo *info) {
+__global__ __launch_bounds__(256) void k_layout_dfs(TopNode<T> *top, const LevelInfo *info, uint32_t *top_rank) {
   const uint32_t i = blockIdx.x * 256u + threadIdx.x;
   if (i >= info->top_count || info->top_count <= kLayoutLds) return;
-  uint32_t dfs = 0;
-  for (uint32_t x = i, pw = top[i].parent; (pw & ~kHighChild) != kNoParent; x = pw & ~kHighChild, pw = top[x].parent)
-    dfs += 1u + ((pw & kHighChild) ? top[x - 1u].size : 0u);
+  uint32_t dfs = 0, rank = 0;
+  for (uint32_t x = i, pw = top[i].parent; (pw & ~kHighChild) != kNoParent; x = pw & ~kHighChild, pw = top[x].parent) {
+    const uint32_t low = (pw & kHighChild) ? top[x - 1u].size : 0u;
+    dfs += 1u + low;
+    rank += 1u + (low ? (low - 1u) >> 1 : 0u);
+  }
   top[i].dfs = dfs;
+  top_rank[i] = rank;
 }
 
 template <typename T>
 __global__ __launch_bounds__(256) void k_emit_top(const TopNode<T> *__restrict__ top, const LevelInfo *info,
                                                   const PrimRec<T> *__restrict__ recs0,
                                                   const PrimRec<T> *__restrict__ recs1,
-                                                  typename Wire<T>::Node *nodes, uint32_t *indices) {
+                                                  typename Wire<T>::Node *nodes, uint32_t *indices,
+                                                  const uint32_t *__restrict__ top_rank, uint32_t *branch_rank,
+                                                  BuildState *state, uint32_t seq) {
   const uint32_t i = blockIdx.x * 256u + threadIdx.x;
   if (i >= info->top_count) return;
+  if (i == 0u && seq != 0u) {
+    __hip_atomic_store(&state->num_nodes, info->num_nodes, __ATOMIC_RELAXED, __HIP_MEMORY_SCOPE_SYSTEM);
+    __hip_atomic_store(&state->max_depth, info->max_depth, __ATOMIC_RELAXED, __HIP_MEMORY_SCOPE_SYSTEM);
+    __hip_atomic_store(&state->num_leaves, info->num_leaves, __ATOMIC_RELAXED, __HIP_MEMORY_SCOPE_SYSTEM);
+    __hip_atomic_store(&state->num_branches, info->num_branches, __ATOMIC_RELAXED, __HIP_MEMORY_SCOPE_SYSTEM);
+    __hip_atomic_store(&state->max_leaf_count, info->max_leaf_count, __ATOMIC_RELAXED, __HIP_MEMORY_SCOPE_SYSTEM);
+    __hip_atomic_store(&state->seq, seq, __ATOMIC_RELEASE, __HIP_MEMORY_SCOPE_SYSTEM);
+  }
   const TopNode<T> &t = top[i];
   if (t.kind == KIND_SMALL) return;
   typename Wire<T>::Node nd;
@@ -1154,6 +1216,7 @@
     nd.axis = t.axis;
     nd.data[0] = top[t.child0].dfs;
     nd.data[1] = top[t.child0 + 1].dfs;
+    if (branch_rank) branch_rank[t.dfs] = top_rank[i];
   } else {
     nd.flag = 1;
     nd.axis = 0;
@@ -1170,29 +1233,56 @@
                                                    const uint32_t *__restrict__ small_list,
                                                    const typename Wire<T>::Node *__restrict__ scratch_nodes,
                                                    const uint16_t *__restrict__ premap, typename Wire<T>::Node *nodes,
-                                                   const LevelInfo *info) {
+                                                   const LevelInfo *info, const uint32_t *__restrict__ top_rank,
+                                                   uint32_t *branch_rank) {
   if (blockIdx.x >= info->num_small) return;
-  const TopNode<T> &t = top[small_list[blockIdx.x]];
+  constexpr uint32_t kWords = 2u * kHandoff / 32u;
+  static_assert(kWords <= 64u, "one lane per word of the task's branch bits");
+  __shared__ uint32_t s_branch[kWords], s_before[kWords];
+  const uint32_t ti = small_list[blockIdx.x];
+  const TopNode<T> &t = top[ti];
   const typename Wire<T>::Node *src = scratch_nodes + 2 * (size_t)t.l;
+  if (threadIdx.x < kWords) s_branch[threadIdx.x] = 0u;
+  __syncthreads();
   if (premap) {
     const uint16_t *map = premap + 2 * (size_t)t.l;
     for (uint32_t i = threadIdx.x; i < t.size; i += 64u) {
       typename Wire<T>::Node nd = src[i];
+      const uint32_t m = map[i];
       if (nd.flag == 0) {
         nd.data[0] = t.dfs + map[nd.data[0]];
         nd.data[1] = t.dfs + map[nd.data[1]];
-      }
-      nodes[t.dfs + map[i]] = nd;
-    }
-    return;
-  }
-  for (uint32_t i = threadIdx.x; i < t.size; i += 64u) {
-    typename Wire<T>::Node nd = src[i];
-    if (nd.flag == 0) {
-      nd.data[0] += t.dfs;
-      nd.data[1] += t.dfs;
-    }
-    nodes[t.dfs + i] = nd;
+        atomicOr(&s_branch[m >> 5], 1u << (m & 31u));
+      }
+      nodes[t.dfs + m] = nd;
+    }
+  } else {
+    for (uint32_t i = threadIdx.x; i < t.size; i += 64u) {
+      typename Wire<T>::Node nd = src[i];
+      if (nd.flag == 0) {
+        nd.data[0] += t.dfs;
+        nd.data[1] += t.dfs;
+        atomicOr(&s_branch[i >> 5], 1u << (i & 31u));
+      }
+      nodes[t.dfs + i] = nd;
+    }
+  }
+  if (branch_rank == nullptr) return;
+  const uint32_t root_rank = top_rank[ti];
+  __syncthreads();
+  {
+    const uint32_t c = threadIdx.x < kWords ? (uint32_t)__builtin_popcount(s_branch[threadIdx.x]) : 0u;
+    uint32_t inc = c;
+    for (int off = 1; off < 64; off <<= 1) {
+      const uint32_t u = __shfl_up(inc, off);
+      if (threadIdx.x >= (unsigned)off) inc += u;
+    }
+    if (threadIdx.x < kWords) s_before[threadIdx.x] = inc - c;
+  }
+  __syncthreads();
+  for (uint32_t m = threadIdx.x; m < t.size; m += 64u) {
+    const uint32_t bits = s_branch[m >> 5], bit = 1u << (m & 31u);
+    if (bits & bit) branch_rank[t.dfs + m] = root_rank + s_before[m >> 5] + (uint32_t)__builtin_popcount(bits & (bit - 1u));
   }
 }
 
@@ -1202,7 +1292,7 @@
 struct BuildPlan {
   size_t max_top, max_active, max_chunks;
   size_t off_recs0, off_recs1, off_scratch, off_top, off_child_acc, off_active, off_chunk_base, off_gbins,
-      off_chunk_hist, off_chunk_left, off_small, off_scene, off_info, off_sort, off_premap, sort_blocks, total;
+      off_chunk_hist, off_chunk_left, off_small, off_scene, off_info, off_sort, off_premap, off_top_rank, sort_blocks, total;
   BuildPlan(uint32_t n, size_t top_scale, bool tiny_top = false) {
     typedef typename Wire<T>::Node Node;
     max_active = (size_t)n / kHandoff + 2;
@@ -1227,6 +1317,7 @@
     off_chunk_hist = take(max_chunks * 3 * kMaxBins * sizeof(uint32_t));
     off_chunk_left = take(max_chunks * sizeof(uint32_t));
     off_small = take((max_top + 1) * sizeof(uint32_t));
+    off_top_rank = take(max_top * sizeof(uint32_t));
     off_scene = take((1 + kSceneReplicas) * sizeof(BoundsAcc<T>));
     off_info = take(sizeof(LevelInfo));
     sort_blocks = ((size_t)n + kSortTile - 1) / kSortTile;
@@ -1244,17 +1335,41 @@
     }                                                                   \
   } while (0)
 
+static hipError_t wait_build_state(const BuildStateRef &state) {
+  const uint32_t want = *state.last_seq;
+  const auto t_start = std::chrono::steady_clock::now();
+  bool patient = false;
+  for (unsigned long spins = 1; state.host->seq != want; spins++) {
+    if (!patient && (spins & 255) != 0) continue;
+    const auto waited = std::chrono::steady_clock::now() - t_start;
+    if (!patient) {
+      patient = waited > std::chrono::milliseconds(50);
+      continue;
+    }
+    std::this_thread::sleep_for(std::chrono::microseconds(20));
+    if ((spins & 1023) == 0 && waited > std::chrono::seconds(30)) {
+      hipError_t e = hipDeviceSynchronize();
+      if (e != hipSuccess) return e;
+      if (state.host->seq != want) return hipErrorUnknown;
+    }
+  }
+  std::atomic_thread_fence(std::memory_order_acquire);
+  return hipSuccess;
+}
+
 template <typename T>
 hipError_t gpu_build(hipStream_t s, const T *d_verts, const T *d_verts1, const uint32_t *d_faces, const T *d_radii, int prim_kind, const uint32_t *d_prim_map, uint32_t n,
                      uint32_t min_leaf, uint32_t max_depth, uint32_t bin_size, unsigned build_flags, DevBuf *workspace, DevBuf *nodes_buf,
-                     DevBuf *indices_buf, void *pinned, hipEvent_t ev, std::string *err) {
+                     DevBuf *indices_buf, uint32_t *branch_rank, const BuildStateRef &state, std::string *err) {
   typedef typename Wire<T>::Node Node;
   const bool morton_order = (build_flags & kBuildMorton) != 0;
-  static_assert(offsetof(LevelInfo, level_begin) <= kBuildPinnedBytes, "state block");
+  auto next_seq = [&]() {
+    if (++*state.last_seq == 0u) ++*state.last_seq;
+    return *state.last_seq;
+  };
   const int K = (int)(bin_size < 2 ? 2 : (bin_size > (uint32_t)kMaxBins ? (uint32_t)kMaxBins : bin_size));
   const int Ks = K < kSmallBins ? K : kSmallBins;
-  const size_t state_bytes = offsetof(LevelInfo, level_begin);
-  volatile const LevelInfo *hp = (volatile const LevelInfo *)pinned;
+  volatile const BuildState *hp = state.host;
 
   const char *tiny_env = env_overrides_allowed() ? getenv("NRT_BUILD_TINY_TOP") : nullptr;
   const bool tiny_top = tiny_env && atoi(tiny_env) != 0;
@@ -1275,6 +1390,7 @@
     uint32_t *chunk_hist = (uint32_t *)(base + plan.off_chunk_hist);
     uint32_t *chunk_left = (uint32_t *)(base + plan.off_chunk_left);
     uint32_t *small_list = (uint32_t *)(base + plan.off_small);
+    uint32_t *top_rank = (uint32_t *)(base + plan.off_top_rank);
     BoundsAcc<T> *scene = (BoundsAcc<T> *)(base + plan.off_scene);
     LevelInfo *info = (LevelInfo *)(base + plan.off_info);
     uint32_t *indices = (uint32_t *)indices_buf->p;
@@ -1327,25 +1443,25 @@
       if (wide)
         hipLaunchKernelGGL((k_children<T>), dim3((unsigned)((prev_max + 255) / 256)), dim3(256), 0, s, top, active, child_acc,
                            (uint32_t)plan.max_active, rule, (uint32_t)cur, small_list, info);
+      const bool check = level >= first_check;
       hipLaunchKernelGGL((k_level_setup<T>), dim3(1), dim3(1024), 0, s, top, active, chunk_base, info, child_acc,
-                         (uint32_t)plan.max_active, rule, (uint32_t)cur, small_list, wide ? 0 : 1);
-      const bool check = level >= first_check;
-      if (check) {
-        BCHK(hipMemcpyAsync(pinned, info, state_bytes, hipMemcpyDeviceToHost, s));
-        BCHK(hipEventRecord(ev, s));
-      }
+                         (uint32_t)plan.max_active, rule, (uint32_t)cur, small_list, wide ? 0 : 1, state.dev, check ? next_seq() : 0u);
       const size_t a_max = level < 31 ? std::min<size_t>((size_t)1 << level, plan.max_active) : plan.max_active;
       const size_t c_max = std::min<size_t>((size_t)n / kTile + a_max + 1, plan.max_chunks);
       hipLaunchKernelGGL((k_bin<T>), dim3((unsigned)c_max), dim3(256), 0, s, top, active, chunk_base, info, recs[cur],
                          K | (Ks << 8), gbins, chunk_hist, chunk_left, (uint32_t)plan.max_active);
-      hipLaunchKernelGGL((k_split<T>), dim3((unsigned)a_max), dim3(64), 0, s, top, active, gbins, K | (Ks << 8), chunk_hist,
-                         chunk_left, info, (uint32_t)plan.max_active);
+      if ((size_t)n / kTile > 32 * a_max)
+        hipLaunchKernelGGL((k_split<T, 4>), dim3((unsigned)a_max), dim3(256), 0, s, top, active, gbins, K | (Ks << 8), chunk_hist,
+                           chunk_left, info, (uint32_t)plan.max_active);
+      else
+        hipLaunchKernelGGL((k_split<T, 1>), dim3((unsigned)a_max), dim3(64), 0, s, top, active, gbins, K | (Ks << 8), chunk_hist,
+                           chunk_left, info, (uint32_t)plan.max_active);
       hipLaunchKernelGGL((k_partition<T>), dim3((unsigned)c_max), dim3(256), 0, s, top, active, chunk_base, info,
                          chunk_left, recs[cur], recs[1 - cur], K | (Ks << 8), child_acc, (uint32_t)plan.max_active);
       BCHK(hipGetLastError());
       cur = 1 - cur;
       if (check) {
-        BCHK(hipEventSynchronize(ev));
+        BCHK(wait_build_state(state));
         if (hp->error) {
           overflow = true;
           break;
@@ -1371,25 +1487,24 @@
       hipLaunchKernelGGL((k_layout_init<T>), dim3(lg), dim3(256), 0, s, top, info);
       hipLaunchKernelGGL((k_layout_sizes<T>), dim3(lg), dim3(256), 0, s, top, info);
     }
-    hipLaunchKernelGGL((k_layout<T>), dim3(1), dim3(1024), 2 * kLayoutLds * sizeof(uint32_t), s, top, info);
+    hipLaunchKernelGGL((k_layout<T>), dim3(1), dim3(1024), 2 * kLayoutLds * sizeof(uint32_t), s, top, info, top_rank);
     if (plan.max_top > kLayoutLds)
-      hipLaunchKernelGGL((k_layout_dfs<T>), dim3((unsigned)((plan.max_top + 255) / 256)), dim3(256), 0, s, top, info);
-    BCHK(hipMemcpyAsync(pinned, info, state_bytes, hipMemcpyDeviceToHost, s));
-    BCHK(hipEventRecord(ev, s));
+      hipLaunchKernelGGL((k_layout_dfs<T>), dim3((unsigned)((plan.max_top + 255) / 256)), dim3(256), 0, s, top, info, top_rank);
     Node *nodes = (Node *)nodes_buf->p;
     hipLaunchKernelGGL((k_emit_top<T>), dim3((unsigned)((plan.max_top + 255) / 256)), dim3(256), 0, s, top, info, recs[0], recs[1],
-                       nodes, indices);
+                       nodes, indices, top_rank, branch_rank, state.dev, next_seq());
     if (num_small)
-      hipLaunchKernelGGL((k_emit_small<T>), dim3(num_small), dim3(64), 0, s, top, small_list, scratch, emit_map, nodes, info);
+      hipLaunchKernelGGL((k_emit_small<T>), dim3(num_small), dim3(64), 0, s, top, small_list, scratch, emit_map, nodes, info,
+                         top_rank, branch_rank);
     BCHK(hipGetLastError());
     return hipSuccess;
   }
 }
 
-hipError_t gpu_build_result(const void *pinned, hipEvent_t ev, BuildResult *res) {
-  hipError_t e = hipEventSynchronize(ev);
+hipError_t gpu_build_result(const BuildStateRef &state, BuildResult *res) {
+  hipError_t e = wait_build_state(state);
   if (e != hipSuccess) return e;
-  volatile const LevelInfo *hp = (volatile const LevelInfo *)pinned;
+  volatile const BuildState *hp = state.host;
   res->num_nodes = hp->num_nodes;
   res->max_depth = hp->max_depth;
   res->num_leaves = hp->num_leaves;
diff --git a/nanort_amd/csrc/ctx.h b/nanort_amd/csrc/ctx.h
--- a/nanort_amd/csrc/ctx.h
+++ b/nanort_amd/csrc/ctx.h
@@ -123,8 +123,9 @@
   struct { int lds_entries; unsigned blocks_per_cu; } occupancy[(int)Walk::Own + kNumOwnWalks][kNumPrimKinds] = {};
 
   hipEvent_t ev_b0 = nullptr, ev_b1 = nullptr;
-  hipEvent_t ev_build_state = nullptr;
   void *build_state = nullptr;
+  void *d_build_state = nullptr;
+  uint32_t build_seq = 0;
   int last_timed_slot = -1;
   int launch_timing = 0;
   bool have_build_time = false;
diff --git a/nanort_amd/csrc/kernels.h b/nanort_amd/csrc/kernels.h
--- a/nanort_amd/csrc/kernels.h
+++ b/nanort_amd/csrc/kernels.h
@@ -23,7 +23,7 @@
 template <typename T>
 int traverse_wide_blocks_per_cu(int lds_entries, int prim_kind, bool wide4);
 template <typename T>
-hipError_t launch_make_wide(const typename Wire<T>::Node *nodes, uint32_t n, uint32_t packed, uint32_t *scratch, WideNode<T> *wide,
+hipError_t launch_make_wide(const typename Wire<T>::Node *nodes, uint32_t n, uint32_t packed, uint32_t *scratch, bool ranked, WideNode<T> *wide,
                             Wide4Node<T> *wide4, uint32_t scramble_mod, hipStream_t s);
 
 hipError_t launch_scene_trace(const SceneTraceArgs &args, unsigned grid, hipStream_t s);
@@ -62,11 +62,22 @@
   uint64_t num_nodes;
   uint32_t max_depth, num_leaves, num_branches, max_leaf_count;
 };
+struct BuildState {
+  uint32_t num_active, num_small, error;
+  uint32_t num_nodes, max_depth, num_leaves, num_branches, max_leaf_count;
+  uint32_t seq;
+};
+static_assert(sizeof(BuildState) <= kBuildPinnedBytes, "state block");
+struct BuildStateRef {
+  volatile const BuildState *host;
+  BuildState *dev;
+  uint32_t *last_seq;
+};
 template <typename T>
 hipError_t gpu_build(hipStream_t s, const T *d_verts, const T *d_verts1, const uint32_t *d_faces, const T *d_radii, int prim_kind, const uint32_t *d_prim_map,
                      uint32_t num_faces, uint32_t min_leaf, uint32_t max_depth, uint32_t bin_size, unsigned build_flags, DevBuf *workspace,
-                     DevBuf *nodes_buf, DevBuf *indices_buf, void *pinned, hipEvent_t ev, std::string *err);
-hipError_t gpu_build_result(const void *pinned, hipEvent_t ev, BuildResult *res);
+                     DevBuf *nodes_buf, DevBuf *indices_buf, uint32_t *branch_rank, const BuildStateRef &state, std::string *err);
+hipError_t gpu_build_result(const BuildStateRef &state, BuildResult *res);
 
 template <typename T>
 struct TopNode;
diff --git a/nanort_amd/csrc/traverse.hip b/nanort_amd/csrc/traverse.hip
--- a/nanort_amd/csrc/traverse.hip
+++ b/nanort_amd/csrc/traverse.hip
@@ -822,14 +822,16 @@
 }
 
 template <typename T>
-hipError_t launch_make_wide(const typename Wire<T>::Node *nodes, uint32_t n, uint32_t packed, uint32_t *scratch,
+hipError_t launch_make_wide(const typename Wire<T>::Node *nodes, uint32_t n, uint32_t packed, uint32_t *scratch, bool ranked,
                             WideNode<T> *wide, Wide4Node<T> *wide4, uint32_t scramble_mod, hipStream_t s) {
   if (n == 0) return hipSuccess;
   const uint32_t tiles = (n + 1023u) / 1024u;
-  uint32_t *tile_count = scratch, *dense_of = scratch + tiles;
-  hipLaunchKernelGGL((k_wide_count<T>), dim3(tiles), dim3(256), 0, s, nodes, n, tile_count);
-  hipLaunchKernelGGL(k_wide_scan_tiles, dim3(1), dim3(256), 0, s, tile_count, tiles);
-  hipLaunchKernelGGL((k_wide_index<T>), dim3(tiles), dim3(256), 0, s, nodes, n, tile_count, dense_of, scramble_mod);
+  uint32_t *tile_count = scratch, *dense_of = ranked ? scratch : scratch + tiles;
+  if (!ranked) {
+    hipLaunchKernelGGL((k_wide_count<T>), dim3(tiles), dim3(256), 0, s, nodes, n, tile_count);
+    hipLaunchKernelGGL(k_wide_scan_tiles, dim3(1), dim3(256), 0, s, tile_count, tiles);
+    hipLaunchKernelGGL((k_wide_index<T>), dim3(tiles), dim3(256), 0, s, nodes, n, tile_count, dense_of, scramble_mod);
+  }
   hipLaunchKernelGGL((k_make_wide<T>), dim3((n + 255u) / 256u), dim3(256), 0, s, nodes, n, dense_of, packed, wide, wide4);
   return hipGetLastError();
 }
```

After: 7250 Mrays/s (median of 2 runs). No clear change (-0.1%).
